# NVIDIA/OpenSeq2Seq

Hardware: AMD Instinct MI355X
Metric: audio-frames/sec/node Jasper10x5 bf16 (train step, objects = input feature frames) (higher is better)
Workload: dtype bf16; 1 GPU; Jasper 10x5 DR (jasper10x5_LibriSpeech_nvgrad_masks) full train step: log-mel front end from int16 PCM resident in HBM+fwd+bwd+NovoGrad/LARC/Backoff, B=32/GPU, durations U[2,16.7]s padded to the batch max, F=64, V=29; global_batch=32, parallelism=dp1, skipped_steps=0

## Files before the change

include/os2s.h:

```cpp
#ifndef OS2S_H_
#define OS2S_H_

#include <stddef.h>
#include <stdint.h>

#ifdef __cplusplus
extern "C" {
#endif

typedef void* os2s_stream_t;

enum {
  OS2S_OK = 0,
  OS2S_ERR_INVALID_ARG = -1,
  OS2S_ERR_LAUNCH = -2,
  OS2S_ERR_UNSUPPORTED = -3,
  OS2S_ERR_WORKSPACE = -4
};

int os2s_abi_version(void);
const char* os2s_strerror(int code);
const char* os2s_last_error_detail(void);
int os2s_deterministic(void);
void os2s_set_deterministic(int on);

size_t os2s_ctc_greedy_decode_workspace_bytes(int T, int B);
int os2s_ctc_greedy_decode(os2s_stream_t stream, const float* logits,
                           const int32_t* seq_len, int T, int B, int V,
                           int blank, int merge_repeated, int32_t* out_ids,
                           int32_t* out_len, float* neg_sum_logits,
                           void* workspace, size_t workspace_bytes);

int os2s_conv1d_num_mtiles(int B, int Tout);
int os2s_conv1d_fwd_ex(os2s_stream_t stream, const uint16_t* x, const uint16_t* w, void* y,
                       const int32_t* in_len, const float* bias, float* stats, int B,
                       int Tin, int Cin, int Cout, int K, int stride, int dil, int padL,
                       int Tout, long long y_stride_b, long long y_stride_t, int out_f32,
                       int accumulate, int act, float keep_prob, unsigned long long seed,
                       const uint16_t* residual, const int32_t* out_len);
int os2s_conv1d_dgrad_bnact_ws(os2s_stream_t stream, const uint16_t* dy, const uint16_t* wT, void* dx,
                               float* stats, int B, int Tin, int Cin, int Cout, int K, int dil, int padL,
                               int Tout, int accumulate, const int32_t* out_len, const uint16_t* mask_ref,
                               float mask_scale, const uint16_t* stat_ref, void* workspace,
                               size_t workspace_bytes);
int os2s_bn_bwd_finalize_raw(os2s_stream_t stream, const float* partial, int nparts, int C, long long count,
                             const float* mean, const float* rstd, float* dgamma, float* dbeta,
                             int accumulate, float* c1, float* c2);
size_t os2s_conv1d_workspace_bytes(void);
int os2s_conv1d_fwd_ws(os2s_stream_t stream, const uint16_t* x, const uint16_t* w, void* y,
                       const int32_t* in_len, const float* bias, float* stats, int B,
                       int Tin, int Cin, int Cout, int K, int stride, int dil, int padL,
                       int Tout, long long y_stride_b, long long y_stride_t, int out_f32,
                       int accumulate, int act, float keep_prob, unsigned long long seed,
                       const uint16_t* residual, const int32_t* out_len, void* workspace,
                       size_t workspace_bytes);
int os2s_conv1d_set_host_lens(const int32_t* lens, int B);
int os2s_set_option(const char* name, double value);
int os2s_get_option(const char* name, double* value);
const char* os2s_option_name(int index);
int os2s_set_debug_stamps(const char* kernel, void* stamps, int mode);
int os2s_clock_probe(void* out_u64x2, unsigned long long spin_cycles);
int os2s_clock_probe_wait(void);
typedef struct {
  const uint16_t* x;
  const uint16_t* w;
  void* y;
  float* stats;
  int Cin, Cout, accumulate;
} os2s_conv_group_t;
int os2s_conv1x1_fwd_grouped(os2s_stream_t stream, const os2s_conv_group_t* groups, int ngroups,
                             const int32_t* in_len, const int32_t* out_len, int B, int T);
typedef struct {
  const uint16_t* x;
  const uint16_t* dy;
  float* dw;
  long long x_row_stride;
  int Cin, Cout;
} os2s_wgrad_group_t;
int os2s_conv1x1_wgrad_grouped(os2s_stream_t stream, const os2s_wgrad_group_t* groups, int ngroups,
                               const int32_t* in_len, int B, int T);
typedef struct {
  const uint16_t* x;
  const uint16_t* dy;
  float* dw;
  long long x_row_stride;
} os2s_cwgrad_group_t;
int os2s_conv1d_wgrad_grouped_ws(os2s_stream_t stream, const os2s_cwgrad_group_t* groups, int ngroups,
                                 const int32_t* in_len, int B, int Tin, int Cin, int Cout, int K,
                                 int stride, int dil, int padL, int Tout, int accumulate,
                                 void* workspace, size_t workspace_bytes);
int os2s_conv1x1_wgrad_grouped_ws(os2s_stream_t stream, const os2s_wgrad_group_t* groups, int ngroups,
                                  const int32_t* in_len, int B, int T, void* workspace,
                                  size_t workspace_bytes);
int os2s_gemm_wgrad_grouped(os2s_stream_t stream, const os2s_wgrad_group_t* groups, int ngroups,
                            long long M, int accumulate, void* workspace, size_t workspace_bytes);
int os2s_gemm_nt(os2s_stream_t stream, const uint16_t* A, long long lda, const uint16_t* W, void* C,
                 long long ldc, int M, int N, int K, const float* bias, int act, float keep_prob,
                 unsigned long long seed, const uint16_t* residual, int accumulate, int out_f32);
int os2s_gemm_nt_ws(os2s_stream_t stream, const uint16_t* A, long long lda, const uint16_t* W, void* C,
                    long long ldc, int M, int N, int K, const float* bias, int act, float keep_prob,
                    unsigned long long seed, const uint16_t* residual, int accumulate, int out_f32,
                    void* workspace, size_t workspace_bytes);
int os2s_gemm_nt_mask_ws(os2s_stream_t stream, const uint16_t* A, long long lda, const uint16_t* W, void* C,
                         long long ldc, int M, int N, int K, const uint16_t* mask_ref, float mask_scale,
                         float* stats, void* workspace, size_t workspace_bytes);
int os2s_conv1d_fwd(os2s_stream_t stream, const uint16_t* x, const uint16_t* w,
                    void* y, const int32_t* in_len, const float* bias,
                    float* stats, int B, int Tin, int Cin, int Cout, int K,
                    int stride, int dil, int padL, int Tout,
                    long long y_stride_b, long long y_stride_t, int out_f32,
                    int accumulate);

int os2s_conv1d_wgrad(os2s_stream_t stream, const uint16_t* x, const uint16_t* dy,
                      float* dw, const int32_t* in_len, int B, int Tin, int Cin,
                      int Cout, int K, int stride, int dil, int padL, int Tout,
                      int accumulate);
int os2s_conv1d_wgrad_ex(os2s_stream_t stream, const uint16_t* x, long long x_row_stride,
                         const uint16_t* dy, float* dw, const int32_t* in_len, int B, int Tin,
                         int Cin, int Cout, int K, int stride, int dil, int padL, int Tout,
                         int accumulate);
int os2s_conv1d_wgrad_ws(os2s_stream_t stream, const uint16_t* x, long long x_row_stride,
                         const uint16_t* dy, float* dw, const int32_t* in_len, int B, int Tin,
                         int Cin, int Cout, int K, int stride, int dil, int padL, int Tout,
                         int accumulate, void* workspace, size_t workspace_bytes);

int os2s_bn_finalize(os2s_stream_t stream, const float* partial, int nparts, int C,
                     long long count, const float* gamma, const float* beta,
                     float eps, float momentum, int training, float* moving_mean,
                     float* moving_var, float* mean_out, float* rstd_out,
                     float* scale_out, float* shift_out);
int os2s_bn_finalize_multi(os2s_stream_t stream, int J, const float* const* partial, int nparts, int C,
                           long long count, const float* const* gamma, const float* const* beta, float eps,
                           float momentum, int training, float* const* moving_mean,
                           float* const* moving_var, float* const* mean_out, float* const* rstd_out,
                           float* const* scale_out, float* const* shift_out);
int os2s_bn_stats_num_parts(long long rows);
int os2s_bn_stats(os2s_stream_t stream, const uint16_t* y, long long rows, int C,
                  float* partial);
int os2s_bn_act_fwd(os2s_stream_t stream, int J, const uint16_t* const* y,
                    const float* const* scale, const float* const* shift,
                    uint16_t* out, const int32_t* out_len, int B, int T, int C,
                    int act, float keep_prob, unsigned long long seed);
int os2s_bn_act_bwd_num_parts(long long rows);
int os2s_bn_act_bwd_reduce(os2s_stream_t stream, int J, const uint16_t* dout,
                           const uint16_t* out, const uint16_t* const* y,
                           const float* const* mean, const float* const* rstd,
                           uint16_t* dz, float* partial, const int32_t* out_len,
                           int B, int T, int C, int act, float keep_prob,
                           unsigned long long seed);
int os2s_bn_bwd_finalize(os2s_stream_t stream, const float* partial, int nparts,
                         int nq, int q, int C, long long count, float* dgamma,
                         float* dbeta, int accumulate, float* c1, float* c2);
int os2s_bn_bwd_finalize_multi(os2s_stream_t stream, const float* partial, int nparts, int J,
                               int C, long long count, float* const* dgamma,
                               float* const* dbeta, int accumulate, float* c1, float* c2);
int os2s_bn_bwd_apply(os2s_stream_t stream, const uint16_t* dz, const uint16_t* y,
                      const float* gamma, const float* mean, const float* rstd,
                      const float* c1, const float* c2, uint16_t* dy,
                      long long rows, int C);
int os2s_bn_bwd_apply_ragged(os2s_stream_t stream, const uint16_t* dz, const uint16_t* y,
                             const float* gamma, const float* mean, const float* rstd,
                             const float* c1, const float* c2, uint16_t* dy,
                             const int32_t* out_len, int margin, int B, int T, int C);
int os2s_bn_bwd_apply_ragged_dz(os2s_stream_t stream, const uint16_t* dz, const uint16_t* y,
                             const float* gamma, const float* mean, const float* rstd,
                             const float* c1, const float* c2, uint16_t* dy,
                             const int32_t* out_len, int margin, int B, int T, int C);
int os2s_dropout_mask(os2s_stream_t stream, unsigned long long seed, long long n8,
                      float keep_prob, uint8_t* out);

size_t os2s_ctc_loss_workspace_bytes(int T, int B, int V, int Lmax);
int os2s_ctc_loss(os2s_stream_t stream, const float* logits, const int32_t* in_len,
                  const int32_t* labels, const int32_t* label_len, int T, int B,
                  int V, int Lmax, int blank, float grad_scale,
                  const float* grad_scale_dev, float* loss_per_sample,
                  float* loss_mean, float* dlogits,
                  uint16_t* dlogits_bf16, int Vpad, void* workspace,
                  size_t workspace_bytes);

#define OS2S_LR_MAX_BOUNDARIES 16
typedef struct {
  int optimizer;
  float beta1, beta2, epsilon, weight_decay;
  int grad_averaging;
  int lr_policy;
  float learning_rate, min_lr, power, decay_rate, max_lr, coefficient;
  long long decay_steps, begin_decay_at, warmup_steps;
  int use_staircase_decay, d_model, has_max_lr;
  int use_larc;
  float larc_eta, larc_min_update, larc_epsilon;
  int larc_mode_scale;
  float clip_global_norm;
  int scaler;
  float scale_min, scale_max, step_factor;
  long long step_window;
  float log_max, lm_beta1, lm_beta2, overflow_std_dev;
  int world_size;
  int pw_count;
  long long pw_boundaries[16];
  float pw_rates[17];
  int novograd_ema;
} os2s_opt_config_t;

int os2s_opt_chunk_elems(void);
size_t os2s_opt_state_bytes(void);
size_t os2s_opt_config_bytes(void);
int os2s_opt_init_state(os2s_stream_t stream, void* state, float loss_scale);
int os2s_opt_step(os2s_stream_t stream, const os2s_opt_config_t* cfg, void* state,
                  const float* grads, float* weights, float* m1, float* m2,
                  uint16_t* w16, int nchunks, int ntensors,
                  const int32_t* chunk_tensor, const int32_t* tensor_chunk_begin,
                  const float* tensor_l2, const float* tensor_wd_mask,
                  float* partial, float* tensor_gnorm2, float* tensor_wnorm2,
                  float* tensor_amax, float* tensor_mult, float* tensor_v);
int os2s_opt_prepare(os2s_stream_t stream, const os2s_opt_config_t* cfg, void* state,
                     const float* grads, const float* weights, int nchunks, int ntensors,
                     const int32_t* chunk_tensor, const int32_t* tensor_chunk_begin,
                     const float* tensor_l2, float* partial, float* tensor_gnorm2, float* tensor_wnorm2,
                     float* tensor_amax, float* tensor_mult, float* tensor_v);
int os2s_opt_apply_range(os2s_stream_t stream, const os2s_opt_config_t* cfg, const void* state,
                         float* grads, float* weights, float* m1, float* m2, uint16_t* w16,
                         int chunk_begin, int chunk_end, const int32_t* chunk_tensor,
                         const float* tensor_l2, const float* tensor_mult,
                         const float* tensor_wd_mask, int zero_grads);
int os2s_cast_f32_to_bf16(os2s_stream_t stream, const float* src, uint16_t* dst,
                          long long n);
int os2s_conv_weight_dgrad_copy(os2s_stream_t stream, const uint16_t* w16,
                                uint16_t* wt16, const void* descs, int ndesc,
                                int total_tiles);

uint32_t os2s_crc32c(uint32_t init, const void* data, size_t n);

size_t os2s_psf_spectrogram_workspace_bytes(int B, int Tpad, int num_features);
int os2s_psf_spectrogram(os2s_stream_t stream, const void* signal, int sample_is_int16,
                         const int32_t* n_samples, int B, long long Nmax, int n_win, int n_step,
                         int pad_to, int num_features, int Tpad, uint16_t* out_bf16, float* out_f32,
                         int32_t* out_len, void* workspace, size_t workspace_bytes);
int os2s_psf_logfbank(os2s_stream_t stream, const void* signal, int sample_is_int16, const int32_t* n_samples,
                      int B, long long Nmax, int n_win, int n_step, int pad_to, int nfilt, int nfft,
                      const float* fb, int Tpad, uint16_t* out_bf16, float* out_f32, int32_t* out_len,
                      void* workspace, size_t workspace_bytes);
int os2s_psf_mfcc(os2s_stream_t stream, const void* signal, int sample_is_int16, const int32_t* n_samples, int B,
                  long long Nmax, int n_win, int n_step, int pad_to, int numcep, int nfilt, int nfft,
                  const float* fb, const float* dctl, int Tpad, uint16_t* out_bf16, float* out_f32,
                  int32_t* out_len, void* workspace, size_t workspace_bytes);
size_t os2s_librosa_features_workspace_bytes(int B, int Tmax, int F);
int os2s_librosa_mfcc(os2s_stream_t stream, const void* signal, const int32_t* n_samples, int sample_is_int16,
                      int B, long long Nmax, int n_fft, int win_length, int hop, int n_mfcc, const double* window,
                      const double* dct, float preemph, float dither, unsigned long long seed, float fixed_gain,
                      int norm_per_feature, const double* features_mean, const double* features_std, int Tmax,
                      int Tpad, uint16_t* out_bf16, float* out_f32, int32_t* out_len, void* workspace,
                      size_t workspace_bytes);
int os2s_librosa_spectrogram(os2s_stream_t stream, const void* signal, const int32_t* n_samples,
                             int sample_is_int16, int B, long long Nmax, int n_win, int hop, int num_features,
                             const double* window, float dither, unsigned long long seed, float fixed_gain,
                             int norm_per_feature, const double* features_mean, const double* features_std,
                             int Tmax, int Tpad, uint16_t* out_bf16, float* out_f32, int32_t* out_len,
                             void* workspace, size_t workspace_bytes);
size_t os2s_logmel_workspace_bytes(int B, int Tmax, int n_mels);
int os2s_logmel(os2s_stream_t stream, const void* signal, const int32_t* n_samples,
                int sample_is_int16, int B, long long Nmax, int n_fft, int hop,
                int n_mels, const float* window, const int32_t* mel_start,
                const int32_t* mel_len, const float* mel_wt, int mel_maxlen,
                float preemph, float dither, unsigned long long seed, float fixed_gain,
                float log_floor, int norm_per_feature, int Tmax, int Tpad,
                uint16_t* out_bf16, float* out_f32, int32_t* out_len, void* workspace,
                size_t workspace_bytes);

int os2s_embed_fwd(os2s_stream_t stream, const int32_t* ids, const int32_t* pos,
                   const uint16_t* table, int V, int D, long long N, float emb_scale,
                   float keep_prob, unsigned long long seed, uint16_t* out, int plain_lookup);
int os2s_embed_bwd(os2s_stream_t stream, const int32_t* ids, const uint16_t* dout, int V,
                   int D, long long N, float emb_scale, float keep_prob,
                   unsigned long long seed, float* dtable, int plain_lookup);
int os2s_layernorm_fwd(os2s_stream_t stream, const uint16_t* x, const float* gamma,
                       const float* beta, float eps, long long N, int D, uint16_t* y,
                       float* mean, float* rstd);
int os2s_layernorm_bwd_num_parts(long long N);
int os2s_layernorm_bwd(os2s_stream_t stream, const uint16_t* dy, const uint16_t* x,
                       const float* gamma, const float* mean, const float* rstd,
                       const uint16_t* dres, long long N, int D, uint16_t* dx,
                       float* partial);
int os2s_layernorm_l1_fwd(os2s_stream_t stream, const uint16_t* x, const float* gamma,
                          const float* beta, float eps, long long N, int D, uint16_t* y,
                          float* mean, float* rinv);
int os2s_layernorm_l1_bwd_num_parts(long long N);
int os2s_layernorm_l1_bwd(os2s_stream_t stream, const uint16_t* dy, const uint16_t* x,
                          const float* gamma, const float* mean, const float* rinv,
                          const uint16_t* dres, long long N, int D, uint16_t* dx,
                          float* partial);
int os2s_token_bn_apply(os2s_stream_t stream, const uint16_t* x, const float* scale,
                        const float* shift, long long N, int D, uint16_t* y);
int os2s_token_bn_bwd_num_parts(long long N);
int os2s_token_bn_bwd_reduce(os2s_stream_t stream, const uint16_t* dy, const uint16_t* x,
                             const float* mean, const float* rstd, long long N, int D,
                             float* partial);
int os2s_token_bn_bwd_apply(os2s_stream_t stream, const uint16_t* dy, const uint16_t* x,
                            const float* gamma, const float* mean, const float* rstd,
                            const float* c1, const float* c2, const uint16_t* dres,
                            long long N, int D, uint16_t* dx);
int os2s_dropout_bwd(os2s_stream_t stream, const uint16_t* dout, const uint16_t* out,
                     int mode, float keep_prob, unsigned long long seed, long long n,
                     uint16_t* d);
int os2s_dropout_bwd_colsum_num_parts(long long rows);
int os2s_dropout_bwd_colsum(os2s_stream_t stream, const uint16_t* dout, const uint16_t* out, int mode,
                            float keep_prob, unsigned long long seed, long long rows, int C,
                            uint16_t* d, float* partial);
int os2s_add_bf16(os2s_stream_t stream, const uint16_t* a, const uint16_t* b, long long n,
                  uint16_t* out);
int os2s_attention_fwd(os2s_stream_t stream, const uint16_t* q, const uint16_t* k,
                       const uint16_t* v, uint16_t* o, float* lse, const int32_t* cu_q,
                       const int32_t* cu_k, int B, int H, int dh, int max_len,
                       long long ldq, long long ldk, long long ldv, long long ldo,
                       int causal, float scale, float keep_prob, unsigned long long seed);
int os2s_attention_bwd(os2s_stream_t stream, const uint16_t* q, const uint16_t* k,
                       const uint16_t* v, const uint16_t* d_o, const float* lse,
                       uint16_t* dq, uint16_t* dk, uint16_t* dv, const int32_t* cu_q,
                       const int32_t* cu_k, int B, int H, int dh, int max_len,
                       long long ldq, long long ldk, long long ldv, long long lddo,
                       long long lddq, long long lddk, long long lddv, int causal,
                       float scale, float keep_prob, unsigned long long seed);
int os2s_xent_smooth(os2s_stream_t stream, const uint16_t* logits, const int32_t* labels,
                     long long N, int V, int V_valid, long long ld, float label_smoothing,
                     float grad_scale, const float* grad_scale_dev, float* row_loss,
                     float* loss_mean, uint16_t* dlogits);
int os2s_argmax_rows(os2s_stream_t stream, const uint16_t* x, long long N, int V_valid,
                     long long ld, int32_t* out);

int os2s_augment_signal(os2s_stream_t stream, const void* signal, int is_int16, int B,
                        long long nmax, const int32_t* n_in, const int32_t* n_out,
                        const double* ratio, const float* noise_amp, float fixed_gain,
                        const float* interp_win, int nwin, int num_table, unsigned long long seed,
                        uint32_t* absmax_scratch, float* out, long long nout_max);
int os2s_spec_augment(os2s_stream_t stream, uint16_t* feats, int B, int T, int F,
                      const int32_t* masks, int n_masks);

int os2s_beam_chunks(int V);
long long os2s_beam_workspace_bytes(int B, int beam, int V);
int os2s_beam_init(os2s_stream_t stream, int B, int beam, int max_decode_length,
                   const int32_t* initial_ids, int32_t* status, int32_t* alive_seq,
                   int32_t* fin_seq, float* alive_lp, float* fin_scores, int32_t* fin_flags,
                   int32_t* last_ids, int32_t* pos);
int os2s_beam_step(os2s_stream_t stream, const void* logits, int logits_f32, long long ld, int B,
                   int beam, int V, int max_decode_length, int eos_id, const float* lnorm,
                   int32_t* status, int32_t* alive_seq, int32_t* fin_seq, float* alive_lp,
                   float* fin_scores, int32_t* fin_flags, int32_t* parent, float* topk_lp,
                   int32_t* topk_idx, int32_t* last_ids, int32_t* pos, void* workspace);
int os2s_beam_finalize(os2s_stream_t stream, int B, int beam, int max_decode_length,
                       const int32_t* status, const int32_t* alive_seq, const int32_t* fin_seq,
                       const float* alive_lp, const float* fin_scores, const int32_t* fin_flags,
                       int32_t* out_seq, float* out_scores);
long long os2s_tf_beam_workspace_bytes(int B, int beam);
int os2s_tf_beam_step(os2s_stream_t stream, const void* logits, int logits_f32, long long ld, int B,
                      int beam, int V, int eos_id, int time, float length_penalty_weight,
                      float* log_probs, int32_t* finished, int32_t* lengths, int32_t* word_ids,
                      int32_t* parent, float* scores, void* workspace);
int os2s_gather_rows(os2s_stream_t stream, const void* src, const int32_t* idx, long long rows,
                     long long row_bytes, const int32_t* enable, void* dst);
int os2s_dense_epilogue(os2s_stream_t stream, uint16_t* y, const float* bias, long long rows, int C,
                        int act, float keep_prob, unsigned long long seed, const uint16_t* residual);
int os2s_gemm_skinny(os2s_stream_t stream, const uint16_t* x, long long ldx, const uint16_t* w,
                     long long ldw, const float* bias, const uint16_t* residual, long long ldr,
                     int M, int N, int K, int relu, uint16_t* y, long long ldy);
int os2s_decode_self_attention(os2s_stream_t stream, const uint16_t* q, long long ldq,
                               const uint16_t* knew, const uint16_t* vnew, long long ldnew,
                               uint16_t* kcache, uint16_t* vcache, int32_t* ancestry, int N,
                               int H, int dh, int Tmax, int step, const int32_t* status_dev,
                               float scale, uint16_t* o, long long ldo);
int os2s_decode_cross_attention(os2s_stream_t stream, const uint16_t* q, long long ldq,
                                const uint16_t* k, const uint16_t* v, long long ldkv,
                                const int32_t* cu_k, int beam, int N, int H, int dh,
                                int max_len, float scale, uint16_t* o, long long ldo);

size_t os2s_rnn_fwd_workspace_bytes(int B, int H);
long long os2s_gru_xcd_launch_count(void);
void os2s_gru_xcd_set_mode(int mode);
int os2s_gru_xcd_status(int clear);
// ... 276 lines not shown
```

openseq2seq_amd/capi.py:

```python
import torch

from . import _lib
from ._lib import c_void_p, c_int, c_float

c_ll = _lib.ctypes.c_longlong


_raw_stream = getattr(torch._C, "_cuda_getCurrentRawStream", None)
_cur_device = getattr(torch._C, "_cuda_getDevice", None)


def _stream():
  if _raw_stream is not None and _cur_device is not None:
    return c_void_p(_raw_stream(_cur_device()))
  return c_void_p(torch.cuda.current_stream().cuda_stream)


def _ptr(t, dtype=None, allow_none=False):
  if t is None:
    if allow_none:
      return None
    raise ValueError("tensor required")
  if not t.is_cuda:
    raise _lib.Os2sError("os2s kernels need CUDA(HIP) tensors; got %s" % t.device)
# ... 168 lines not shown
def zero_arena_leave(depth):
  global _zero_arena
  _zero_arena = _zero_arenas[max(depth - 1, 0)]


def zero_arena_reset():
  zero_arena_enter(0)


def zero_scratch(shape, device):
  return _zero_arena.take(tuple(shape), device)


def conv1d_dgrad_bnact(dy, wt, dx, *, dil, pad_left, accumulate, out_len, mask_ref, mask_scale, stat_ref):
  B, Tin, Cin = dy.shape
  K, Cout, _ = wt.shape
  Tout = dx.shape[1]
  assert tuple(dx.shape) == (B, Tout, Cout) == tuple(mask_ref.shape) == tuple(stat_ref.shape)
  assert dx.is_contiguous() and mask_ref.is_contiguous() and stat_ref.is_contiguous() and dy.is_contiguous()
  stats = _zero_arena.take((conv1d_num_mtiles(B, Tout), 2, Cout), dy.device)
  ws = conv1d_workspace(dy.device)
  _lib.C.os2s_conv1d_dgrad_bnact_ws(_stream(), _ptr(dy, torch.bfloat16), _ptr(wt, torch.bfloat16),
                                    _ptr(dx, torch.bfloat16), _ptr(stats, torch.float32), B, Tin, Cin, Cout, K,
                                    int(dil), int(pad_left), Tout, int(bool(accumulate)),
                                    _ptr(out_len, torch.int32, True), _ptr(mask_ref, torch.bfloat16), float(mask_scale),
                                    _ptr(stat_ref, torch.bfloat16), _ptr(ws), ws.numel())
  return stats


def bn_bwd_finalize_raw(partial, count, mean, rstd, dgamma, dbeta, accumulate, c1, c2):
  nparts, two, C = partial.shape
  assert two == 2
  _lib.C.os2s_bn_bwd_finalize_raw(_stream(), _ptr(partial, torch.float32), nparts, C, int(count),
                                  _ptr(mean, torch.float32), _ptr(rstd, torch.float32),
                                  _ptr(dgamma, torch.float32, True), _ptr(dbeta, torch.float32, True), int(accumulate),
                                  _ptr(c1, torch.float32), _ptr(c2, torch.float32))


class _ConvGroup(_lib.ctypes.Structure):
  _fields_ = [("x", c_void_p), ("w", c_void_p), ("y", c_void_p), ("stats", c_void_p),
              ("Cin", c_int), ("Cout", c_int), ("accumulate", c_int)]


def conv1x1_fwd_grouped(items, in_len=None, out_len=None, out_f32=False):
  B, T, _ = items[0]["x"].shape
  ydt = torch.float32 if out_f32 else torch.bfloat16
  outs = [it["y"].data_ptr() for it in items]
  assert len(set(outs)) == len(outs), "two groups of one launch must not write the same tensor"
  for i0 in range(0, len(items), 16):
    part = items[i0:i0 + 16]
    arr = (_ConvGroup * len(part))()
    for g, it in zip(arr, part):
      x, w, y = it["x"], it["w"], it["y"]
      assert x.shape[0] == B and x.shape[1] == T and w.shape[0] == 1 and w.shape[2] == x.shape[2]
      assert tuple(y.shape) == (B, T, w.shape[1]) and x.is_contiguous() and y.is_contiguous()
      g.x, g.w, g.y = _ptr(x, torch.bfloat16), _ptr(w, torch.bfloat16), _ptr(y, ydt)
      g.stats = _ptr(it.get("stats"), torch.float32, True)
      g.Cin, g.Cout, g.accumulate = x.shape[2], w.shape[1], int(bool(it.get("accumulate", False)))
    _lib.C.os2s_conv1x1_fwd_grouped_ex(_stream(), arr, len(part), _ptr(in_len, torch.int32, True),
                                       _ptr(out_len, torch.int32, True), B, T, int(bool(out_f32)))


def _rows_view_ok(t):
  return t.dim() == 3 and t.stride(2) == 1 and t.stride(0) == t.shape[1] * t.stride(1) and t.stride(1) % 8 == 0


def dres_copy_cols(src, dst, lens=None, want_colsum=False):
  B, T, C = src.shape
  assert tuple(dst.shape) == (B, T, C) and _rows_view_ok(src) and _rows_view_ok(dst)
  assert src.dtype == torch.bfloat16 and dst.dtype == torch.bfloat16
  part = None
  if want_colsum:
    n = int(_lib.C.os2s_dres_copy_num_parts(B, T))
    part = torch.empty((n, C), dtype=torch.float32, device=src.device)
  _lib.C.os2s_dres_copy_cols(_stream(), c_void_p(src.data_ptr()), src.stride(1), c_void_p(dst.data_ptr()),
                             dst.stride(1), _ptr(lens, torch.int32, True), B, T, C, _ptr(part, torch.float32, True))
  return part


def dres_cov(colsum_partial, gram, count, s, m, chl):
  nparts, C = colsum_partial.shape
  assert tuple(gram.shape[-2:]) == (C, C) and chl.numel() == 2 * C * C and s.numel() == C and m.numel() == C
  _lib.C.os2s_dres_cov(_stream(), _ptr(colsum_partial, torch.float32), nparts, _ptr(gram, torch.float32), C, int(count),
                       _ptr(s, torch.float32), _ptr(m, torch.float32), _ptr(chl, torch.bfloat16))


class _DresSeg(_lib.ctypes.Structure):
  _fields_ = [("w", c_void_p), ("tt", c_void_p), ("m", c_void_p), ("s", c_void_p), ("gamma", c_void_p),
              ("beta", c_void_p), ("moving_mean", c_void_p), ("moving_var", c_void_p), ("mean", c_void_p),
              ("rstd", c_void_p), ("dgamma", c_void_p), ("dbeta", c_void_p), ("dw", c_void_p), ("wd1", c_void_p),
              ("wd2", c_void_p), ("wt", c_void_p), ("ld", c_ll), ("c", c_int), ("koff", c_int)]


def dres_seg_table(segs, device):
  import ctypes
  arr = (_DresSeg * len(segs))()
  for g, d in zip(arr, segs):
    for k, _ in _DresSeg._fields_:
      v = d[k]
      if k in ("ld", "c", "koff"):
        setattr(g, k, int(v))
      else:
        setattr(g, k, None if v is None else v.data_ptr())
  raw = bytes(ctypes.string_at(ctypes.addressof(arr), ctypes.sizeof(arr)))
  return torch.frombuffer(bytearray(raw), dtype=torch.uint8).to(device)


def dres_bn_fwd(table, nseg, Cout, Kk, wp, shift, count, eps, momentum, training):
  assert wp.numel() == Cout * Kk and shift.numel() == Cout and table.numel() == nseg * _lib.ctypes.sizeof(_DresSeg)
  _lib.C.os2s_dres_bn_fwd(_stream(), _ptr(table, torch.uint8), nseg, Cout, Kk, _ptr(wp, torch.bfloat16),
                          _ptr(shift, torch.float32), int(count), float(eps), float(momentum), int(bool(training)))


def dres_bn_bwd(table, nseg, Cout, Kk, P, mean_dz, count, coef):
  assert P.numel() == Cout * Kk and mean_dz.numel() == Cout and coef.numel() >= nseg * 4 * Cout
  _lib.C.os2s_dres_bn_bwd(_stream(), _ptr(table, torch.uint8), nseg, Cout, Kk, _ptr(P, torch.float32),
                          _ptr(mean_dz, torch.float32), int(count), _ptr(coef, torch.float32))


def conv1x1_cat_fwd(x, w, y, in_len=None, out_len=None, bias=None, accumulate=False):
  B, T, Cin = x.shape
  Cout = w.shape[-2]
  assert w.shape[-1] == Cin and w.is_contiguous() and w.numel() == Cout * Cin and w.dtype == torch.bfloat16
  assert tuple(y.shape) == (B, T, Cout) and _rows_view_ok(x) and _rows_view_ok(y)
  assert x.dtype == torch.bfloat16 and y.dtype == torch.bfloat16
  ws = conv1d_workspace(x.device)
  _lib.C.os2s_conv1x1_cat_fwd(_stream(), c_void_p(x.data_ptr()), x.stride(1), c_void_p(w.data_ptr()),
                              c_void_p(y.data_ptr()), y.stride(1), _ptr(in_len, torch.int32, True),
                              _ptr(out_len, torch.int32, True), _ptr(bias, torch.float32, True), B, T, Cin, Cout,
                              int(bool(accumulate)), _ptr(ws), ws.numel())
  return y


def conv1d_wgrad(x, dy, K, *, stride=1, dil=1, pad_left=None, in_len=None,
                 out=None, accumulate=False, use_workspace=True):
  B, Tin, Cin = x.shape
  B2, Tout, Cout = dy.shape
  assert B == B2
  if pad_left is None:
    tout, pad_left = same_padding(Tin, K, stride, dil)
    assert tout == Tout
  if out is None:
    assert not accumulate
    out = torch.empty((K, Cout, Cin), dtype=torch.float32, device=x.device)
  assert x.stride(2) == 1 and x.stride(0) == Tin * x.stride(1)
  ws = conv1d_workspace(x.device) if use_workspace else None
  _lib.C.os2s_conv1d_wgrad_ws(_stream(), c_void_p(x.data_ptr()), x.stride(1), _ptr(dy, torch.bfloat16),
                              _ptr(out, torch.float32), _ptr(in_len, torch.int32, True), B, Tin,
                              Cin, Cout, K, stride, dil, pad_left, Tout, int(accumulate), _ptr(ws, None, True),
                              ws.numel() if ws is not None else 0)
  return out


class _CWgradGroup(_lib.ctypes.Structure):
  _fields_ = [("x", c_void_p), ("dy", c_void_p), ("dw", c_void_p), ("x_row_stride", c_ll)]


def conv1d_wgrad_grouped(items, K, *, stride=1, dil=1, pad_left=None, in_len=None, accumulate=True):
  n = len(items)
  assert 1 <= n <= 8
  x0, dy0 = items[0]["x"], items[0]["dy"]
  B, Tin, Cin = x0.shape
  _, Tout, Cout = dy0.shape
  if pad_left is None:
    tout, pad_left = same_padding(Tin, K, stride, dil)
    assert tout == Tout
  arr = (_CWgradGroup * n)()
  for g, it in zip(arr, items):
    x, dy, dw = it["x"], it["dy"], it["dw"]
    assert tuple(x.shape) == (B, Tin, Cin) and tuple(dy.shape) == (B, Tout, Cout) and tuple(dw.shape) == (K, Cout, Cin)
    assert x.stride(2) == 1 and x.stride(0) == Tin * x.stride(1) and x.stride(1) == x0.stride(1)
    g.x, g.dy, g.dw = c_void_p(x.data_ptr()), _ptr(dy, torch.bfloat16), _ptr(dw, torch.float32)
    g.x_row_stride = x.stride(1)
  ws = conv1d_workspace(x0.device)
  _lib.C.os2s_conv1d_wgrad_grouped_ws(_stream(), arr, n, _ptr(in_len, torch.int32, True), B, Tin, Cin, Cout, K, stride,
                                      dil, pad_left, Tout, int(bool(accumulate)), _ptr(ws), ws.numel())


ACT_NONE, ACT_RELU, ACT_TANH = 0, 1, 2


class _WgradGroup(_lib.ctypes.Structure):
  _fields_ = [("x", c_void_p), ("dy", c_void_p), ("dw", c_void_p), ("x_row_stride", c_ll),
              ("Cin", c_int), ("Cout", c_int)]


def conv1x1_wgrad_grouped(items, in_len=None, pingpong=True):
  n = len(items)
  assert 1 <= n <= 16
  B, T, _ = items[0]["x"].shape
  arr = (_WgradGroup * n)()
  for i, it in enumerate(items):
    x, dy, dw = it["x"], it["dy"], it["dw"]
    assert x.shape[:2] == (B, T) and dy.shape[:2] == (B, T) and x.dtype == torch.bfloat16
    assert x.stride(2) == 1 and x.stride(0) == T * x.stride(1) and dy.is_contiguous()
    assert dw.dtype == torch.float32 and dw.is_contiguous() and dw.numel() == dy.shape[2] * x.shape[2]
    g = arr[i]
    g.x, g.dy, g.dw = c_void_p(x.data_ptr()), _ptr(dy, torch.bfloat16), _ptr(dw, torch.float32)
    g.x_row_stride, g.Cin, g.Cout = x.stride(1), x.shape[2], dy.shape[2]
  if not pingpong:
    _lib.C.os2s_conv1x1_wgrad_grouped(_stream(), arr, n, _ptr(in_len, torch.int32, True), B, T)
    return
  ws = conv1d_workspace(items[0]["x"].device)
  _lib.C.os2s_conv1x1_wgrad_grouped_ws(_stream(), arr, n, _ptr(in_len, torch.int32, True), B, T, _ptr(ws), ws.numel())


def gemm_wgrad_grouped(items, accumulate=True):
  n = len(items)
  assert 1 <= n <= 16
  M = items[0]["x"].shape[0]
  arr = (_WgradGroup * n)()
  keep = []
  for g, it in zip(arr, items):
    x, dy, dw = it["x"], it["dy"], it["dw"]
    if dy.stride(1) != 1 or dy.stride(0) != dy.shape[1]:
      dy = dy.contiguous()
    if x.stride(1) != 1 or x.stride(0) % 8:
      x = x.contiguous()
    keep += [x, dy]
    assert x.shape[0] == M and dy.shape[0] == M and x.dtype == torch.bfloat16 and dy.dtype == torch.bfloat16
    assert dw.dtype == torch.float32 and dw.is_contiguous() and tuple(dw.shape[-2:]) == (dy.shape[1], x.shape[1])
    g.x, g.dy, g.dw = c_void_p(x.data_ptr()), c_void_p(dy.data_ptr()), _ptr(dw, torch.float32)
    g.x_row_stride, g.Cin, g.Cout = x.stride(0), x.shape[1], dy.shape[1]
  ws = conv1d_workspace(items[0]["x"].device)
  _lib.C.os2s_gemm_wgrad_grouped(_stream(), arr, n, M, int(bool(accumulate)), _ptr(ws), ws.numel())


def _ptr_array(tensors, dtype):
  arr = (c_void_p * len(tensors))()
  for i, t in enumerate(tensors):
    arr[i] = _ptr(t, dtype)
  return arr


def bn_finalize(partial, count, gamma, beta, eps, momentum, training, moving_mean,
                moving_var, mean_out, rstd_out, scale_out, shift_out):
  C = scale_out.numel()
  nparts = 0 if partial is None else partial.shape[0]
  _lib.C.os2s_bn_finalize(_stream(), _ptr(partial, torch.float32, True), nparts, C, int(count),
                          _ptr(gamma, torch.float32, True), _ptr(beta, torch.float32, True),
                          float(eps), float(momentum), int(training),
                          _ptr(moving_mean, torch.float32, True), _ptr(moving_var, torch.float32, True),
                          _ptr(mean_out, torch.float32, True), _ptr(rstd_out, torch.float32, True),
                          _ptr(scale_out, torch.float32), _ptr(shift_out, torch.float32))


def bn_finalize_multi(items, count, eps, momentum, training):
  J = len(items)
  C = items[0]["scale_out"].numel()
  nparts = 0 if items[0]["partial"] is None else items[0]["partial"].shape[0]
  keys = ("partial", "gamma", "beta", "moving_mean", "moving_var", "mean_out", "rstd_out", "scale_out", "shift_out")
  arrs = {}
  for k in keys:
    a = (c_void_p * J)()
    for j, it in enumerate(items):
      t = it.get(k)
      assert t is None or (t.dtype == torch.float32 and t.is_contiguous())
      if k == "partial" and t is not None:
        assert t.shape[0] == nparts and t.shape[2] == C
      a[j] = None if t is None else t.data_ptr()
    arrs[k] = a
  _lib.C.os2s_bn_finalize_multi(_stream(), J, arrs["partial"], nparts, C, int(count), arrs["gamma"], arrs["beta"],
                                float(eps), float(momentum), int(training), arrs["moving_mean"], arrs["moving_var"],
                                arrs["mean_out"], arrs["rstd_out"], arrs["scale_out"], arrs["shift_out"])


def bn_stats(y2d):
  rows, C = y2d.shape
  n = int(_lib.C.os2s_bn_stats_num_parts(rows))
  partial = torch.empty((n, 2, C), dtype=torch.float32, device=y2d.device)
  _lib.C.os2s_bn_stats(_stream(), _ptr(y2d, torch.bfloat16), rows, C, _ptr(partial))
  return partial


def sample_norm_fwd(x, gamma, beta, mode, eps):
  B, T, C = x.shape
  assert x.is_contiguous() and x.dtype == torch.bfloat16
  dev = x.device
  z = torch.empty_like(x)
  mean = torch.empty((B, C), dtype=torch.float32, device=dev)
  rstd = torch.empty((B, C), dtype=torch.float32, device=dev)
  nf = int(_lib.C.os2s_sample_norm_partial_floats(B, C))
  part = torch.empty(nf, dtype=torch.float32, device=dev)
  _lib.C.os2s_sample_norm_fwd(_stream(), _ptr(x, torch.bfloat16), _ptr(gamma, torch.float32), _ptr(beta, torch.float32),
                              B, T, C, int(mode), float(eps), _ptr(z, torch.bfloat16), _ptr(mean, torch.float32),
                              _ptr(rstd, torch.float32), _ptr(part, torch.float32))
  return z, mean, rstd


def sample_norm_bwd(dz, x, gamma, mean, rstd, mode, dgamma, dbeta):
  B, T, C = x.shape
  assert x.is_contiguous() and dz.is_contiguous()
  dev = x.device
  dx = torch.empty_like(x)
  nf = int(_lib.C.os2s_sample_norm_partial_floats(B, C))
  part = torch.empty(nf, dtype=torch.float32, device=dev)
  scratch = torch.empty(4 * B * C, dtype=torch.float32, device=dev)
  _lib.C.os2s_sample_norm_bwd(_stream(), _ptr(dz, torch.bfloat16), _ptr(x, torch.bfloat16), _ptr(gamma, torch.float32),
                              _ptr(mean, torch.float32), _ptr(rstd, torch.float32), B, T, C, int(mode),
                              _ptr(dx, torch.bfloat16), _ptr(dgamma, torch.float32), _ptr(dbeta, torch.float32),
                              _ptr(part, torch.float32), _ptr(scratch, torch.float32))
  return dx


def bn_act_fwd(ys, scales, shifts, out, out_len, act, keep_prob, seed):
  B, T, C = out.shape
# ... 16 lines not shown
  _lib.C.os2s_bn_act_bwd_reduce(_stream(), J, _ptr(dout, torch.bfloat16), _ptr(out, torch.bfloat16),
                                _ptr_array(ys, torch.bfloat16), _ptr_array(means, torch.float32),
                                _ptr_array(rstds, torch.float32), _ptr(dz, torch.bfloat16),
                                _ptr(partial, torch.float32), _ptr(out_len, torch.int32, True), B, T, C,
                                int(act), float(keep_prob), int(seed) & (2**64 - 1))


def bn_bwd_finalize(partial, q, count, dgamma, dbeta, accumulate, c1, c2):
  nparts, nq, C = partial.shape
  _lib.C.os2s_bn_bwd_finalize(_stream(), _ptr(partial, torch.float32), nparts, nq, q, C, int(count),
                              _ptr(dgamma, torch.float32, True), _ptr(dbeta, torch.float32, True),
                              int(accumulate), _ptr(c1, torch.float32), _ptr(c2, torch.float32))


def colsum_finalize(partial, dgamma, dbeta):
  scratch = torch.empty((2, partial.shape[2]), dtype=torch.float32, device=partial.device)
  bn_bwd_finalize(partial, 1, 1, dgamma, dbeta, True, scratch[0], scratch[1])


def bn_bwd_finalize_multi(partial, count, dgammas, dbetas, accumulate, c1, c2):
  import ctypes
  nparts, nq, C = partial.shape
  J = nq - 1
  assert len(dgammas) == J and len(dbetas) == J and tuple(c1.shape) == (J, C) == tuple(c2.shape)
  arr = ctypes.c_void_p * J
  dg = arr(*[t.data_ptr() if t is not None else None for t in dgammas])
  db = arr(*[t.data_ptr() if t is not None else None for t in dbetas])
  _lib.C.os2s_bn_bwd_finalize_multi(_stream(), _ptr(partial, torch.float32), nparts, J, C, int(count), dg, db,
                                    int(accumulate), _ptr(c1, torch.float32), _ptr(c2, torch.float32))


def bn_bwd_apply(dz, y, gamma, mean, rstd, c1, c2, dy, out_len=None, margin=0, dz_to_len=False):
  C = dz.shape[-1]
  rows = dz.numel() // C
  if out_len is not None:
    B, T = dz.shape[0], dz.shape[1]
    f = _lib.C.os2s_bn_bwd_apply_ragged_dz if dz_to_len else _lib.C.os2s_bn_bwd_apply_ragged
    f(_stream(), _ptr(dz, torch.bfloat16), _ptr(y, torch.bfloat16),
      _ptr(gamma, torch.float32, True), _ptr(mean, torch.float32),
      _ptr(rstd, torch.float32), _ptr(c1, torch.float32), _ptr(c2, torch.float32),
      _ptr(dy, torch.bfloat16), _ptr(out_len, torch.int32), int(margin), B, T, C)
    return dy
  assert not dz_to_len
  _lib.C.os2s_bn_bwd_apply(_stream(), _ptr(dz, torch.bfloat16), _ptr(y, torch.bfloat16),
                           _ptr(gamma, torch.float32, True), _ptr(mean, torch.float32),
                           _ptr(rstd, torch.float32), _ptr(c1, torch.float32), _ptr(c2, torch.float32),
                           _ptr(dy, torch.bfloat16), rows, C)
  return dy


def dropout_mask(seed, n_elems, keep_prob, device):
  assert n_elems % 8 == 0
  out = torch.empty((n_elems // 8,), dtype=torch.uint8, device=device)
  _lib.C.os2s_dropout_mask(_stream(), int(seed) & (2**64 - 1), n_elems // 8, float(keep_prob),
                           _ptr(out))
  bits = (out[:, None].to(torch.int32) >> torch.arange(8, device=device)[None, :]) & 1
  return bits.reshape(-1).bool()


def ctc_loss(logits, in_len, labels, label_len, blank=None, grad_scale=1.0,
             want_grad=True, want_grad_bf16=False, vpad=32, grad_scale_dev=None):
  T, B, V = logits.shape
  Lmax = labels.shape[1]
  if blank is None:
    blank = V - 1
  dev = logits.device
  nbytes = int(_lib.C.os2s_ctc_loss_workspace_bytes(T, B, V, Lmax))
  ws = torch.empty((nbytes,), dtype=torch.uint8, device=dev)
  lps = torch.empty((B,), dtype=torch.float32, device=dev)
  lm = torch.empty((1,), dtype=torch.float32, device=dev)
  dl = torch.empty((T, B, V), dtype=torch.float32, device=dev) if want_grad else None
  dl16 = (torch.empty((B, T, vpad), dtype=torch.bfloat16, device=dev)
          if want_grad_bf16 else None)
  _lib.C.os2s_ctc_loss(_stream(), _ptr(logits, torch.float32), _ptr(in_len, torch.int32),
                       _ptr(labels, torch.int32), _ptr(label_len, torch.int32), T, B, V, Lmax,
                       int(blank), float(grad_scale), _ptr(grad_scale_dev, torch.float32, True),
                       _ptr(lps), _ptr(lm),
                       _ptr(dl, None, True), _ptr(dl16, None, True), int(vpad), _ptr(ws), nbytes)
  return {"loss_per_sample": lps, "loss_mean": lm, "dlogits": dl, "dlogits_bf16": dl16}


class OptConfig(_lib.ctypes.Structure):
  _fields_ = [
      ("optimizer", c_int), ("beta1", c_float), ("beta2", c_float), ("epsilon", c_float),
      ("weight_decay", c_float), ("grad_averaging", c_int), ("lr_policy", c_int),
      ("learning_rate", c_float), ("min_lr", c_float), ("power", c_float),
      ("decay_rate", c_float), ("max_lr", c_float), ("coefficient", c_float),
      ("decay_steps", c_ll), ("begin_decay_at", c_ll), ("warmup_steps", c_ll),
      ("use_staircase_decay", c_int), ("d_model", c_int), ("has_max_lr", c_int),
      ("use_larc", c_int), ("larc_eta", c_float), ("larc_min_update", c_float),
      ("larc_epsilon", c_float), ("larc_mode_scale", c_int), ("clip_global_norm", c_float),
      ("scaler", c_int), ("scale_min", c_float), ("scale_max", c_float),
      ("step_factor", c_float), ("step_window", c_ll), ("log_max", c_float),
      ("lm_beta1", c_float), ("lm_beta2", c_float), ("overflow_std_dev", c_float),
      ("world_size", c_int), ("pw_count", c_int), ("pw_boundaries", c_ll * 16), ("pw_rates", c_float * 17),
      ("novograd_ema", c_int),
  ]


OPT_STATE_FIELDS = [
    ("global_step", "q"), ("scaler_iteration", "q"), ("last_overflow_iteration", "q"),
    ("num_skipped", "q"), ("loss_scale", "f"), ("lr", "f"), ("global_grad_norm", "f"),
    ("grad_amax", "f"), ("has_nan", "i"), ("skip", "i"), ("x_hat", "f"),
    ("slow_x_hat", "f"), ("xsquared_hat", "f"), ("b1_correction", "f"),
    ("b2_correction", "f"), ("grad_scale_latched", "f"),
]


def opt_chunk_elems():
  return int(_lib.C.os2s_opt_chunk_elems())


def opt_state_bytes():
  n = int(_lib.C.os2s_opt_state_bytes())
  assert int(_lib.C.os2s_opt_config_bytes()) == _lib.ctypes.sizeof(OptConfig), \
      "OptConfig ctypes mirror out of sync with os2s_opt_config_t"
  return n


def opt_init_state(state, loss_scale):
  _lib.C.os2s_opt_init_state(_stream(), _ptr(state, torch.uint8), float(loss_scale))


def opt_read_state(state):
  import struct
  raw = bytes(state.cpu().numpy().tobytes())
  fmt = "<" + "".join(c for _, c in OPT_STATE_FIELDS)
  vals = struct.unpack(fmt, raw[:struct.calcsize(fmt)])
  gru_xcd_check()
  return dict(zip([n for n, _ in OPT_STATE_FIELDS], vals))


def gru_xcd_status(clear=False):
  return int(_lib.C.os2s_gru_xcd_status(int(bool(clear))))


def gru_xcd_launch_count():
  return int(_lib.C.os2s_gru_xcd_launch_count())


def gru_xcd_set_mode(mode):
  _lib.C.os2s_gru_xcd_set_mode(int(mode))


def gru_xcd_check(clear=False):
  st = gru_xcd_status(clear)
  if st and not clear:
    raise _lib.Os2sError("a persistent GRU launch gave up (code %d: 1 = poll timeout, 2 = workgroup placement); "
                         "the step's results are invalid. OS2S_GRU_XCD=0 selects the launch-per-step path" % st)
  return st


def opt_step(cfg, state, grads, weights, m1, m2, w16, chunk_tensor, tensor_chunk_begin,
             tensor_l2, tensor_wd_mask, partial, gnorm2, wnorm2, amax, mult, tensor_v):
  nchunks = chunk_tensor.numel()
  ntensors = tensor_chunk_begin.numel() - 1
  _lib.C.os2s_opt_step(_stream(), _lib.ctypes.byref(cfg), _ptr(state, torch.uint8),
                       _ptr(grads, torch.float32), _ptr(weights, torch.float32),
                       _ptr(m1, torch.float32, True), _ptr(m2, torch.float32, True),
                       _ptr(w16, torch.bfloat16, True), nchunks, ntensors,
                       _ptr(chunk_tensor, torch.int32), _ptr(tensor_chunk_begin, torch.int32),
                       _ptr(tensor_l2, torch.float32, True), _ptr(tensor_wd_mask, torch.float32, True),
                       _ptr(partial, torch.float32), _ptr(gnorm2, torch.float32),
                       _ptr(wnorm2, torch.float32), _ptr(amax, torch.float32),
                       _ptr(mult, torch.float32), _ptr(tensor_v, torch.float32, True))


def opt_prepare(cfg, state, grads, weights, chunk_tensor, tensor_chunk_begin, tensor_l2, partial, gnorm2, wnorm2,
                amax, mult, tensor_v):
  nchunks = chunk_tensor.numel()
  ntensors = tensor_chunk_begin.numel() - 1
  _lib.C.os2s_opt_prepare(_stream(), _lib.ctypes.byref(cfg), _ptr(state, torch.uint8), _ptr(grads, torch.float32),
                          _ptr(weights, torch.float32), nchunks, ntensors, _ptr(chunk_tensor, torch.int32),
                          _ptr(tensor_chunk_begin, torch.int32), _ptr(tensor_l2, torch.float32, True),
                          _ptr(partial, torch.float32), _ptr(gnorm2, torch.float32), _ptr(wnorm2, torch.float32),
                          _ptr(amax, torch.float32), _ptr(mult, torch.float32), _ptr(tensor_v, torch.float32, True))


def opt_apply_range(cfg, state, grads, weights, m1, m2, w16, chunk_begin, chunk_end, chunk_tensor, tensor_l2, mult,
                    zero_grads=False):
  _lib.C.os2s_opt_apply_range(_stream(), _lib.ctypes.byref(cfg), _ptr(state, torch.uint8), _ptr(grads, torch.float32),
                              _ptr(weights, torch.float32), _ptr(m1, torch.float32, True),
                              _ptr(m2, torch.float32, True), _ptr(w16, torch.bfloat16, True), int(chunk_begin),
                              int(chunk_end), _ptr(chunk_tensor, torch.int32), _ptr(tensor_l2, torch.float32, True),
                              _ptr(mult, torch.float32), c_void_p(0), int(bool(zero_grads)))


def cast_f32_to_bf16(src, dst):
  n = src.numel()
  _lib.C.os2s_cast_f32_to_bf16(_stream(), _ptr(src, torch.float32), _ptr(dst, torch.bfloat16), n)


def conv_weight_dgrad_copy(w16, wt16, descs, total_tiles):
  ndesc = descs.shape[0]
  _lib.C.os2s_conv_weight_dgrad_copy(_stream(), _ptr(w16, torch.bfloat16), _ptr(wt16, torch.bfloat16),
                                     _ptr(descs, torch.uint8), ndesc, int(total_tiles))


def _feature_buffers(signal, F, t_ws, tpad, want_f32, workspace_bytes_fn):
  B, dev = signal.shape[0], signal.device
  assert signal.dtype in (torch.int16, torch.float32)
  nbytes = int(workspace_bytes_fn(B, t_ws, F))
  ws = torch.empty((nbytes,), dtype=torch.uint8, device=dev)
  out = torch.empty((B, tpad, F), dtype=torch.bfloat16, device=dev)
  out32 = torch.empty((B, tpad, F), dtype=torch.float32, device=dev) if want_f32 else None
  olen = torch.empty((B,), dtype=torch.int32, device=dev)
  return ws, nbytes, out, out32, olen


def logmel(signal, n_samples, window, mel_start, mel_len, mel_wt, *, hop, n_mels, tmax, tpad,
           preemph=0.97, dither=0.0, seed=0, fixed_gain=-1.0, log_floor=1e-20,
           norm_per_feature=True, want_f32=False, n_fft=512):
  B, Nmax = signal.shape
  ws, nbytes, out, out32, olen = _feature_buffers(signal, n_mels, tmax, tpad, want_f32,
                                                  _lib.C.os2s_logmel_workspace_bytes)
  _lib.C.os2s_logmel(_stream(), _ptr(signal), _ptr(n_samples, torch.int32), int(signal.dtype == torch.int16), B, Nmax,
                     n_fft, hop, n_mels, _ptr(window, torch.float32), _ptr(mel_start, torch.int32),
                     _ptr(mel_len, torch.int32), _ptr(mel_wt, torch.float32), mel_wt.shape[0],
                     float(preemph), float(dither), int(seed) & (2**64 - 1), float(fixed_gain),
                     float(log_floor), int(bool(norm_per_feature)), tmax, tpad, _ptr(out),
                     _ptr(out32, None, True), _ptr(olen), _ptr(ws), nbytes)
  return out, olen, out32


def psf_spectrogram(signal, n_samples, *, n_win, n_step, pad_to, num_features, tpad, want_f32=False):
  B, Nmax = signal.shape
  ws, nbytes, out, out32, olen = _feature_buffers(signal, num_features, tpad, tpad, want_f32,
                                                  _lib.C.os2s_psf_spectrogram_workspace_bytes)
  _lib.C.os2s_psf_spectrogram(_stream(), _ptr(signal), int(signal.dtype == torch.int16), _ptr(n_samples, torch.int32),
                              B, Nmax, n_win, n_step, pad_to, num_features, tpad, _ptr(out), _ptr(out32, None, True),
                              _ptr(olen), _ptr(ws), nbytes)
  return out, olen, out32


def psf_logfbank(signal, n_samples, fb, *, n_win, n_step, pad_to, nfft, tpad, want_f32=False):
  B, Nmax = signal.shape
  nfilt = fb.shape[0]
  assert fb.is_contiguous() and fb.shape[1] == nfft // 2 + 1
  ws, nbytes, out, out32, olen = _feature_buffers(signal, nfilt, tpad, tpad, want_f32,
                                                  _lib.C.os2s_psf_spectrogram_workspace_bytes)
  _lib.C.os2s_psf_logfbank(_stream(), _ptr(signal), int(signal.dtype == torch.int16), _ptr(n_samples, torch.int32), B,
                           Nmax, n_win, n_step, pad_to, nfilt, nfft, _ptr(fb, torch.float32), tpad, _ptr(out),
                           _ptr(out32, None, True), _ptr(olen), _ptr(ws), nbytes)
  return out, olen, out32


def psf_mfcc(signal, n_samples, fb, dctl, *, n_win, n_step, pad_to, nfft, tpad, want_f32=False):
  B, Nmax = signal.shape
  nfilt, numcep = fb.shape[0], dctl.shape[0]
  assert fb.is_contiguous() and fb.shape[1] == nfft // 2 + 1 and dctl.is_contiguous() and dctl.shape[1] == nfilt
  ws, nbytes, out, out32, olen = _feature_buffers(signal, numcep, tpad, tpad, want_f32,
                                                  _lib.C.os2s_psf_spectrogram_workspace_bytes)
  _lib.C.os2s_psf_mfcc(_stream(), _ptr(signal), int(signal.dtype == torch.int16), _ptr(n_samples, torch.int32), B,
                       Nmax, n_win, n_step, pad_to, numcep, nfilt, nfft, _ptr(fb, torch.float32),
                       _ptr(dctl, torch.float32), tpad, _ptr(out), _ptr(out32, None, True), _ptr(olen), _ptr(ws),
                       nbytes)
  return out, olen, out32


def librosa_mfcc(signal, n_samples, window, dct, *, win_length, hop, tmax, tpad, preemph=0.97, dither=0.0, seed=0,
                 fixed_gain=-1.0, norm_per_feature=False, features_mean=None, features_std=None, want_f32=False):
  B, Nmax = signal.shape
  n_fft, F = window.numel(), dct.shape[0]
  assert dct.is_contiguous() and dct.shape[1] == n_fft // 2 + 1
  assert all(t is None or t.numel() == F for t in (features_mean, features_std))
  ws, nbytes, out, out32, olen = _feature_buffers(signal, F, tmax, tpad, want_f32,
                                                  _lib.C.os2s_librosa_features_workspace_bytes)
  _lib.C.os2s_librosa_mfcc(_stream(), _ptr(signal), _ptr(n_samples, torch.int32), int(signal.dtype == torch.int16),
                           B, Nmax, n_fft, int(win_length), int(hop), F, _ptr(window, torch.float64),
                           _ptr(dct, torch.float64), float(preemph), float(dither), int(seed) & (2**64 - 1),
                           float(fixed_gain), int(bool(norm_per_feature)), _ptr(features_mean, torch.float64, True),
                           _ptr(features_std, torch.float64, True), tmax, tpad, _ptr(out), _ptr(out32, None, True),
                           _ptr(olen), _ptr(ws), nbytes)
  return out, olen, out32


def librosa_spectrogram(signal, n_samples, window, *, hop, num_features, tmax, tpad, dither=0.0, seed=0,
                        fixed_gain=-1.0, norm_per_feature=False, features_mean=None, features_std=None,
                        want_f32=False):
  B, Nmax = signal.shape
  n_win, F = window.numel(), int(num_features)
  assert all(t is None or t.numel() == F for t in (features_mean, features_std))
  ws, nbytes, out, out32, olen = _feature_buffers(signal, F, tmax, tpad, want_f32,
                                                  _lib.C.os2s_librosa_features_workspace_bytes)
  _lib.C.os2s_librosa_spectrogram(_stream(), _ptr(signal), _ptr(n_samples, torch.int32),
                                  int(signal.dtype == torch.int16), B, Nmax, n_win, int(hop), F,
                                  _ptr(window, torch.float64), float(dither), int(seed) & (2**64 - 1),
                                  float(fixed_gain), int(bool(norm_per_feature)),
                                  _ptr(features_mean, torch.float64, True), _ptr(features_std, torch.float64, True),
                                  tmax, tpad, _ptr(out), _ptr(out32, None, True), _ptr(olen), _ptr(ws), nbytes)
  return out, olen, out32


def augment_signal(signal, n_in, n_out, ratio, noise_amp, interp_win, num_table, nout_max, seed=0,
                   fixed_gain=-1.0):
  B, Nmax = signal.shape
  dev = signal.device
  is_i16 = signal.dtype == torch.int16
  assert is_i16 or signal.dtype == torch.float32
  out = torch.empty((B, int(nout_max)), dtype=torch.float32, device=dev)
  scratch = torch.empty(B, dtype=torch.int32, device=dev)
  _lib.C.os2s_augment_signal(_stream(), _ptr(signal), int(is_i16), B, Nmax, _ptr(n_in, torch.int32),
                             _ptr(n_out, torch.int32), _ptr(ratio, torch.float64), _ptr(noise_amp, torch.float32, True),
                             float(fixed_gain), _ptr(interp_win, torch.float32), interp_win.numel(), int(num_table),
                             int(seed) & (2**64 - 1), _ptr(scratch), _ptr(out), int(nout_max))
  return out


def spec_augment(feats, masks):
  B, T, F = feats.shape
  _lib.C.os2s_spec_augment(_stream(), _ptr(feats, torch.bfloat16), B, T, F, _ptr(masks, torch.int32), masks.shape[1])
  return feats


BIG_TILE_MIN_ROWS = 256


def gemm(x2d, w, **kw):
  plain = (all(kw.get(k) is None for k in ("residual", "stats", "in_len", "out_len"))
           and not kw.get("act", 0) and not kw.get("out_f32", False) and not kw.get("time_major", False)
           and kw.get("keep_prob", 1.0) >= 1.0)
  bias = kw.get("bias", None)
  if bias is not None and bias.dtype != torch.float32:
    plain = False
  if plain and x2d.shape[0] >= BIG_TILE_MIN_ROWS and x2d.stride(1) == 1 and w.stride(1) == 1:
    out_t = kw.get("out", None)
    if (x2d.shape[1] % 64 == 0 and w.shape[0] % 8 == 0 and w.is_contiguous() and x2d.stride(0) % 8 == 0
          and (out_t is None or (out_t.stride(1) == 1 and out_t.stride(0) % 8 == 0))):
      return gemm_nt(x2d, w, out=out_t, bias=bias, accumulate=bool(kw.get("accumulate", False)))
  out = kw.pop("out", None)
  N, Cin = x2d.shape
  Cout = w.shape[0]
  if out is not None:
    out = out.view(1, N, Cout)
  res = kw.pop("residual", None)
  if res is not None:
    res = res.view(1, N, Cout)
  y = conv1d_fwd(x2d.view(1, N, Cin), w.view(1, Cout, Cin), pad_left=0, tout=N, out=out,
# ... 1041 lines not shown
```

openseq2seq_amd/csrc/conv1d_wgrad.hip:

```cpp
#include "os2s_common.hpp"
#include "os2s_split_reduce.hpp"

namespace os2s {

struct WgradArgs {
  const bf16_t* x;
  const bf16_t* dy;
  float* dw;
  const int32_t* in_len;
  int B, Tin, Tout, Cin, Cout, K, stride, dil, padL;
  int NCO, NCI, NTP, NSPLIT, steps_per_split, use_atomic;
  float* part;
  int xrows, xrows_pad;
  int xbuf_bytes, steptab_bytes;
  long long x_ld;
  int accumulate;
  float* ws_slabs;
  int* ws_cnt;
  int ws_nslabs, ncu, force_split;
  int xcd_order;
  int NG;
  const bf16_t* gx[8];
  const bf16_t* gdy[8];
  float* gdw[8];
// ... 851 lines not shown
#pragma unroll
          for (int j = 0; j < 2; ++j)
            acc[1][i][j] = __builtin_amdgcn_mfma_f32_32x32x16_bf16(yf[i][kk], xf[j][kk], acc[1][i][j], 0, 0, 0);
      wpp_barrier();
    }
    if (!grp) wpp_barrier();
  }
  __syncthreads();

  if (npiece > 1) {
    const int sidx = rank - nfull;
    auto at = [&](int v) -> f32x16& { return acc[v >> 2][(v >> 1) & 1][v & 1]; };
    if (!split_publish_and_reduce(at, p.ws_slabs + (size_t)sidx * f * kSplitSlabFloats,
                                  p.ws_cnt + sidx, piece, f, smem, tid))
      return;
  }

  const int l31 = lane & 31;
  const bool inside = __builtin_amdgcn_readfirstlane((co0 + 256 <= p.Cout && ci0 + 256 <= p.Cin) ? 1 : 0);
#pragma unroll
  for (int e = 0; e < 2; ++e) {
    const int cob = co0 + grp * 128 + e * 64, cib = ci0 + wn * 64;
    if (inside) {
      float* const base = p.dw + (long long)(cob + 4 * lhi) * p.Cin + cib + l31;
      float old[2][2][16];
      if (p.accumulate) {
#pragma unroll
        for (int i = 0; i < 2; ++i)
#pragma unroll
          for (int j = 0; j < 2; ++j)
#pragma unroll
            for (int v = 0; v < 16; ++v)
              old[i][j][v] = base[(long long)(i * 32 + (v & 3) + 8 * (v >> 2)) * p.Cin + j * 32];
#pragma unroll
        for (int i = 0; i < 2; ++i)
#pragma unroll
          for (int j = 0; j < 2; ++j)
#pragma unroll
            for (int v = 0; v < 16; ++v) acc[e][i][j][v] += old[i][j][v];
      }
#pragma unroll
      for (int i = 0; i < 2; ++i)
#pragma unroll
        for (int j = 0; j < 2; ++j)
#pragma unroll
          for (int v = 0; v < 16; ++v)
            base[(long long)(i * 32 + (v & 3) + 8 * (v >> 2)) * p.Cin + j * 32] = acc[e][i][j][v];
    } else {
#pragma unroll
      for (int i = 0; i < 2; ++i)
#pragma unroll
        for (int j = 0; j < 2; ++j) {
          const int ci = cib + j * 32 + l31;
#pragma unroll
          for (int v = 0; v < 16; ++v) {
            const int co = cob + i * 32 + (v & 3) + 8 * (v >> 2) + 4 * lhi;
            if (co < p.Cout && ci < p.Cin) {
              float* dst = p.dw + (long long)co * p.Cin + ci;
              float val = acc[e][i][j][v];
              if (p.accumulate) val += *dst;
              *dst = val;
            }
          }
        }
    }
  }
}

}

static int g_wgrad_pp_min_units = 8;
static int g_wgrad_k1_pp = -1;
static bool wgrad1x1_pp_auto(int B, int T, int Cin, int Cout, bool have_ws) {
  if (g_wgrad_k1_pp == 0) return false;
  if (g_wgrad_k1_pp == 1) return true;
  const long long rows = (long long)B * T;
  const int units = os2s::ceil_div(Cout, 256) * os2s::ceil_div(Cin, 256);
  return have_ws && rows >= 2048 && units >= 32;
}
static int g_wgrad_variant = -1;
static int g_wgrad_split = -1;
static int g_wgrad_sw_ablate = 0;
static int g_wgrad_xcd = 1;
static unsigned long long* g_wgrad_dbg = nullptr;
static int g_wgrad_dbg_mode = 0;
static os2s::OptionReg r_wg_variant("conv1d_wgrad.variant", &g_wgrad_variant);
static os2s::OptionReg r_wg_split("conv1d_wgrad.split", &g_wgrad_split);
static os2s::OptionReg r_wg_abl("conv1d_wgrad.sw_ablate", &g_wgrad_sw_ablate);
static os2s::OptionReg r_wg_xcd("conv1d_wgrad.xcd_order", &g_wgrad_xcd);
static os2s::OptionReg r_wg_min("conv1d_wgrad.pp_min_units", &g_wgrad_pp_min_units, "OS2S_WGRAD_PP_MIN_UNITS");
static os2s::OptionReg r_wg_k1("conv1d_wgrad.k1_pp", &g_wgrad_k1_pp, "OS2S_WGRAD1X1_PP");
static os2s::StampReg r_wg_stamps("conv1d_wgrad", [](void* stamps, int mode) {
  g_wgrad_dbg = (unsigned long long*)stamps;
  g_wgrad_dbg_mode = mode;
});


static os2s::WgradArgs wgrad_args(const uint16_t* x, long long x_ld, const uint16_t* dy, float* dw,
                                  const int32_t* in_len, int B, int T, int Cin, int Cout, int accumulate) {
  os2s::WgradArgs a{};
  a.x = x; a.dy = dy; a.dw = dw; a.in_len = in_len; a.x_ld = x_ld;
  a.B = B; a.Tin = T; a.Tout = T; a.Cin = Cin; a.Cout = Cout;
  a.K = 1; a.stride = 1; a.dil = 1;
  a.accumulate = accumulate ? 1 : 0;
  a.NTP = 1; a.NSPLIT = 1; a.NG = 1;
  a.xrows = 64; a.xrows_pad = 64;
  a.ncu = 256; a.force_split = g_wgrad_split; a.xcd_order = g_wgrad_xcd != 0;
  return a;
}

static void wgrad_tap_quad_geometry(os2s::WgradArgs& a, int xbuf_bytes) {
  using namespace os2s;
  a.NCO = ceil_div(a.Cout, 128);
  a.NCI = ceil_div(a.Cin, 128);
  a.NTP = ceil_div(a.K, kWppTaps);
  a.xrows = 63 + (kWppTaps - 1) * a.dil + 1;
  a.xrows_pad = ceil_div(a.xrows, 4) * 4;
  a.xbuf_bytes = xbuf_bytes;
  a.steptab_bytes = ceil_div(a.B * ceil_div(a.Tout, 64) * 4, 16) * 16;
}

static int wgrad_split_grid(os2s::WgradArgs& a, int units, void* workspace, size_t workspace_bytes) {
  a.ncu = os2s::device_cus();
  const os2s::SplitWorkspace ws = os2s::split_carve(workspace, workspace_bytes, a.ncu);
  a.ws_cnt = ws.tickets; a.ws_slabs = ws.slabs; a.ws_nslabs = ws.nslabs;
  return units + os2s::split_tail_pieces(units, a.ncu, ws.nslabs);
}

static os2s::WgradGroupTable wgrad_group_table(const os2s_wgrad_group_t* groups, int ngroups, int edge, int nsplit) {
  using namespace os2s;
  WgradGroupTable gt;
  gt.ngroups = ngroups;
  int units = 0;
  for (int i = 0; i < kMaxWgradGroups; ++i) {
    const os2s_wgrad_group_t& s = groups[i < ngroups ? i : 0];
    WgradGroup& g = gt.g[i];
    g.x = s.x; g.dy = s.dy; g.dw = s.dw; g.x_ld = s.x_row_stride;
    g.Cin = s.Cin; g.Cout = s.Cout; g.NCI = ceil_div(s.Cin, edge);
    g.unit_begin = units;
    if (i < ngroups) units += ceil_div(s.Cout, edge) * g.NCI * nsplit;
  }
  gt.total_units = units;
  return gt;
}

static int launch_wgrad1x1_pp(hipStream_t stream, os2s::WgradArgs a, const os2s::WgradGroupTable& gt, int units,
                              void* workspace, size_t workspace_bytes) {
  using namespace os2s;
  const int grid = wgrad_split_grid(a, units, workspace, workspace_bytes);
  OS2S_LAUNCH_LDS(conv1d_wgrad1x1_pp_kernel, dim3(grid), dim3(512), (size_t)160 * 1024, stream, a, gt);
  return OS2S_OK;
}

static int conv1d_wgrad_impl_g(os2s_stream_t stream, const uint16_t* x, long long x_row_stride,
                               const uint16_t* dy, float* dw, const int32_t* in_len, int B,
                               int Tin, int Cin, int Cout, int K, int stride, int dil,
                               int padL, int Tout, int accumulate, void* workspace,
                               size_t workspace_bytes, const os2s_cwgrad_group_t* groups, int ngroups) {
  using namespace os2s;
  OS2S_REQUIRE(x_row_stride >= Cin && x_row_stride % 8 == 0);
  OS2S_REQUIRE(x && dy && dw);
  OS2S_REQUIRE(B >= 0 && Tin >= 1 && Tout >= 1 && Cin >= 8 && Cout >= 8 && K >= 1);
  OS2S_REQUIRE(Cin % 8 == 0 && Cout % 8 == 0 && stride >= 1 && dil >= 1);
  if (B == 0) return OS2S_OK;
  WgradArgs a = wgrad_args(x, x_row_stride, dy, dw, in_len, B, Tin, Cin, Cout, accumulate);
  a.Tout = Tout; a.K = K; a.stride = stride; a.dil = dil; a.padL = padL;
  a.dbg = g_wgrad_dbg; a.dbg_mode = g_wgrad_dbg_mode;
  if (groups) {
    a.NG = ngroups;
    for (int i = 0; i < ngroups; ++i) { a.gx[i] = groups[i].x; a.gdy[i] = groups[i].dy; a.gdw[i] = groups[i].dw; }
  }

  const bool pp_shape = stride == 1 && K >= 2 && B <= 64 && Cout >= 128 && Cin >= 64 &&
                        Tin < 65536 && Tout <= 255 * 64 && 63 + 3 * dil + 1 <= 96 &&
                        (long long)Tin * x_row_stride * 2 < (1ll << 30) &&
                        (long long)Tin * x_row_stride * 2 < (1ll << 31) &&
                        (long long)Tout * Cout * 2 < (1ll << 31);
  const int pp_units = ceil_div(Cout, 128) * ceil_div(Cin, 128) * ceil_div(K, kWppTaps);
  const bool sw_shape = pp_shape && 63 + 3 * dil + 1 <= kSwXInstr * 16 &&
                        Cout % 128 == 0 && Cin % 128 == 0;
  if (sw_shape && g_wgrad_variant == 3 && !groups) {
    wgrad_tap_quad_geometry(a, kSwXBuf);
    const size_t smem = (size_t)kSwRing * (kSwYBuf + kSwXBuf) + a.steptab_bytes;
    if (smem <= 160 * 1024) {
      const int grid = wgrad_split_grid(a, pp_units, workspace, workspace_bytes);
#ifdef OS2S_SW_ABLATE
      switch (g_wgrad_sw_ablate) {
        case 1: OS2S_LAUNCH_LDS(conv1d_wgrad_sw_kernel<1>, dim3(grid), dim3(256), smem, (hipStream_t)stream, a); return OS2S_OK;
        case 2: OS2S_LAUNCH_LDS(conv1d_wgrad_sw_kernel<2>, dim3(grid), dim3(256), smem, (hipStream_t)stream, a); return OS2S_OK;
        case 3: OS2S_LAUNCH_LDS(conv1d_wgrad_sw_kernel<3>, dim3(grid), dim3(256), smem, (hipStream_t)stream, a); return OS2S_OK;
        case 4: OS2S_LAUNCH_LDS(conv1d_wgrad_sw_kernel<4>, dim3(grid), dim3(256), smem, (hipStream_t)stream, a); return OS2S_OK;
        case 5: OS2S_LAUNCH_LDS(conv1d_wgrad_sw_kernel<5>, dim3(grid), dim3(256), smem, (hipStream_t)stream, a); return OS2S_OK;
        case 8: OS2S_LAUNCH_LDS(conv1d_wgrad_sw_kernel<8>, dim3(grid), dim3(256), smem, (hipStream_t)stream, a); return OS2S_OK;
        default: break;
      }
#endif
      OS2S_LAUNCH_LDS(conv1d_wgrad_sw_kernel<0>, dim3(grid), dim3(256), smem, (hipStream_t)stream, a);
      return OS2S_OK;
    }
  }

  if (pp_shape && g_wgrad_variant != 0 && (groups || g_wgrad_variant == 1 || pp_units >= g_wgrad_pp_min_units)) {
    wgrad_tap_quad_geometry(a, 24 * 1024);
    const size_t smem = (size_t)2 * 64 * 256 + (size_t)3 * a.xbuf_bytes + a.steptab_bytes + (a.dbg ? 2 * 48 * 10 * 8 : 0);
    if (smem <= 160 * 1024) {
      const int grid = wgrad_split_grid(a, a.NG * pp_units, workspace, workspace_bytes);
      if (a.dbg) {
        OS2S_LAUNCH_LDS(conv1d_wgrad_pp_kernel<true>, dim3(grid), dim3(512), smem, (hipStream_t)stream, a);
      } else {
        OS2S_LAUNCH_LDS(conv1d_wgrad_pp_kernel<false>, dim3(grid), dim3(512), smem, (hipStream_t)stream, a);
      }
      return OS2S_OK;
    }
  }

  if (groups) return OS2S_ERR_UNSUPPORTED;

  const bool pp1_shape = K == 1 && stride == 1 && padL == 0 && Tin == Tout && B <= 64 &&
                         Cout >= 128 && Cin >= 128 && x_row_stride * 2 * 64 < (1ll << 30) &&
                         (long long)Cout * 2 * 64 < (1ll << 30);
  if (pp1_shape && g_wgrad_variant != 0 && g_wgrad_variant != 1 &&
      (g_wgrad_variant == 2 || wgrad1x1_pp_auto(B, Tout, Cin, Cout, workspace != nullptr))) {
    a.NCO = ceil_div(Cout, 256);
    a.NCI = ceil_div(Cin, 256);
    WgradGroupTable none;
    none.ngroups = 0; none.total_units = 0;
    return launch_wgrad1x1_pp((hipStream_t)stream, a, none, a.NCO * a.NCI, workspace, workspace_bytes);
  }

  const int TAPS = K == 1 ? 1 : 2;
  const bool wide = (Cout % 256 == 0) && (K >= 8) && (Cout >= 512);
  const int COT = wide ? 256 : 128;
  a.NCO = ceil_div(Cout, COT);
  a.NCI = ceil_div(Cin, 128);
  a.NTP = ceil_div(K, TAPS);
  const int base_blocks = a.NCO * a.NCI * a.NTP;
  const int total_steps = B * ceil_div(Tout, 64);
  int nsplit = 1;
  if (accumulate) {
    const int target = wide ? 256 : 512;
    nsplit = ceil_div(target, base_blocks);
    const int max_split = total_steps / 8 > 0 ? total_steps / 8 : 1;
    if (nsplit > max_split) nsplit = max_split;
    if (nsplit < 1) nsplit = 1;
    if (os2s_deterministic()) nsplit = 1;
  }
  const long long dw_elems = (long long)K * Cout * Cin;
  if (workspace) {
    const long long part_room = workspace_bytes > kSplitTicketBytes
                                    ? (long long)((workspace_bytes - kSplitTicketBytes) / ((size_t)dw_elems * 4)) : 0;
    if (nsplit > part_room) nsplit = (int)part_room;
    if (nsplit < 1) nsplit = 1;
  }
  a.steps_per_split = ceil_div(total_steps, nsplit);
  a.NSPLIT = ceil_div(total_steps, a.steps_per_split);
  if (workspace && a.NSPLIT > 1)
    a.part = reinterpret_cast<float*>(reinterpret_cast<char*>(workspace) + kSplitTicketBytes);
  a.use_atomic = (accumulate && !a.part) ? 1 : 0;
  a.xrows = 63 * stride + (TAPS - 1) * dil + 1;
  a.xrows_pad = ceil_div(a.xrows, 4) * 4;
  const size_t smem = (size_t)2 * 64 * 2 * COT + (size_t)2 * a.xrows_pad * 256;
  if (smem > 160 * 1024) return OS2S_ERR_UNSUPPORTED;
  const int nunits = a.NCO * a.NCI * a.NSPLIT;
  const int grid = ceil_div(nunits, 8) * 8 * a.NTP;
  if (wide) {
    if (TAPS == 1)
      OS2S_LAUNCH_LDS((conv1d_wgrad_kernel<1, 256>), dim3(grid), dim3(512), smem, (hipStream_t)stream, a);
    else
      OS2S_LAUNCH_LDS((conv1d_wgrad_kernel<2, 256>), dim3(grid), dim3(512), smem, (hipStream_t)stream, a);
  } else {
    if (TAPS == 1)
      OS2S_LAUNCH_LDS((conv1d_wgrad_kernel<1, 128>), dim3(grid), dim3(256), smem, (hipStream_t)stream, a);
    else
      OS2S_LAUNCH_LDS((conv1d_wgrad_kernel<2, 128>), dim3(grid), dim3(256), smem, (hipStream_t)stream, a);
  }
  if (a.part) {
    const int blocks = ceil_div(dw_elems, 256) < 2048 ? ceil_div(dw_elems, 256) : 2048;
    OS2S_LAUNCH(wgrad_split_sum_kernel, dim3(blocks), dim3(256), 0, (hipStream_t)stream,
                (const float*)a.part, dw, dw_elems, a.NSPLIT);
  }
  return OS2S_OK;
}

extern "C" int os2s_conv1d_wgrad_ws(os2s_stream_t stream, const uint16_t* x, long long x_row_stride,
                                    const uint16_t* dy, float* dw, const int32_t* in_len, int B,
                                    int Tin, int Cin, int Cout, int K, int stride, int dil,
                                    int padL, int Tout, int accumulate, void* workspace,
                                    size_t workspace_bytes) {
  return conv1d_wgrad_impl_g(stream, x, x_row_stride, dy, dw, in_len, B, Tin, Cin, Cout, K, stride,
                             dil, padL, Tout, accumulate, workspace, workspace_bytes, nullptr, 1);
}

extern "C" int os2s_conv1d_wgrad_ex(os2s_stream_t stream, const uint16_t* x, long long x_row_stride,
                                    const uint16_t* dy, float* dw, const int32_t* in_len, int B,
                                    int Tin, int Cin, int Cout, int K, int stride, int dil,
                                    int padL, int Tout, int accumulate) {
  return conv1d_wgrad_impl_g(stream, x, x_row_stride, dy, dw, in_len, B, Tin, Cin, Cout, K, stride,
                             dil, padL, Tout, accumulate, nullptr, 0, nullptr, 1);
}

extern "C" int os2s_conv1d_wgrad(os2s_stream_t stream, const uint16_t* x,
                                 const uint16_t* dy, float* dw,
                                 const int32_t* in_len, int B, int Tin, int Cin,
                                 int Cout, int K, int stride, int dil, int padL,
                                 int Tout, int accumulate) {
  return conv1d_wgrad_impl_g(stream, x, Cin, dy, dw, in_len, B, Tin, Cin, Cout, K, stride, dil,
                             padL, Tout, accumulate, nullptr, 0, nullptr, 1);
}

extern "C" int os2s_conv1d_wgrad_grouped_ws(os2s_stream_t stream, const os2s_cwgrad_group_t* groups, int ngroups,
                                            const int32_t* in_len, int B, int Tin, int Cin, int Cout, int K,
                                            int stride, int dil, int padL, int Tout, int accumulate,
                                            void* workspace, size_t workspace_bytes) {
  OS2S_REQUIRE(groups && ngroups >= 1 && ngroups <= 8);
  for (int i = 0; i < ngroups; ++i) OS2S_REQUIRE(groups[i].x && groups[i].dy && groups[i].dw);
  for (int i = 1; i < ngroups; ++i) OS2S_REQUIRE(groups[i].x_row_stride == groups[0].x_row_stride);
  int rc = OS2S_ERR_UNSUPPORTED;
  if (ngroups > 1)
    rc = conv1d_wgrad_impl_g(stream, groups[0].x, groups[0].x_row_stride, groups[0].dy, groups[0].dw, in_len, B, Tin,
                             Cin, Cout, K, stride, dil, padL, Tout, accumulate, workspace, workspace_bytes, groups,
                             ngroups);
  if (rc != OS2S_ERR_UNSUPPORTED) return rc;
  for (int i = 0; i < ngroups; ++i) {
    rc = conv1d_wgrad_impl_g(stream, groups[i].x, groups[i].x_row_stride, groups[i].dy, groups[i].dw, in_len, B, Tin,
                             Cin, Cout, K, stride, dil, padL, Tout, accumulate, workspace, workspace_bytes, nullptr, 1);
    if (rc != OS2S_OK) return rc;
  }
  return OS2S_OK;
}


extern "C" int os2s_conv1x1_wgrad_grouped(os2s_stream_t stream, const os2s_wgrad_group_t* groups, int ngroups,
                                          const int32_t* in_len, int B, int T) {
  using namespace os2s;
  OS2S_REQUIRE(groups && ngroups >= 1 && ngroups <= kMaxWgradGroups && B >= 0 && T >= 1);
  if (B == 0) return OS2S_OK;
  int tiles = 0;
  for (int i = 0; i < ngroups; ++i) {
    const os2s_wgrad_group_t& s = groups[i];
    OS2S_REQUIRE(s.x && s.dy && s.dw && s.Cin >= 8 && s.Cout >= 8 && s.Cin % 8 == 0 && s.Cout % 8 == 0);
    OS2S_REQUIRE(s.x_row_stride >= s.Cin && s.x_row_stride % 8 == 0);
    tiles += ceil_div(s.Cout, 128) * ceil_div(s.Cin, 128);
  }
  const int total_steps = B * ceil_div(T, 64);
  int nsplit = ceil_div(512, tiles);
  const int max_split = total_steps / 8 > 0 ? total_steps / 8 : 1;
  if (nsplit > max_split) nsplit = max_split;
  if (tiles >= 256 || nsplit < 1 || os2s_deterministic()) nsplit = 1;
  WgradArgs a = wgrad_args(nullptr, 0, nullptr, nullptr, in_len, B, T, 0, 0, 1);
  a.force_split = -1;
  a.steps_per_split = ceil_div(total_steps, nsplit);
  a.NSPLIT = ceil_div(total_steps, a.steps_per_split);
  a.use_atomic = 1;
  const WgradGroupTable gt = wgrad_group_table(groups, ngroups, 128, a.NSPLIT);
  const size_t smem = (size_t)2 * 64 * 2 * 128 + (size_t)2 * a.xrows_pad * 256;
  OS2S_LAUNCH_LDS(conv1d_wgrad_grouped_kernel, dim3(gt.total_units), dim3(256), smem, (hipStream_t)stream, a, gt);
  return OS2S_OK;
}


extern "C" int os2s_conv1x1_wgrad_grouped_ws(os2s_stream_t stream, const os2s_wgrad_group_t* groups, int ngroups,
                                             const int32_t* in_len, int B, int T, void* workspace,
                                             size_t workspace_bytes) {
  using namespace os2s;
  OS2S_REQUIRE(groups && ngroups >= 1 && ngroups <= kMaxWgradGroups && B >= 0 && T >= 1);
  if (B == 0) return OS2S_OK;
  bool pp = B <= 64 && (long long)B * T >= 2048 && workspace != nullptr;
  for (int i = 0; i < ngroups && pp; ++i) {
    const os2s_wgrad_group_t& s = groups[i];
    OS2S_REQUIRE(s.x && s.dy && s.dw && s.Cin >= 8 && s.Cout >= 8 && s.Cin % 8 == 0 && s.Cout % 8 == 0);
    OS2S_REQUIRE(s.x_row_stride >= s.Cin && s.x_row_stride % 8 == 0);
    pp = s.Cin >= 128 && s.Cout >= 128 && s.x_row_stride * 2 * 64 < (1ll << 30) &&
         (long long)s.Cout * 2 * 64 < (1ll << 30);
  }
  if (!pp) return os2s_conv1x1_wgrad_grouped(stream, groups, ngroups, in_len, B, T);
  const WgradGroupTable gt = wgrad_group_table(groups, ngroups, 256, 1);
  const os2s_wgrad_group_t& g0 = groups[0];
  WgradArgs a = wgrad_args(g0.x, g0.x_row_stride, g0.dy, g0.dw, in_len, B, T, g0.Cin, g0.Cout, 1);
  a.NCO = gt.total_units; a.NCI = 1;
  return launch_wgrad1x1_pp((hipStream_t)stream, a, gt, gt.total_units, workspace, workspace_bytes);
}

extern "C" int os2s_gemm_wgrad_grouped(os2s_stream_t stream, const os2s_wgrad_group_t* groups, int ngroups,
                                       long long M, int accumulate, void* workspace, size_t workspace_bytes) {
  using namespace os2s;
  OS2S_REQUIRE(groups && ngroups >= 1 && ngroups <= kMaxWgradGroups && M >= 1 && M < (1ll << 30));
  for (int i = 0; i < ngroups; ++i) {
    const os2s_wgrad_group_t& s = groups[i];
    OS2S_REQUIRE(s.x && s.dy && s.dw && s.Cin >= 128 && s.Cout >= 128 && s.Cin % 8 == 0 && s.Cout % 8 == 0);
    OS2S_REQUIRE(s.x_row_stride >= s.Cin && s.x_row_stride % 8 == 0);
    OS2S_REQUIRE(s.x_row_stride * 2 * 64 < (1ll << 30) && (long long)s.Cout * 2 * 64 < (1ll << 30));
  }
  const WgradGroupTable gt = wgrad_group_table(groups, ngroups, 256, 1);
  const os2s_wgrad_group_t& g0 = groups[0];
  WgradArgs a = wgrad_args(g0.x, g0.x_row_stride, g0.dy, g0.dw, nullptr, 1, (int)M, g0.Cin, g0.Cout, accumulate);
  a.NCO = gt.total_units; a.NCI = 1;
  return launch_wgrad1x1_pp((hipStream_t)stream, a, gt, gt.total_units, workspace, workspace_bytes);
}
```

openseq2seq_amd/csrc/optimizer.hip:

```cpp
#include "os2s_common.hpp"

namespace os2s {

constexpr int kChunk = 4096;

struct OptDeviceState {
  long long global_step;
  long long scaler_iteration;
  long long last_overflow_iteration;
  long long num_skipped;
  float loss_scale;
  float lr;
  float global_grad_norm;
  float grad_amax;
  int has_nan;
  int skip;
  float x_hat, slow_x_hat, xsquared_hat, b1_correction, b2_correction;
  float grad_scale_latched;
};

}

using namespace os2s;

namespace os2s {

__device__ float lr_policy_value(const os2s_opt_config_t& c, long long step) {
  float lr = c.learning_rate;
  const float fs = (float)step;
  switch (c.lr_policy) {
    case 1: {
      if (c.warmup_steps > 0 && step < c.warmup_steps) lr = lr * fs / (float)c.warmup_steps;
      if (step < c.begin_decay_at) return lr;
      long long s = step - c.begin_decay_at;
      if (s > c.decay_steps) s = c.decay_steps;
      const float frac = 1.f - (float)s / (float)c.decay_steps;
      return (lr - c.min_lr) * powf(frac, c.power) + c.min_lr;
    }
    case 2: {
      if (step >= c.begin_decay_at) {
        float p = (float)(step - c.begin_decay_at) / (float)c.decay_steps;
        if (c.use_staircase_decay) p = floorf(p);
        lr = lr * powf(c.decay_rate, p);
      }
      return fmaxf(c.min_lr, lr);
    }
    case 3: {
      const float ws = (float)c.warmup_steps;
      const float decay = c.coefficient * powf((float)c.d_model, -0.5f) *
                          fminf((fs + 1.f) * powf(ws, -1.5f), powf(fs + 1.f, -0.5f));
      const float nl = decay * lr;
      return c.has_max_lr ? fminf(c.max_lr, nl) : nl;
    }
    case 4: {
      if (c.warmup_steps > 0 && step < c.warmup_steps) lr = lr * fs / (float)c.warmup_steps;
      if (step < c.begin_decay_at) return lr;
      long long s = step - c.begin_decay_at;
      if (s > c.decay_steps) s = c.decay_steps;
      const float cosd = 0.5f * (1.f + cosf(3.14159265358979323846f * (float)s / (float)c.decay_steps));
      return lr * ((1.f - c.min_lr) * cosd + c.min_lr);
    }
    case 5: {
      int i = 0;
      while (i < c.pw_count && step > c.pw_boundaries[i]) ++i;
      return lr * c.pw_rates[i];
    }
    case 6: {
      const float mn = fminf(fmaxf(c.min_lr, 1e-8f), lr);
      const float scale = (powf(lr / mn, 1.f / c.power) - 1.f) / (float)c.decay_steps;
      return lr / powf(1.f + scale * fs, c.power);
    }
    default:
      return lr;
  }
}

template <bool NEED_W>
__global__ __launch_bounds__(256) void mt_grad_stats_kernel(
    const float* __restrict__ grads, const float* __restrict__ weights,
    const int32_t* __restrict__ chunk_tensor, const float* __restrict__ tensor_l2,
    const OptDeviceState* __restrict__ st, int world_size, float* __restrict__ partial) {
  __shared__ float red[4][4];
  const int c = blockIdx.x;
  const int ti = chunk_tensor[c];
  const float inv = 1.f / (st->grad_scale_latched * (float)world_size);
  const float l2 = tensor_l2 ? tensor_l2[ti] : 0.f;
  const f32x4* g4 = reinterpret_cast<const f32x4*>(grads + (long long)c * kChunk);
  const f32x4* w4 = reinterpret_cast<const f32x4*>(weights + (long long)c * kChunk);
  float sg = 0.f, sw = 0.f, mx = 0.f, nan = 0.f;
#pragma unroll
  for (int i = 0; i < kChunk / 4 / 256; ++i) {
    const f32x4 g = g4[i * 256 + threadIdx.x];
    f32x4 w = {0.f, 0.f, 0.f, 0.f};
    if (NEED_W) w = w4[i * 256 + threadIdx.x];
#pragma unroll
    for (int e = 0; e < 4; ++e) {
      const float ge = NEED_W ? g[e] * inv + l2 * w[e] : g[e] * inv;
      sg += ge * ge;
      sw += w[e] * w[e];
      mx = fmaxf(mx, fabsf(ge));
      nan = (ge != ge) ? 1.f : nan;
    }
  }
  sg = wave_sum(sg); sw = wave_sum(sw); mx = wave_max(mx); nan = wave_max(nan);
  const int lane = threadIdx.x & 63, wid = threadIdx.x >> 6;
  if (lane == 0) { red[wid][0] = sg; red[wid][1] = sw; red[wid][2] = mx; red[wid][3] = nan; }
  __syncthreads();
  if (threadIdx.x == 0) {
    float a = 0.f, b = 0.f, m = 0.f, n = 0.f;
    for (int w = 0; w < 4; ++w) { a += red[w][0]; b += red[w][1]; m = fmaxf(m, red[w][2]); n = fmaxf(n, red[w][3]); }
    partial[c * 4 + 0] = a; partial[c * 4 + 1] = b; partial[c * 4 + 2] = m; partial[c * 4 + 3] = n;
  }
}

__global__ __launch_bounds__(256) void mt_tensor_reduce_kernel(
    const float* __restrict__ partial, const int32_t* __restrict__ tensor_chunk_begin,
    float* __restrict__ tensor_gnorm2, float* __restrict__ tensor_wnorm2,
    float* __restrict__ tensor_amax, float* __restrict__ tensor_nan) {
  __shared__ double sh_g[4], sh_w[4];
  __shared__ float sh_m[4], sh_n[4];
  const int t = blockIdx.x;
  const int c0 = tensor_chunk_begin[t], c1 = tensor_chunk_begin[t + 1];
  double g2 = 0.0, w2 = 0.0;
  float mx = 0.f, nn = 0.f;
  for (int c = c0 + threadIdx.x; c < c1; c += 256) {
    const f32x4 v = *reinterpret_cast<const f32x4*>(partial + (long long)c * 4);
    g2 += (double)v[0];
    w2 += (double)v[1];
    mx = fmaxf(mx, v[2]);
    nn = fmaxf(nn, v[3]);
  }
#pragma unroll
  for (int o = 32; o > 0; o >>= 1) {
    g2 += __shfl_xor(g2, o, 64);
    w2 += __shfl_xor(w2, o, 64);
  }
  mx = wave_max(mx);
  nn = wave_max(nn);
  const int lane = threadIdx.x & 63, wid = threadIdx.x >> 6;
  if (lane == 0) { sh_g[wid] = g2; sh_w[wid] = w2; sh_m[wid] = mx; sh_n[wid] = nn; }
  __syncthreads();
  if (threadIdx.x == 0) {
    g2 = (sh_g[0] + sh_g[1]) + (sh_g[2] + sh_g[3]);
    w2 = (sh_w[0] + sh_w[1]) + (sh_w[2] + sh_w[3]);
    mx = fmaxf(fmaxf(sh_m[0], sh_m[1]), fmaxf(sh_m[2], sh_m[3]));
    nn = fmaxf(fmaxf(sh_n[0], sh_n[1]), fmaxf(sh_n[2], sh_n[3]));
    tensor_gnorm2[t] = (float)g2;
    tensor_wnorm2[t] = (float)w2;
    tensor_amax[t] = mx;
    tensor_nan[t] = (nn > 0.f || g2 != g2) ? 1.f : 0.f;
  }
}

__global__ __launch_bounds__(256) void mt_finalize_kernel(
    int ntensors, os2s_opt_config_t cfg, OptDeviceState* __restrict__ st,
    float* __restrict__ tensor_gnorm2, float* __restrict__ tensor_wnorm2,
    float* __restrict__ tensor_amax, float* __restrict__ tensor_mult ,
    float* __restrict__ tensor_v ) {
  __shared__ float sh_f[256];
  __shared__ float sh_m[256];
  __shared__ int sh_nan;
  __shared__ float s_gn, s_amax;
  if (threadIdx.x == 0) sh_nan = 0;
  __syncthreads();
  float tot = 0.f;
  int anynan = 0;
  for (int t = threadIdx.x; t < ntensors; t += 256) {
    tot += tensor_gnorm2[t];
    if (tensor_mult[t] > 0.f) anynan = 1;
  }
  if (anynan) atomicOr(&sh_nan, 1);
  sh_f[threadIdx.x] = tot;
  __syncthreads();
  if (threadIdx.x == 0) {
    double s = 0.0;
    for (int i = 0; i < 256; ++i) s += (double)sh_f[i];
    s_gn = (float)sqrt(s);
  }
  __syncthreads();
  const float gnorm = s_gn;
  if (threadIdx.x == 0 && cfg.clip_global_norm > 0.f && !(gnorm == gnorm)) sh_nan = 1;
  const long long step = st->global_step;
  const float lr = lr_policy_value(cfg, step);
  float clip_scale = 1.f;
  if (cfg.clip_global_norm > 0.f)
    clip_scale = cfg.clip_global_norm * fminf(1.f / gnorm, 1.f / cfg.clip_global_norm);
  float amax = 0.f;
  for (int t = threadIdx.x; t < ntensors; t += 256) {
    float f = clip_scale;
    if (cfg.use_larc) {
      const float vn = sqrtf(tensor_wnorm2[t]);
      const float gn = sqrtf(tensor_gnorm2[t]) * clip_scale;
      float u;
      if (!cfg.larc_mode_scale) {
        u = fmaxf(cfg.larc_eta * vn / (lr * (gn + cfg.larc_epsilon)), cfg.larc_min_update);
        u = fminf(u, 1.f);
      } else {
        u = fmaxf(cfg.larc_eta * vn / (gn + cfg.larc_epsilon), cfg.larc_min_update);
      }
      f *= u;
    }
    tensor_mult[t] = f;
    const float am = tensor_amax[t] * f;
    amax = fmaxf(amax, am);
    if (!(f == f) || !(am == am)) atomicOr(&sh_nan, 1);
  }
  sh_m[threadIdx.x] = amax;
  __syncthreads();
  if (threadIdx.x == 0) {
    float m = 0.f;
    for (int i = 0; i < 256; ++i) m = fmaxf(m, sh_m[i]);
    s_amax = m;
    const int has_nan = sh_nan;
    const bool overflow = has_nan || isinf(m);
    st->has_nan = has_nan;
    st->grad_amax = m;
    st->global_grad_norm = gnorm;
    st->lr = lr;
    int skip = 0;
    if (cfg.scaler == 1) {
      skip = overflow;
      float sc = st->loss_scale;
      if (overflow) {
        sc = fminf(fmaxf(sc / cfg.step_factor, cfg.scale_min), cfg.scale_max);
        st->last_overflow_iteration = st->scaler_iteration;
      } else {
        const long long since = st->scaler_iteration - st->last_overflow_iteration;
        if (since % cfg.step_window == 0)
          sc = fminf(fmaxf(sc * cfg.step_factor, cfg.scale_min), cfg.scale_max);
      }
      st->loss_scale = sc;
      st->scaler_iteration += 1;
    } else if (cfg.scaler == 2) {
      skip = overflow;
      const float x = overflow ? powf(2.f, cfg.log_max) : (logf(m) / logf(2.f));
      st->x_hat = cfg.lm_beta1 * st->x_hat + (1.f - cfg.lm_beta1) * x;
      st->b1_correction *= cfg.lm_beta1;
      const float mu = st->x_hat / (1.f - st->b1_correction);
      st->slow_x_hat = cfg.lm_beta2 * st->slow_x_hat + (1.f - cfg.lm_beta2) * x;
      st->xsquared_hat = cfg.lm_beta2 * st->xsquared_hat + (1.f - cfg.lm_beta2) * (x * x);
      st->b2_correction *= cfg.lm_beta2;
      const float e_x2 = st->xsquared_hat / (1.f - st->b2_correction);
      const float slow_mu = st->slow_x_hat / (1.f - st->b2_correction);
      const float sigma = sqrtf(fmaxf(e_x2 - slow_mu * slow_mu, 0.f));
      const float log_cutoff = sigma * cfg.overflow_std_dev + mu;
      const float proposed = powf(2.f, 16.f - log_cutoff);
      st->loss_scale = fminf(fmaxf(proposed, cfg.scale_min), cfg.scale_max);
      st->scaler_iteration += 1;
    }
    st->skip = skip;
    if (skip) st->num_skipped += 1;
  }
  __syncthreads();
  if (st->skip) return;
  if (cfg.optimizer == 2) {
    for (int t = threadIdx.x; t < ntensors; t += 256) {
      const float f = tensor_mult[t];
      const float g2 = tensor_gnorm2[t] * f * f;
      float v = tensor_v[t];
      v = (v == 0.f || !cfg.novograd_ema) ? g2 : (v * cfg.beta2 + g2 * (1.f - cfg.beta2));
      tensor_v[t] = v;
      tensor_mult[t] = f / sqrtf(v + cfg.epsilon);
    }
  }
  if (threadIdx.x == 0) st->global_step = step + 1;
}

template <int OPT>
__global__ __launch_bounds__(256) void mt_apply_kernel(
    float* __restrict__ grads, float* __restrict__ weights, float* __restrict__ m1,
    float* __restrict__ m2, bf16_t* __restrict__ w16, const int32_t* __restrict__ chunk_tensor,
    const float* __restrict__ tensor_l2, const float* __restrict__ tensor_mult,
    const float* __restrict__ tensor_wd_mask, os2s_opt_config_t cfg,
    const OptDeviceState* __restrict__ st, int chunk0, int zero_grads) {
  constexpr int N = kChunk / 4 / 256;
  const int c = blockIdx.x + chunk0;
  if (st->skip) {
    if (zero_grads) {
      const long long b0 = (long long)c * kChunk + (long long)threadIdx.x * 4;
#pragma unroll
      for (int i = 0; i < N; ++i) *reinterpret_cast<f32x4*>(grads + b0 + (long long)i * 1024) = f32x4{0.f, 0.f, 0.f, 0.f};
    }
    return;
  }
  const int ti = chunk_tensor[c];
  const float inv = 1.f / (st->grad_scale_latched * (float)cfg.world_size);
  const float l2 = tensor_l2 ? tensor_l2[ti] : 0.f;
  const float mult = tensor_mult[ti];
  const float lr = st->lr;
  const float wd = cfg.weight_decay * (tensor_wd_mask ? tensor_wd_mask[ti] : 1.f);
  const float ga = cfg.grad_averaging ? (1.f - cfg.beta1) : 1.f;
  float adam_lr = lr;
  if (OPT == 3) {
    const float t = (float)(st->global_step);
    adam_lr = lr * sqrtf(1.f - powf(cfg.beta2, t)) / (1.f - powf(cfg.beta1, t));
  }
  const long long base = (long long)c * kChunk + (long long)threadIdx.x * 4;
  f32x4 g[N], w[N], m[N], v[N];
#pragma unroll
  for (int i = 0; i < N; ++i) {
    const long long off = base + (long long)i * 1024;
    g[i] = __builtin_nontemporal_load(reinterpret_cast<const f32x4*>(grads + off));
    w[i] = *reinterpret_cast<const f32x4*>(weights + off);
    if (OPT != 0) m[i] = *reinterpret_cast<const f32x4*>(m1 + off);
    if (OPT == 3) v[i] = *reinterpret_cast<const f32x4*>(m2 + off);
  }
#pragma unroll
  for (int i = 0; i < N; ++i) {
    const long long off = base + (long long)i * 1024;
#pragma unroll
    for (int e = 0; e < 4; ++e) {
      float ge = (g[i][e] * inv + l2 * w[i][e]) * mult;
      if (OPT == 0) {
        w[i][e] -= lr * ge;
      } else if (OPT == 1) {
        m[i][e] = cfg.beta1 * m[i][e] + ge;
        w[i][e] -= lr * m[i][e];
      } else if (OPT == 2) {
        ge += wd * w[i][e];
        ge *= ga;
        m[i][e] = cfg.beta1 * m[i][e] + ge;
        w[i][e] -= lr * m[i][e];
      } else {
        m[i][e] = cfg.beta1 * m[i][e] + (1.f - cfg.beta1) * ge;
        v[i][e] = cfg.beta2 * v[i][e] + (1.f - cfg.beta2) * ge * ge;
        w[i][e] -= adam_lr * m[i][e] / (sqrtf(v[i][e]) + cfg.epsilon);
      }
    }
    *reinterpret_cast<f32x4*>(weights + off) = w[i];
    if (zero_grads) *reinterpret_cast<f32x4*>(grads + off) = f32x4{0.f, 0.f, 0.f, 0.f};
    if (OPT != 0) *reinterpret_cast<f32x4*>(m1 + off) = m[i];
    if (OPT == 3) *reinterpret_cast<f32x4*>(m2 + off) = v[i];
    if (w16) {
      u32x2 o;
      o[0] = pack2bf(w[i][0], w[i][1]);
      o[1] = pack2bf(w[i][2], w[i][3]);
      __builtin_nontemporal_store(o, reinterpret_cast<u32x2*>(w16 + off));
    }
  }
}

__global__ void opt_latch_scale_kernel(OptDeviceState* st) { st->grad_scale_latched = st->loss_scale; }

__global__ void opt_init_state_kernel(OptDeviceState* st, float loss_scale) {
  st->global_step = 0; st->scaler_iteration = 0; st->last_overflow_iteration = -1;
  st->num_skipped = 0; st->loss_scale = loss_scale; st->lr = 0.f; st->global_grad_norm = 0.f;
  st->grad_amax = 0.f; st->has_nan = 0; st->skip = 0; st->x_hat = 0.f; st->slow_x_hat = 0.f;
  st->xsquared_hat = 0.f; st->b1_correction = 1.f; st->b2_correction = 1.f; st->grad_scale_latched = loss_scale;
}

__global__ __launch_bounds__(256) void cast_f32_bf16_kernel(const float* __restrict__ src,
                                                            bf16_t* __restrict__ dst,
                                                            long long n4) {
  for (long long i = (long long)blockIdx.x * 256 + threadIdx.x; i < n4;
       i += (long long)gridDim.x * 256) {
    const f32x4 v = reinterpret_cast<const f32x4*>(src)[i];
    u32x2 o;
    o[0] = pack2bf(v[0], v[1]);
    o[1] = pack2bf(v[2], v[3]);
    reinterpret_cast<u32x2*>(dst)[i] = o;
  }
}

struct WtDesc { long long src_off, dst_off; int K, Cout, Cin, tile_begin; };

__global__ __launch_bounds__(256) void conv_weight_dgrad_copy_kernel(
    const bf16_t* __restrict__ w16, bf16_t* __restrict__ wt16, const WtDesc* __restrict__ descs,
    int ndesc) {
  __shared__ bf16_t tile[64][66];
  const int tileid = blockIdx.x;
  int lo = 0, hi = ndesc - 1;
  while (lo < hi) {
    const int mid = (lo + hi + 1) >> 1;
    if (descs[mid].tile_begin <= tileid) lo = mid; else hi = mid - 1;
  }
  const WtDesc d = descs[lo];
  const int local = tileid - d.tile_begin;
  const int tco = (d.Cout + 63) / 64, tci = (d.Cin + 63) / 64;
  const int k = local / (tco * tci);
  const int r = local - k * (tco * tci);
  const int co0 = (r / tci) * 64, ci0 = (r % tci) * 64;
  const bf16_t* src = w16 + d.src_off + (long long)k * d.Cout * d.Cin;
  bf16_t* dst = wt16 + d.dst_off + (long long)(d.K - 1 - k) * d.Cin * d.Cout;
  const bool vec = (d.Cin % 8 == 0) && (d.Cout % 8 == 0) && ((((uintptr_t)src) | ((uintptr_t)dst)) % 16 == 0);
  if (vec) {
#pragma unroll
    for (int it = 0; it < 2; ++it) {
      const int piece = it * 256 + threadIdx.x;
      const int a = piece >> 3, b8 = piece & 7;
      const int co = co0 + a, ci = ci0 + b8 * 8;
      u32x4 v = {0u, 0u, 0u, 0u};
      if (co < d.Cout && ci < d.Cin) v = *reinterpret_cast<const u32x4*>(src + (long long)co * d.Cin + ci);
      uint32_t* t32 = reinterpret_cast<uint32_t*>(&tile[a][b8 * 8]);
      t32[0] = v[0]; t32[1] = v[1]; t32[2] = v[2]; t32[3] = v[3];
    }
    __syncthreads();
#pragma unroll
    for (int it = 0; it < 2; ++it) {
      const int piece = it * 256 + threadIdx.x;
      const int a = piece >> 3, b8 = piece & 7;
      const int ci = ci0 + a, co = co0 + b8 * 8;
      if (ci < d.Cin && co < d.Cout) {
        u32x4 v;
#pragma unroll
        for (int e = 0; e < 4; ++e)
          v[e] = (uint32_t)tile[b8 * 8 + 2 * e][a] | ((uint32_t)tile[b8 * 8 + 2 * e + 1][a] << 16);
        *reinterpret_cast<u32x4*>(dst + (long long)ci * d.Cout + co) = v;
      }
    }
    return;
  }
  for (int i = threadIdx.x; i < 64 * 64; i += 256) {
    const int a = i >> 6, b = i & 63;
    const int co = co0 + a, ci = ci0 + b;
    tile[a][b] = (co < d.Cout && ci < d.Cin) ? src[(long long)co * d.Cin + ci] : (bf16_t)0;
  }
  __syncthreads();
  for (int i = threadIdx.x; i < 64 * 64; i += 256) {
    const int a = i >> 6, b = i & 63;
    const int ci = ci0 + a, co = co0 + b;
    if (co < d.Cout && ci < d.Cin) dst[(long long)ci * d.Cout + co] = tile[b][a];
  }
}

}

extern "C" int os2s_opt_chunk_elems(void) { return kChunk; }
extern "C" size_t os2s_opt_state_bytes(void) { return sizeof(OptDeviceState); }
extern "C" size_t os2s_opt_config_bytes(void) { return sizeof(os2s_opt_config_t); }

extern "C" int os2s_opt_init_state(os2s_stream_t stream, void* state, float loss_scale) {
  OS2S_REQUIRE(state);
  OS2S_LAUNCH(opt_init_state_kernel, dim3(1), dim3(1), 0, (hipStream_t)stream,
              (OptDeviceState*)state, loss_scale);
  return OS2S_OK;
}

extern "C" int os2s_opt_prepare(os2s_stream_t stream_, const os2s_opt_config_t* cfg, void* state,
                                const float* grads, const float* weights, int nchunks, int ntensors,
                                const int32_t* chunk_tensor, const int32_t* tensor_chunk_begin,
                                const float* tensor_l2, float* partial, float* tensor_gnorm2, float* tensor_wnorm2,
                                float* tensor_amax, float* tensor_mult, float* tensor_v) {
  OS2S_REQUIRE(cfg && state && grads && weights && chunk_tensor && tensor_chunk_begin);
  OS2S_REQUIRE(partial && tensor_gnorm2 && tensor_wnorm2 && tensor_amax && tensor_mult);
  OS2S_REQUIRE(nchunks >= 1 && ntensors >= 1 && cfg->world_size >= 1);
  if (cfg->optimizer == 2) OS2S_REQUIRE(tensor_v);
  hipStream_t stream = (hipStream_t)stream_;
  OptDeviceState* st = (OptDeviceState*)state;
  OS2S_LAUNCH(opt_latch_scale_kernel, dim3(1), dim3(1), 0, stream, st);
  if (tensor_l2 != nullptr || cfg->use_larc) {
    OS2S_LAUNCH(mt_grad_stats_kernel<true>, dim3(nchunks), dim3(256), 0, stream, grads, weights,
                chunk_tensor, tensor_l2, st, cfg->world_size, partial);
  } else {
    OS2S_LAUNCH(mt_grad_stats_kernel<false>, dim3(nchunks), dim3(256), 0, stream, grads, weights,
                chunk_tensor, tensor_l2, st, cfg->world_size, partial);
  }
  OS2S_LAUNCH(mt_tensor_reduce_kernel, dim3(ntensors), dim3(256), 0, stream, partial,
              tensor_chunk_begin, tensor_gnorm2, tensor_wnorm2, tensor_amax, tensor_mult);
  OS2S_LAUNCH(mt_finalize_kernel, dim3(1), dim3(256), 0, stream, ntensors, *cfg, st,
              tensor_gnorm2, tensor_wnorm2, tensor_amax, tensor_mult, tensor_v);
  return OS2S_OK;
}

extern "C" int os2s_opt_apply_range(os2s_stream_t stream_, const os2s_opt_config_t* cfg, const void* state,
                                    float* grads, float* weights, float* m1, float* m2, uint16_t* w16,
                                    int chunk_begin, int chunk_end, const int32_t* chunk_tensor,
                                    const float* tensor_l2, const float* tensor_mult,
                                    const float* tensor_wd_mask, int zero_grads) {
  OS2S_REQUIRE(cfg && state && grads && weights && chunk_tensor && tensor_mult);
  OS2S_REQUIRE(chunk_begin >= 0 && chunk_end >= chunk_begin);
  if (cfg->optimizer != 0) OS2S_REQUIRE(m1);
  if (cfg->optimizer == 3) OS2S_REQUIRE(m2);
  if (chunk_end == chunk_begin) return OS2S_OK;
  hipStream_t stream = (hipStream_t)stream_;
  const OptDeviceState* st = (const OptDeviceState*)state;
  const int n = chunk_end - chunk_begin;
#define OS2S_APPLY(OPT)                                                                    \
  OS2S_LAUNCH(mt_apply_kernel<OPT>, dim3(n), dim3(256), 0, stream, grads, weights, m1, m2, \
              w16, chunk_tensor, tensor_l2, tensor_mult, tensor_wd_mask, *cfg, st, chunk_begin, zero_grads ? 1 : 0)
  switch (cfg->optimizer) {
    case 0: OS2S_APPLY(0); break;
    case 1: OS2S_APPLY(1); break;
    case 2: OS2S_APPLY(2); break;
    default: OS2S_APPLY(3); break;
  }
#undef OS2S_APPLY
  return OS2S_OK;
}

extern "C" int os2s_opt_step(os2s_stream_t stream_, const os2s_opt_config_t* cfg, void* state,
                             const float* grads, float* weights, float* m1, float* m2,
                             uint16_t* w16, int nchunks, int ntensors,
                             const int32_t* chunk_tensor, const int32_t* tensor_chunk_begin,
                             const float* tensor_l2, const float* tensor_wd_mask,
                             float* partial, float* tensor_gnorm2, float* tensor_wnorm2,
                             float* tensor_amax, float* tensor_mult, float* tensor_v) {
  OS2S_REQUIRE(cfg);
  if (cfg->optimizer != 0) OS2S_REQUIRE(m1);
  if (cfg->optimizer == 3) OS2S_REQUIRE(m2);
  const int rc = os2s_opt_prepare(stream_, cfg, state, grads, weights, nchunks, ntensors, chunk_tensor,
                                  tensor_chunk_begin, tensor_l2, partial, tensor_gnorm2, tensor_wnorm2, tensor_amax,
                                  tensor_mult, tensor_v);
  if (rc != OS2S_OK) return rc;
  return os2s_opt_apply_range(stream_, cfg, state, const_cast<float*>(grads), weights, m1, m2, w16, 0, nchunks,
                              chunk_tensor, tensor_l2, tensor_mult, tensor_wd_mask, 0);
}

extern "C" int os2s_cast_f32_to_bf16(os2s_stream_t stream, const float* src, uint16_t* dst,
                                     long long n) {
  OS2S_REQUIRE(src && dst && n >= 0 && n % 4 == 0);
  if (n == 0) return OS2S_OK;
  long long blocks = (n / 4 + 255) / 256;
  if (blocks > 4096) blocks = 4096;
  OS2S_LAUNCH(cast_f32_bf16_kernel, dim3((int)blocks), dim3(256), 0, (hipStream_t)stream, src,
              dst, n / 4);
  return OS2S_OK;
}

extern "C" int os2s_conv_weight_dgrad_copy(os2s_stream_t stream, const uint16_t* w16,
                                           uint16_t* wt16, const void* descs, int ndesc,
                                           int total_tiles) {
  OS2S_REQUIRE(w16 && wt16 && descs && ndesc >= 1 && total_tiles >= 1);
  static_assert(sizeof(WtDesc) == 32, "descriptor layout");
  OS2S_LAUNCH(conv_weight_dgrad_copy_kernel, dim3(total_tiles), dim3(256), 0,
              (hipStream_t)stream, w16, wt16, (const WtDesc*)descs, ndesc);
  return OS2S_OK;
}
```

openseq2seq_amd/models/model.py:

```python
from __future__ import absolute_import, division, print_function

import abc
import os
import copy
import time

import six
import torch

from .. import capi
from ..optimizers.flat_params import FlatParams
from ..optimizers.optimizers import optimize_loss
from ..parts.streams import set_side_stream_enabled
from ..parts.tape import Tape
from ..utils import distributed as dist_utils
from ..utils.utils import check_params

ASYNC_OPTIMIZER = os.environ.get("OS2S_ASYNC_OPT", "0") == "1"
DEFER_TAPE_FREE = os.environ.get("OS2S_DEFER_TAPE_FREE", "1") != "0"


def resolve_lr_params(lr_policy, lr_policy_params, last_step, steps_in_epoch, has_num_epochs):
  import inspect
  lr_params = dict(lr_policy_params)
# ... 49 lines not shown
        'os2s_async_optimizer': bool,
    }

  def __init__(self, params, mode="train", hvd=None, device=None):
    check_params(params, self.get_required_params(), self.get_optional_params())
    self._params = copy.deepcopy(params)
    if self._params.get('iter_size', 1) > 1 and not self._params['use_horovod']:
      raise ValueError("iter_size is only supported in Horovod mode")
    if mode not in ['train', 'infer', 'eval', 'interactive_infer']:
      raise ValueError("Mode has to be one of ['train', 'infer', 'eval', 'interactive_infer']")
    if 'max_steps' in params and 'num_epochs' in params and mode == "train":
      raise ValueError("You can't provide both max_steps and num_epochs. "
                       "Please, remove one of them from the config.")
    self._mode = mode
    self._hvd = hvd
    p = self._params
    self._towers = 1
    if not p['use_horovod']:
      self._towers = dist_utils.configured_towers(p)
      world = hvd.size() if hvd is not None else 1
      if self._towers != world and mode in ("train", "eval"):
        raise ValueError(
            "config asks for %d replicas (use_horovod False, num_gpus/gpu_ids) but this process "
            "group has %d rank(s): launch through run.py (it starts the ranks itself) or "
            "`python -m torch.distributed.run --nproc-per-node %d`" % (self._towers, world,
                                                                      self._towers))
    p.setdefault('dtype', 'mixed')
    p.setdefault('iter_size', 1)
    p.setdefault('loss_scaling', 1.0)
    self._device = device or torch.device("cuda", torch.cuda.current_device())
    rs = p.get('random_seed', int(time.time()))
    rank = hvd.rank() if hvd is not None else 0
    self._seed = rs + rank
    torch.manual_seed(rs)
    self._step_count = 0
    self._store = None
    self._train_op = None
    self._compiled = False
    self._data_layer = None

  @property
  def params(self):
    return self._params

  @property
  def mode(self):
    return self._mode

  @property
  def hvd(self):
    return self._hvd

  @property
  def on_horovod(self):
    return self._hvd is not None

  def get_data_layer(self, worker_id=0):
    return self._data_layer

  @property
  def num_gpus(self):
    return self._towers

  @property
  def store(self):
    return self._store

  @property
  def train_op(self):
    return self._train_op

  def compile(self, force_var_reuse=False, checkpoint=None):
    self._store = FlatParams(self._device)
    self._build_forward_pass_objects(self._store)
    need_m2 = False
    if self._mode == "train":
      from ..optimizers.optimizers import needs_second_moments
      need_m2 = needs_second_moments(self._params['optimizer'])
    self._store.finalize(need_m2=need_m2)
    world = self._hvd.size() if self._hvd is not None else 1
    if self._hvd is not None and world > 1:
      dist_utils.broadcast_parameters(self._store, self._extra_state_tensors())
    if self._mode == "train":
      p = self._params
      if 'lr_policy' not in p:
        raise ValueError("lr_policy has to be specified for train mode")
      lr_params = resolve_lr_params(p['lr_policy'], p.get('lr_policy_params', {}), self._last_step,
                                    lambda: self.steps_in_epoch, 'num_epochs' in p)
      self._train_op = optimize_loss(
          self._store, p['optimizer'], p.get('optimizer_params', {}), p['lr_policy'],
          lr_params, dtype=p['dtype'], clip_gradients=p.get('max_grad_norm', None),
          summaries=p.get('summaries', None), larc_params=p.get('larc_params', None),
          loss_scaling=p.get('loss_scaling', 1.0),
          loss_scaling_params=p.get('loss_scaling_params', None),
          on_horovod=self.on_horovod, iter_size=p.get('iter_size', 1), world_size=world)
      force = self._hvd is not None and os.environ.get("OS2S_FORCE_REDUCER", "") == "1"
      self._reducer = dist_utils.GradientReducer(self._store, world) if (world > 1 or force) else None
    self._compiled = True
    return self

  def _last_step(self, default=100000):
    p = self._params
    if 'max_steps' in p:
      return p['max_steps']
    if 'num_epochs' in p and self._data_layer is not None:
      try:
        n = self._data_layer.get_size_in_samples()
        world = self._hvd.size() if self._hvd is not None else 1
        spe = n // (p['batch_size_per_gpu'] * world * p.get('iter_size', 1))
        return max(spe * p['num_epochs'], 1)
      except Exception:
        pass
    return default

  @property
  def steps_in_epoch(self):
    p = self._params
    if self._data_layer is None:
      return None
    try:
      n = self._data_layer.get_size_in_samples()
    except Exception:
      return None
    world = self._hvd.size() if self._hvd is not None else 1
    return n // (p['batch_size_per_gpu'] * world * p.get('iter_size', 1))

  @property
  def last_step(self):
    return self._last_step()

  def _extra_state_tensors(self):
    return list(self._store.state.values()) if self._store is not None else []

  @abc.abstractmethod
  def _build_forward_pass_objects(self, store):
    """Create data layer + encoder/decoder/loss objects and their variables."""

  @abc.abstractmethod
  def _forward_backward(self, batch, tape):
    """Run forward (and record backward) for one batch; returns the loss tensor [1]."""

  @abc.abstractmethod
  def _get_num_objects_per_step(self, batch):
    pass

  def train_step(self, batch):
    assert self._compiled and self._mode == "train"
    p = self._params
    prev = set_side_stream_enabled(p.get('os2s_side_stream', True))
    try:
      iter_size = p.get('iter_size', 1)
      micro = self._step_count % iter_size
      if micro == 0:
        if self._store.grads_zeroed:
          self._store.grads_zeroed = False
        else:
          self._store.zero_grads()
      last_micro = (micro == iter_size - 1)
      overlap = self._reducer is not None and last_micro
      snap = None
      if self._gru_guard:
        snap = ([t.clone() for t in self._extra_state_tensors()],
                self._store.grads.clone() if micro > 0 else None)
      launches0 = capi.gru_xcd_launch_count()
      tape = None
      if getattr(self, "_halves_enabled", None) is not None and self._halves_enabled():
        loss = self._forward_backward_halves(batch)
      else:
        tape = Tape(on_done=self._reducer.mark_done if overlap else None)
        tape.defer_free = DEFER_TAPE_FREE
        loss = self._forward_backward(batch, tape)
        tape.backward()
      ran_persistent = capi.gru_xcd_launch_count() != launches0
      world = self._hvd.size() if self._hvd is not None else 1
      if self._gru_agree is None:
        self._gru_agree = world > 1 and self._has_gru_layers()
      if ran_persistent or (world > 1 and self._gru_agree):
        self._gru_guard = ran_persistent
        loss = self._recover_gru_abort(batch, loss, snap, micro, overlap, ran_persistent)
      self._step_count += 1
      if last_micro:
        if self._reducer is not None:
          self._reducer.finish()
        if p.get('os2s_async_optimizer', ASYNC_OPTIMIZER):
          self._train_op.run_async()
        else:
          self._train_op.run()
      if tape is not None:
        tape.ops = []
    finally:
      set_side_stream_enabled(prev)
    return loss

  def _has_gru_layers(self):
    for part in (getattr(self, "_encoder", None), getattr(self, "_decoder", None)):
      params = getattr(part, "params", None) or {}
      if "gru" in str(params.get("rnn_type", "")).lower():
        return True
    return False

  _gru_guard = False
  _gru_agree = None

  def _recover_gru_abort(self, batch, loss, snap, micro, overlap, ran_persistent=True):
    code = 0
    if ran_persistent:
      torch.cuda.current_stream().synchronize()
      code = capi.gru_xcd_status(clear=True)
    world = self._hvd.size() if self._hvd is not None else 1
    if world > 1:
      t = torch.tensor([code, int(ran_persistent)], dtype=torch.int32, device=self._device)
      torch.distributed.all_reduce(t, op=torch.distributed.ReduceOp.MAX)
      code, anyone = int(t[0].item()), int(t[1].item())
      self._gru_agree = bool(anyone) and code == 0
    if code == 0:
      return loss
    self._gru_guard = False
    import warnings
    warnings.warn("a persistent GRU launch gave up (code %d: 1 = poll timeout, 2 = workgroup placement); the step "
                  "is redone on the launch-per-step kernels, which stay selected for this process" % code)
    capi.gru_xcd_set_mode(0)
    if self._reducer is not None:
      if overlap:
        self._reducer.finish()
      self._reducer.reset()
    if snap is not None:
      for t, s0 in zip(self._extra_state_tensors(), snap[0]):
        t.copy_(s0)
    if micro == 0:
      self._store.zero_grads()
    elif snap is not None and snap[1] is not None:
      self._store.grads.copy_(snap[1])
    else:
      raise RuntimeError("persistent GRU abort inside an accumulation window before a snapshot existed")
    tape = Tape(on_done=self._reducer.mark_done if overlap else None)
    loss = self._forward_backward(batch, tape)
    tape.backward()
    torch.cuda.current_stream().synchronize()
    assert capi.gru_xcd_status(clear=True) == 0
    return loss

  def copy_weights_from(self, other):
    assert self._store.total == other._store.total
    self._store.master.copy_(other._store.master)
    self._store.refresh_compute_copies()
    for mine, theirs in zip(self._extra_state_tensors(), other._extra_state_tensors()):
      mine.copy_(theirs)

  def global_step(self):
    return self._train_op.read_state()["global_step"]
```

openseq2seq_amd/optimizers/flat_params.py:

```python
import struct

import numpy as np
import os

import torch

from .. import capi


def _guarded(slot, wt=False):
  def get(self):
    st = self.store
    if st is not None and (st._pending or st._wt_event is not None):
      st._ready(self, wt)
    return getattr(self, slot)

  def put(self, value):
    setattr(self, slot, value)
  return property(get, put)


class Param(object):
  __slots__ = ("name", "shape", "index", "offset", "numel", "l2", "kind", "store",
               "_master", "_grad", "_w16", "_wt16", "wt_offset", "trainable_mask", "logical_out", "logical_in")
  master = _guarded("_master")
  grad = _guarded("_grad")
  w16 = _guarded("_w16")
  wt16 = _guarded("_wt16", wt=True)

  def __init__(self, name, shape, kind, l2, logical_out=None):
    self.name, self.shape, self.kind, self.l2 = name, tuple(int(s) for s in shape), kind, l2
    self.numel = int(np.prod(self.shape))
    self.logical_out = logical_out
    self.logical_in = None
    self.store = None
    self._master = self._grad = self._w16 = self._wt16 = None


def _whole(slot):
  def get(self):
    if self._pending or self._wt_event is not None:
      self.wait_all()
    return getattr(self, slot)

  def put(self, value):
    setattr(self, slot, value)
  return property(get, put)


class FlatParams(object):

  master = _whole("_master")
  grads = _whole("_grads")
  m1 = _whole("_m1")
  m2 = _whole("_m2")
  w16 = _whole("_w16")
  wt16 = _whole("_wt16")
  t_v = _whole("_t_v")

  def __init__(self, device):
    self.device = device
    self._pending, self._wt_event, self._main_stream, self._opt_stream = [], None, None, None
    self._done_upto = 0
    self.grads_zeroed = False
    self._master = self._grads = self._m1 = self._m2 = self._w16 = self._wt16 = self._t_v = None
    self.params = []
    self.state = {}
    self._inits = []
    self.finalized = False
    self.chunk = capi.opt_chunk_elems()

  def add(self, name, shape, init, kind="dense", l2=0.0, logical_out=None):
    assert not self.finalized
    for p in self.params:
      if p.name == name:
        raise ValueError("duplicate variable " + name)
    p = Param(name, shape, kind, float(l2), logical_out)
    p.index = len(self.params)
    p.store = self
    self.params.append(p)
    self._inits.append(init)
    return p

  def add_state(self, name, tensor):
    if name in self.state:
      raise ValueError("duplicate state variable " + name)
    self.state[name] = tensor
    return tensor

  def finalize(self, need_m2=False):
    dev, ch = self.device, self.chunk
    off = 0
    wt_off = 0
    begins = []
    for p in self.params:
      p.offset = off
      begins.append(off // ch)
      off += -(-p.numel // ch) * ch
      if p.kind == "conv":
        p.wt_offset = wt_off
        wt_off += -(-p.numel // 8) * 8
    self.total = off
    begins.append(off // ch)
    self.master = torch.zeros(off, dtype=torch.float32, device=dev)
    self.grads = torch.zeros(off, dtype=torch.float32, device=dev)
    self.m1 = torch.zeros(off, dtype=torch.float32, device=dev)
    self.m2 = torch.zeros(off, dtype=torch.float32, device=dev) if need_m2 else None
    self.w16 = torch.zeros(off, dtype=torch.bfloat16, device=dev)
    self.wt16 = torch.zeros(max(wt_off, 8), dtype=torch.bfloat16, device=dev)
    nt = len(self.params)
    chunk_tensor = np.zeros(off // ch, np.int32)
    for i, p in enumerate(self.params):
      chunk_tensor[begins[i]:begins[i + 1]] = i
    self.chunk_tensor = torch.from_numpy(chunk_tensor).to(dev)
    self.tensor_chunk_begin = torch.tensor(begins, dtype=torch.int32, device=dev)
    self.tensor_l2 = torch.tensor([p.l2 for p in self.params], dtype=torch.float32, device=dev)
    self.l2_active = any(float(p.l2) != 0.0 for p in self.params)
    self.partial = torch.zeros(off // ch * 4, dtype=torch.float32, device=dev)
    self.t_gnorm2 = torch.zeros(nt, dtype=torch.float32, device=dev)
    self.t_wnorm2 = torch.zeros(nt, dtype=torch.float32, device=dev)
    self.t_amax = torch.zeros(nt, dtype=torch.float32, device=dev)
    self.t_mult = torch.zeros(nt, dtype=torch.float32, device=dev)
    self.t_v = torch.zeros(nt, dtype=torch.float32, device=dev)
    descs = b""
    tiles = 0
    for p, init in zip(self.params, self._inits):
      sl = slice(p.offset, p.offset + p.numel)
      p.master = self.master[sl].view(p.shape)
      p.grad = self.grads[sl].view(p.shape)
      p.w16 = self.w16[sl].view(p.shape)
      val = init(p.shape) if callable(init) else init
      p.master.copy_(torch.as_tensor(val, dtype=torch.float32).reshape(p.shape))
      if p.kind == "conv":
        K, Cout, Cin = p.shape
        p.wt16 = self.wt16[p.wt_offset:p.wt_offset + p.numel].view(K, Cin, Cout)
        descs += struct.pack("<qqiiii", p.offset, p.wt_offset, K, Cout, Cin, tiles)
        tiles += K * (-(-Cout // 64)) * (-(-Cin // 64))
    self._wt_tiles = tiles
    self._wt_descs = (torch.frombuffer(bytearray(descs), dtype=torch.uint8).to(dev)
                      if tiles else None)
    self._n_wt = len(descs) // 32
    self._inits = None
    self.finalized = True
    self.refresh_compute_copies()
    return self

  def refresh_compute_copies(self):
    capi.cast_f32_to_bf16(self.master, self.w16)
    self.refresh_dgrad_copies()

  def refresh_dgrad_copies(self):
    self.version = getattr(self, "version", 0) + 1
    self._refresh_dgrad_copies_raw()

  def _refresh_dgrad_copies_raw(self):
    if self._wt_tiles:
      capi.conv_weight_dgrad_copy(self._w16, self._wt16, self._wt_descs.view(-1, 32),
                                  self._wt_tiles)

  def zero_grads(self):
    self.grads.zero_()

  def _streams(self):
    cur = torch.cuda.current_stream()
    return (cur,) if self._main_stream is None or cur == self._main_stream else (cur, self._main_stream)

  def _ready(self, p, wt=False):
    if wt:
      if self._wt_event is not None:
        for st in self._streams():
          st.wait_event(self._wt_event)
        self._wt_event = None
        self._pending = []
      return
    pend = self._pending
    end = p.offset + p.numel
    if not pend or end <= self._done_upto:
      return
    i, n = 0, len(pend)
    while i < n - 1 and pend[i][0] < end:
      i += 1
    for st in self._streams():
      st.wait_event(pend[i][1])
    self._done_upto = pend[i][0]
    del pend[:i + 1]

  def wait_all(self):
    ev = self._wt_event if self._wt_event is not None else (self._pending[-1][1] if self._pending else None)
    if ev is not None:
      for st in self._streams():
        st.wait_event(ev)
    self._pending, self._wt_event = [], None
    self._done_upto = 0

  def opt_stream(self):
    if self._opt_stream is None:
      self._opt_stream = torch.cuda.Stream(device=self.device)
    return self._opt_stream

  def num_trainable(self):
    return sum(p.numel for p in self.params)

  def by_name(self, name):
    for p in self.params:
      if p.name == name:
        return p
    raise KeyError(name)
```

openseq2seq_amd/optimizers/optimizers.py:

```python
import six

import torch

from .. import capi
from ..utils.utils import check_params
from . import lr_policies
from .automatic_loss_scaler import AutomaticLossScaler
from .novograd import NovoGrad

OPTIMIZER_CLS_NAMES = {"Adagrad": None, "Adam": 3, "Ftrl": None, "Momentum": 1,
                       "RMSProp": None, "SGD": 0, "AdamW": None, "NovoGrad": 2,
                       "LazyAdam": 3}

OPTIMIZER_SUMMARIES = ["learning_rate", "gradients", "gradient_norm", "global_gradient_norm",
                       "variables", "variable_norm", "larc_summaries", "loss_scale"]


def _optimizer_id(optimizer):
  if isinstance(optimizer, six.string_types):
    if optimizer not in OPTIMIZER_CLS_NAMES:
      raise ValueError("Optimizer name should be one of [{}], you provided {}.".format(
          ", ".join(OPTIMIZER_CLS_NAMES), optimizer))
    oid = OPTIMIZER_CLS_NAMES[optimizer]
  else:
    name = getattr(optimizer, "__name__", type(optimizer).__name__)
    name = {"LazyAdamOptimizer": "LazyAdam", "AdamOptimizer": "Adam",
            "MomentumOptimizer": "Momentum", "GradientDescentOptimizer": "SGD"}.get(name, name)
    oid = OPTIMIZER_CLS_NAMES.get(name)
  if oid is None:
    raise NotImplementedError("optimizer %r has no HIP implementation yet" % (optimizer,))
  return oid


def needs_second_moments(optimizer):
  return _optimizer_id(optimizer) == 3


def build_opt_config(optimizer, optimizer_params, learning_rate_decay_fn,
                     lr_policy_params, larc_params=None, loss_scaling=1.0,
                     loss_scaling_params=None, clip_gradients=None, dtype="mixed",
                     world_size=1):
  if clip_gradients is not None and larc_params is not None:
    raise AttributeError("LARC and gradient norm clipping should not be used together")
  cfg = capi.OptConfig()
  oid = _optimizer_id(optimizer)
  op = dict(optimizer_params or {})
  cfg.optimizer = oid
  if oid == 2:
    d = dict(NovoGrad.DEFAULTS, **op)
    cfg.beta1, cfg.beta2, cfg.epsilon = d["beta1"], d["beta2"], d["epsilon"]
    cfg.weight_decay, cfg.grad_averaging = d["weight_decay"], int(bool(d["grad_averaging"]))
    cfg.novograd_ema = int(bool(d["ema_second_moment"]))
  elif oid == 1:
    cfg.beta1 = op.get("momentum", 0.9)
  elif oid == 3:
    cfg.beta1, cfg.beta2 = op.get("beta1", 0.9), op.get("beta2", 0.999)
    cfg.epsilon = op.get("epsilon", 1e-8)
  for k, v in lr_policies.device_policy(learning_rate_decay_fn, lr_policy_params).items():
    if isinstance(v, list):
      arr = getattr(cfg, k)
      for i, e in enumerate(v):
        arr[i] = e
    else:
      setattr(cfg, k, v)
  if larc_params is not None:
    check_params(larc_params, {'larc_eta': float},
                 {'larc_mode': ['clip', 'scale'], 'min_update': float, 'epsilon': float})
    cfg.use_larc = 1
    cfg.larc_eta = larc_params['larc_eta']
    cfg.larc_mode_scale = int(larc_params.get('larc_mode', 'clip') == 'scale')
    cfg.larc_min_update = larc_params.get('min_update', 1e-7)
    cfg.larc_epsilon = larc_params.get('epsilon', 1e-7)
  cfg.clip_global_norm = float(clip_gradients) if clip_gradients is not None else 0.0
  initial_scale = 1.0
  cfg.scaler = 0
  cfg.scale_min, cfg.scale_max, cfg.step_factor, cfg.step_window = 1.0, 2. ** 14, 2.0, 2000
  cfg.log_max, cfg.lm_beta1, cfg.lm_beta2, cfg.overflow_std_dev = 16., 0.99, 0.999, 3.09
  if dtype == "mixed":
    if isinstance(loss_scaling, six.string_types):
      als = AutomaticLossScaler(algorithm=loss_scaling, params=loss_scaling_params)
      cfg.scaler = als.scaler_id
      for k, v in als.cfg.items():
        setattr(cfg, k, v)
      initial_scale = als.initial_scale
    else:
      initial_scale = float(loss_scaling)
  cfg.world_size = int(world_size)
  return cfg, float(initial_scale)


class TrainOp(object):

  def __init__(self, store, cfg, initial_scale):
    self.store, self.cfg = store, cfg
    self.state = torch.zeros(capi.opt_state_bytes(), dtype=torch.uint8, device=store.device)
    capi.opt_init_state(self.state, initial_scale)
    self.loss_scale_view = self.state[32:36].view(torch.float32)
    self.lr_view = self.state[36:40].view(torch.float32)

  def run(self):
    s = self.store
    capi.opt_step(self.cfg, self.state, s.grads, s.master, s.m1, s.m2, s.w16,
                  s.chunk_tensor, s.tensor_chunk_begin, s.tensor_l2 if s.l2_active else None, None, s.partial,
                  s.t_gnorm2, s.t_wnorm2, s.t_amax, s.t_mult, s.t_v)
    s.refresh_dgrad_copies()

  def run_async(self, nranges=8):
    s = self.store
    s.wait_all()
    main = torch.cuda.current_stream()
    side = s.opt_stream()
    side.wait_stream(main)
    nchunks = s.chunk_tensor.numel()
    nranges = max(1, min(int(nranges), nchunks))
    bounds = [(nchunks * i) // nranges for i in range(nranges + 1)]
    pending = []
    with torch.cuda.stream(side):
      capi.opt_prepare(self.cfg, self.state, s._grads, s._master, s.chunk_tensor, s.tensor_chunk_begin,
                       s.tensor_l2 if s.l2_active else None, s.partial, s.t_gnorm2, s.t_wnorm2, s.t_amax,
                       s.t_mult, s._t_v)
      for c0, c1 in zip(bounds[:-1], bounds[1:]):
        capi.opt_apply_range(self.cfg, self.state, s._grads, s._master, s._m1, s._m2, s._w16, c0, c1,
                             s.chunk_tensor, s.tensor_l2 if s.l2_active else None, s.t_mult, zero_grads=True)
        ev = torch.cuda.Event()
        ev.record(side)
        pending.append((c1 * s.chunk, ev))
      s.version = getattr(s, "version", 0) + 1
      s._refresh_dgrad_copies_raw()
      evw = torch.cuda.Event()
      evw.record(side)
    s._pending, s._wt_event, s._main_stream, s._done_upto = pending, evw, main, 0
    s.grads_zeroed = True

  def read_state(self):
    self.store.wait_all()
    return capi.opt_read_state(self.state)


def optimize_loss(store, optimizer, optimizer_params, learning_rate_decay_fn,
                  lr_policy_params=None, dtype="mixed", clip_gradients=None, summaries=None,
                  larc_params=None, loss_scaling=1.0, loss_scaling_params=None,
                  on_horovod=False, iter_size=1, world_size=1):
  if summaries is not None:
    for summ in summaries:
      if summ not in OPTIMIZER_SUMMARIES:
        raise ValueError("Summaries should be one of [{}], you provided {}.".format(
            ", ".join(OPTIMIZER_SUMMARIES), summ))
  cfg, scale = build_opt_config(optimizer, optimizer_params, learning_rate_decay_fn,
                                lr_policy_params or {}, larc_params, loss_scaling,
                                loss_scaling_params, clip_gradients, dtype, world_size)
  if iter_size > 1 and not on_horovod:
    raise ValueError("iter_size is only supported in Horovod mode")
  cfg.world_size = int(world_size) * int(iter_size)
  if cfg.optimizer == 3 and store.m2 is None:
    raise ValueError("Adam needs FlatParams.finalize(need_m2=True)")
  return TrainOp(store, cfg, scale)
```

openseq2seq_amd/parts/cnns/conv_blocks.py:

```python
import math
import os

import torch

from ... import capi
from .. import streams, tape as _tape
from ..activations import act_id
from ..streams import join_side_streams, on_side_stream, set_side_stream_enabled, side_streams
from ..tape import Act, Tape, accumulate_grad, backward_interleaved, current_tape, reshape_act


FUSE_BN_BWD = os.environ.get("OS2S_FUSE_BN_BWD", "1") != "0"
GROUP_WGRAD = os.environ.get("OS2S_GROUP_WGRAD", "1") != "0"
GROUP_POINTWISE_WGRAD = os.environ.get("OS2S_GROUP_POINTWISE_WGRAD", "1") != "0"
POINTWISE_WGRAD_GROUP = int(os.environ.get("OS2S_POINTWISE_WGRAD_GROUP", "5"))
GROUP_WGRAD_PP = os.environ.get("OS2S_GROUP_WGRAD_PP", "1") != "0"
DRES_FWD_SIDE = os.environ.get("OS2S_DRES_FWD_SIDE", "1") != "0"
WGRAD_STREAMS = int(os.environ.get("OS2S_WGRAD_STREAMS", "1"))
_WGRAD_RR = 0
DRES_FUSE_BN_BWD = os.environ.get("OS2S_DRES_FUSE_BN_BWD", "1") != "0"
SEP_FUSE_BN_BWD = os.environ.get("OS2S_SEP_FUSE_BN_BWD", "1") != "0"
FOLD_SEP_K1 = os.environ.get("OS2S_FOLD_SEP_K1", "1") != "0"


def xavier_normal_conv(shape_dev):
  K, Cout, Cin = shape_dev
  std = math.sqrt(1.3 * 2.0 / (K * Cin + K * Cout))
  w = torch.empty(shape_dev)
  torch.nn.init.trunc_normal_(w, 0.0, std, -2 * std, 2 * std)
  return w


def glorot_uniform_conv(shape_dev):
  K, Cout, Cin = shape_dev
  lim = math.sqrt(6.0 / (K * Cin + K * Cout))
  return (torch.rand(shape_dev) * 2 - 1) * lim


class ConvBN(object):

  def __init__(self, store, name, bn_name, cin, cout, k, stride=1, dilation=1,
               padding="SAME", bn_momentum=0.9, bn_epsilon=1e-3, l2=0.0,
               initializer=xavier_normal_conv):
    self._set_geometry(name, cin, cout, k, stride, dilation, padding)
    self.momentum, self.eps = bn_momentum, bn_epsilon
    self.kernel = store.add(name + "/kernel", (k, cout, cin), initializer, kind="conv", l2=l2)
    self._add_bn(store, bn_name, cout, l2)

  def _set_geometry(self, name, cin, cout, k, stride, dilation, padding):
    self.name, self.cin, self.cout, self.k = name, cin, cout, k
    self.stride, self.dil, self.padding = stride, dilation, padding

  def _add_bn(self, store, bn_name, cout, l2):
    self.gamma = store.add(bn_name + "/gamma", (cout,), torch.ones(cout), kind="vector", l2=l2)
    self.beta = store.add(bn_name + "/beta", (cout,), torch.zeros(cout), kind="vector")
    dev = store.device
    self.moving_mean = torch.zeros(cout, dtype=torch.float32, device=dev)
    self.moving_var = torch.ones(cout, dtype=torch.float32, device=dev)
    if hasattr(store, "add_state"):
      store.add_state(bn_name + "/moving_mean", self.moving_mean)
      store.add_state(bn_name + "/moving_variance", self.moving_var)

  def out_geometry(self, tin):
    if self.padding == "SAME":
      return capi.same_padding(tin, self.k, self.stride, self.dil)
    return capi.valid_padding(tin, self.k, self.stride, self.dil)

  def conv_bn_stats(self, x, training):
    B, Tin, _ = x.data.shape
    tout, pl = self.out_geometry(Tin)
    dev = x.data.device
    C = self.cout
    stats = None
    if training:
      stats = torch.empty((capi.conv1d_num_mtiles(B, tout), 2, C), dtype=torch.float32,
                          device=dev)
    y = capi.conv1d_fwd(x.data, self.kernel.w16, stride=self.stride, dil=self.dil,
                        pad_left=pl, tout=tout, in_len=x.lens, stats=stats)
    return self.bn_from_stats(y, stats, B, tout, training, pl)

  def bn_outputs(self, y, training, tout, pl=0):
    sc, sh, mean, rstd = bn_vectors(self.cout, y.device, training)
    return dict(y=y, scale=sc, shift=sh, mean=mean, rstd=rstd, tout=tout, pad_left=pl)

  def bn_from_stats(self, y, stats, B, tout, training, pl=0):
    d = self.bn_outputs(y, training, tout, pl)
    capi.bn_finalize(stats, B * tout, self.gamma.master, self.beta.master, self.eps,
                     self.momentum, training, self.moving_mean, self.moving_var, d["mean"], d["rstd"],
                     d["scale"], d["shift"])
    return d

  def trainable(self):
    return [self.kernel, self.gamma, self.beta]

  def backward_weights(self, inp, dy, f):
    x = inp.data
    tape = current_tape()
    units = ((self.cout + 127) // 128) * ((self.cin + 127) // 128) * ((self.k + 3) // 4)
    if _tape.CONV_WGRAD_UNIT_BUDGET > 0 and tape is not None and self.stride == 1 and self.k >= 2 and \
       units < _tape.CONV_WGRAD_UNIT_BUDGET and x.dim() == 3 and x.shape[0] <= 64 and self.cout >= 128 and self.cin >= 64 and \
       dy.is_contiguous() and x.stride(2) == 1 and x.stride(0) == x.shape[1] * x.stride(1):
      key = (tuple(x.shape), tuple(dy.shape), x.stride(1), self.k, self.dil, f["pad_left"],
             None if inp.lens is None else inp.lens.data_ptr())
      tape.defer_conv_wgrad(self.kernel, key, dict(x=x, dy=dy, dw=self.kernel.grad), units,
                            dict(K=self.k, stride=1, dil=self.dil, pad_left=f["pad_left"], in_len=inp.lens))
      return
    global _WGRAD_RR
    _WGRAD_RR += 1
    with on_side_stream(dy.device, inp.data, dy, which=0 if WGRAD_STREAMS < 2 else (0, 2)[_WGRAD_RR & 1]):
      capi.conv1d_wgrad(inp.data, dy, self.k, stride=self.stride, dil=self.dil,
                        pad_left=f["pad_left"], in_len=inp.lens, out=self.kernel.grad,
                        accumulate=True)

  def backward_branch(self, inp, dy, f, final=False):
    self.backward_weights(inp, dy, f)
    self.backward_data(inp, dy, f, final, self.kernel.wt16)

  def backward_data(self, inp, dy, f, final, wt16):
    if inp.requires_grad:
      g = inp.grad_buffer()
      tin = inp.data.shape[1]
      pl = (self.k - 1) * self.dil - f["pad_left"]
      if self.stride != 1:
        dy = capi.upsample_rows(dy.contiguous(), self.stride, (dy.shape[1] - 1) * self.stride + 1)
        capi.conv1d_fwd(dy, wt16, dil=self.dil, pad_left=pl, tout=tin, out=g,
                        accumulate=inp.grad_init, out_len=inp.lens)
        inp.grad_init = True
        return
      if final and FUSE_BN_BWD and inp.bn_y is not None and not inp.bn_full_rows and dy.is_contiguous() and \
         g.is_contiguous():
        inp.bias_part = capi.conv1d_dgrad_bnact(dy, wt16, g, dil=self.dil, pad_left=pl,
                                                accumulate=inp.grad_init, out_len=inp.lens,
                                                mask_ref=inp.data, mask_scale=inp.bn_scale, stat_ref=inp.bn_y)
        inp.grad_init = True
        inp.grad_masked = True
        return
      capi.conv1d_fwd(dy, wt16, dil=self.dil, pad_left=pl, tout=tin, out=g,
                      accumulate=inp.grad_init, out_len=inp.lens)
      inp.grad_init = True


def bn_vectors(C, dev, training):
  if not training:
    sc, sh = torch.empty((2, C), dtype=torch.float32, device=dev).unbind(0)
    return sc, sh, None, None
  return torch.empty((4, C), dtype=torch.float32, device=dev).unbind(0)


class SepConvBN(ConvBN):

  def __init__(self, store, name, bn_name, cin, cout, k, stride=1, dilation=1,
               padding="SAME", bn_momentum=0.9, bn_epsilon=1e-3, l2=0.0,
               initializer=xavier_normal_conv):
    self._set_geometry(name, cin, cout, k, stride, dilation, padding)
    self.momentum, self.eps = bn_momentum, bn_epsilon

    def dw_init(shape):
      return initializer((shape[0], 1, shape[1]))[:, 0, :] if shape[0] * shape[1] > 0 else torch.zeros(shape)

    self.depthwise = store.add(name + "/depthwise_kernel", (k, cin), dw_init, kind="vector", l2=l2)
    self.kernel = store.add(name + "/pointwise_kernel", (1, cout, cin), initializer, kind="conv", l2=l2)
    self._add_bn(store, bn_name, cout, l2)

  def conv_bn_stats(self, x, training):
    B, Tin, _ = x.data.shape
    tout, pl = self.out_geometry(Tin)
    dev = x.data.device
    C = self.cout
    stats = None
    if training:
      stats = torch.empty((capi.conv1d_num_mtiles(B, tout), 2, C), dtype=torch.float32, device=dev)
    wt_eff = None
    if self.folded():
      if getattr(self, "_fold_bufs", None) is None:
        self._fold_bufs = (torch.empty((1, C, self.cin), dtype=torch.bfloat16, device=dev),
                           torch.empty((1, self.cin, C), dtype=torch.bfloat16, device=dev))
      w_eff, wt_eff = capi.pointwise_fold(self.kernel.master, self.depthwise.master, out=self._fold_bufs)
      z = None
      y = capi.conv1d_fwd(x.data, w_eff, pad_left=0, tout=tout, in_len=x.lens, stats=stats)
    else:
      z = capi.depthwise_conv1d_fwd(x.data, self.depthwise.master, stride=self.stride, dil=self.dil,
                                    pad_left=pl, tout=tout, in_len=x.lens)
      y = capi.conv1d_fwd(z, self.kernel.w16, pad_left=0, tout=tout, stats=stats)
    sc, sh, mean, rstd = bn_vectors(C, dev, training)
    capi.bn_finalize(stats, B * tout, self.gamma.master, self.beta.master, self.eps,
                     self.momentum, training, self.moving_mean, self.moving_var, mean, rstd,
                     sc, sh)
    return dict(y=y, scale=sc, shift=sh, mean=mean, rstd=rstd, tout=tout, pad_left=pl,
                z=z if training else None, wt_eff=wt_eff if training else None)

  def folded(self):
    return FOLD_SEP_K1 and self.k == 1 and self.stride == 1 and self.cin % 8 == 0 and self.cout % 8 == 0

  def trainable(self):
    return [self.depthwise, self.kernel, self.gamma, self.beta]

  def backward_branch(self, inp, dy, f, final=False):
    if f.get("wt_eff") is not None:
      x = inp.data
      rows = x.shape[0] * x.shape[1]
      gw = capi.zero_scratch(self.kernel.grad.shape, dy.device)

      def split(gw=gw):
        capi.pointwise_fold_bwd(gw, self.kernel.master, self.depthwise.master, self.kernel.grad, self.depthwise.grad)
      if GROUP_POINTWISE_WGRAD and current_tape() is not None and self.cin >= 128 and self.cout >= 128 and \
         rows >= 2048 and x.is_contiguous() and dy.is_contiguous():
        current_tape().defer_wgrad(self.kernel, dict(x=x.view(rows, self.cin), dy=dy.view(rows, self.cout),
                                                     dw=gw.view(self.cout, self.cin), after=split,
                                                     also=(self.depthwise,)),
                                   group=POINTWISE_WGRAD_GROUP)
      else:
        with on_side_stream(dy.device, x, dy, gw):
          capi.conv1d_wgrad(x, dy, 1, pad_left=0, in_len=inp.lens, out=gw, accumulate=True)
          split()
      wt_eff, f["wt_eff"] = f["wt_eff"], None
      self.backward_data(inp, dy, f, final, wt_eff)
      return
    z = f["z"]
    rows = z.shape[0] * z.shape[1]
    units = ((self.cout + 255) // 256) * ((self.cin + 255) // 256)
    if GROUP_POINTWISE_WGRAD and current_tape() is not None and units < 32 and self.cin >= 128 and \
       self.cout >= 128 and rows >= 2048 and self.cin % 8 == 0 and self.cout % 8 == 0 and \
       z.is_contiguous() and dy.is_contiguous():
      current_tape().defer_wgrad(self.kernel, dict(x=z.view(rows, self.cin), dy=dy.view(rows, self.cout),
                                                   dw=self.kernel.grad.view(self.cout, self.cin)),
                                 group=POINTWISE_WGRAD_GROUP)
    else:
      with on_side_stream(dy.device, z, dy):
        capi.conv1d_wgrad(z, dy, 1, pad_left=0, out=self.kernel.grad, accumulate=True)
    dz = capi.conv1d_fwd(dy, self.kernel.wt16, pad_left=0, tout=z.shape[1])
    f["z"] = None
    with on_side_stream(dy.device, inp.data, dz):
      capi.depthwise_conv1d_wgrad(inp.data, dz, self.depthwise.grad, stride=self.stride, dil=self.dil,
                                  pad_left=f["pad_left"], in_len=inp.lens)
    if inp.requires_grad:
      if final and FUSE_BN_BWD and SEP_FUSE_BN_BWD and inp.bn_y is not None and dz.is_contiguous() and \
         capi.depthwise_dgrad_bnact_supported(self.k, self.stride, self.dil) and \
         (inp.grad is None or not inp.grad_init or inp.grad.is_contiguous()):
        inp.wait_grad()
        prev = inp.grad if inp.grad_init else None
        out = prev if prev is not None else torch.empty_like(inp.data)
        inp.bias_part = capi.depthwise_dgrad_bnact(dz, self.depthwise.master, out, pad_left=(self.k - 1) - f["pad_left"],
                                                   out_len=inp.lens, mask_ref=inp.data, mask_scale=inp.bn_scale,
                                                   stat_ref=inp.bn_y, addend=prev)
        inp.grad, inp.grad_init, inp.grad_masked = out, True, True
        return
      if self.stride != 1:
        dz = capi.upsample_rows(dz.contiguous(), self.stride, (dz.shape[1] - 1) * self.stride + 1)
      tin = inp.data.shape[1]
      dx = capi.depthwise_conv1d_fwd(dz, self.depthwise.master, dil=self.dil,
                                     pad_left=(self.k - 1) * self.dil - f["pad_left"], tout=tin,
                                     out_len=inp.lens, flip=True)
      accumulate_grad(inp, dx)


class DepthwiseBN(ConvBN):

  def __init__(self, store, name, channels, k, bn_momentum=0.99, bn_epsilon=1e-3, l2=0.0):
    self._set_geometry(name, channels, channels, k, 1, 1, "SAME")
    self.momentum, self.eps = bn_momentum, bn_epsilon

    def init(shape):
      lim = math.sqrt(6.0 / (shape[0] * shape[1] + shape[0]))
      return (torch.rand(shape) * 2 - 1) * lim

    self.depthwise = store.add(name + "/w", (k, channels), init, kind="vector", l2=l2)
    self._add_bn(store, name + "/bn", channels, l2)

  def conv_bn_stats(self, x, training):
    B, Tin, C = x.data.shape
    tout, pl = self.out_geometry(Tin)
    dev = x.data.device
    y = capi.depthwise_conv1d_fwd(x.data, self.depthwise.master, stride=1, dil=1, pad_left=pl,
                                  tout=tout, in_len=x.lens)
    stats = capi.bn_stats(y.view(B * tout, C)) if training else None
    sc, sh, mean, rstd = bn_vectors(C, dev, training)
    capi.bn_finalize(stats, B * tout, self.gamma.master, self.beta.master, self.eps,
                     self.momentum, training, self.moving_mean, self.moving_var, mean, rstd, sc, sh)
    return dict(y=y, scale=sc, shift=sh, mean=mean, rstd=rstd, tout=tout, pad_left=pl)

  def trainable(self):
    return [self.depthwise, self.gamma, self.beta]

  def backward_branch(self, inp, dy, f):
    capi.depthwise_conv1d_wgrad(inp.data, dy, self.depthwise.grad, stride=1, dil=1,
                                pad_left=f["pad_left"], in_len=inp.lens)
    if inp.requires_grad:
      tin = inp.data.shape[1]
      dx = capi.depthwise_conv1d_fwd(dy, self.depthwise.master, dil=1,
                                     pad_left=(self.k - 1) - f["pad_left"], tout=tin,
                                     out_len=inp.lens, flip=True)
      accumulate_grad(inp, dx)


def _bn_act_backward_head(result, dout, out, branches, fw, rows, lens, act, keep_prob, seed, c1, c2):
  if result.grad_masked:
    partial, result.bias_part = result.bias_part, None
    capi.bn_bwd_finalize_raw(partial, rows, fw[0]["mean"], fw[0]["rstd"], branches[0].gamma.grad,
                             branches[0].beta.grad, True, c1[0], c2[0])
    return dout, lens is not None
  dz = torch.empty_like(out)
  partial = torch.empty((capi.bn_act_bwd_num_parts(rows), 1 + len(branches), out.shape[2]), dtype=torch.float32,
                        device=out.device)
  capi.bn_act_bwd_reduce(dout, out, [f["y"] for f in fw], [f["mean"] for f in fw],
                         [f["rstd"] for f in fw], dz, partial, lens, act, keep_prob, seed)
  capi.bn_bwd_finalize_multi(partial, rows, [br.gamma.grad for br in branches],
                             [br.beta.grad for br in branches], True, c1, c2)
  return dz, False


def conv_bn_res_bn_actv(main, res_branches, x, res_inputs, out_lens, activation_fn,
                        training, tape, keep_prob=1.0, seed=0, mask_output=True,
                        drop_block_prob=0.0, drop_block=False, res_fw=None):
  act = act_id(activation_fn)
  branches = [main] + list(res_branches)
  inputs = [x] + list(res_inputs)
  fw_main = main.conv_bn_stats(x, training)
  if res_fw is not None:
    streams.join_side_streams()
    global _FWD_SIDE_BUSY
    _FWD_SIDE_BUSY = False
    fw = [fw_main] + res_fw
  else:
    fw = [fw_main] + grouped_conv1x1_bn_stats(res_branches, res_inputs, training)
  dropped = False
  if res_branches and drop_block_prob > 0:
    if training:
      import random
      dropped = random.Random(int(seed) * 2654435761 % (2 ** 31)).random() < drop_block_prob
    else:
      dropped = bool(drop_block)
  if dropped:
    tout0 = fw[0]["tout"]
    branches, inputs, fw = branches[1:], inputs[1:], fw[1:]
    fw[0]["tout"] = tout0
  B = x.data.shape[0]
  tout, C = fw[0]["tout"], main.cout
  out = torch.empty((B, tout, C), dtype=torch.bfloat16, device=x.data.device)
  lens = out_lens if mask_output else None
  capi.bn_act_fwd([f["y"] for f in fw], [f["scale"] for f in fw], [f["shift"] for f in fw],
                  out, lens, act, keep_prob if training else 1.0, seed)
  result = Act(out, out_lens if mask_output else None)
  if not (training and tape is not None):
    return result
  if FUSE_BN_BWD and len(fw) == 1 and act == 1 and (type(main) is ConvBN or (SEP_FUSE_BN_BWD and type(main) is SepConvBN)) \
     and not dropped and (lens is None or main.stride == 1):
    result.bn_y = fw[0]["y"]
    result.bn_scale = 1.0 / (keep_prob if training else 1.0)
    result.bn_full_rows = type(main) is not ConvBN

  def backward():
    result.wait_grad()
    dout = result.grad
    if dout is None and drop_block_prob > 0:
      return
    assert dout is not None, "no gradient reached " + main.name
    rows = B * tout
    J = len(branches)
    c1 = torch.empty((J, C), dtype=torch.float32, device=out.device)
    c2 = torch.empty((J, C), dtype=torch.float32, device=out.device)
    dz, dz_to_len = _bn_act_backward_head(result, dout, out, branches, fw, rows, lens, act, keep_prob, seed, c1, c2)
    result.grad = None
    grouped = []
    wgrouped = []
    plain = [j for j in range(1, len(branches)) if _is_plain_1x1(branches[j])]
    can_group = len(branches) > 2 and len(plain) >= 2 and \
        len({tuple(inputs[j].data.shape[:2]) for j in plain}) == 1 and \
        len({id(inputs[j].lens) for j in plain}) == 1
    for j, (br, inp, f) in enumerate(zip(branches, inputs, fw)):
      dy = torch.empty_like(f["y"])
      ragged = lens is not None and type(br) is ConvBN and br.stride == 1
      capi.bn_bwd_apply(dz, f["y"], br.gamma.master, f["mean"], f["rstd"], c1[j], c2[j], dy,
                        out_len=lens if ragged else None, margin=(br.k - 1) * br.dil,
                        dz_to_len=dz_to_len and ragged)
      f["y"] = None
      if can_group and j in plain:
        if GROUP_WGRAD:
          wgrouped.append((br, inp, dy))
        else:
          br.backward_weights(inp, dy, f)
        if inp.requires_grad:
          grouped.append((br, inp, dy))
      elif j == 0 and br is main and type(br) in (ConvBN, SepConvBN):
        br.backward_branch(inp, dy, f, final=all(r is not inp for r in inputs[1:]))
      else:
        br.backward_branch(inp, dy, f)
    if wgrouped:
      with on_side_stream(dz.device, *([w[1].data for w in wgrouped] + [w[2] for w in wgrouped])):
        for i0 in range(0, len(wgrouped), 16):
          capi.conv1x1_wgrad_grouped([dict(x=inp.data, dy=dy, dw=br.kernel.grad)
                                      for br, inp, dy in wgrouped[i0:i0 + 16]], in_len=wgrouped[0][1].lens,
                                     pingpong=GROUP_WGRAD_PP)
    if grouped:
      items = []
      for br, inp, dy in grouped:
        items.append(dict(x=dy, w=br.kernel.wt16, y=inp.grad_buffer(), accumulate=inp.grad_init))
        inp.grad_init = True
      capi.conv1x1_fwd_grouped(items, out_len=grouped[0][1].lens)

  tape.record(backward, [p for br in [main] + list(res_branches) for p in br.trainable()])
  return result


def launch_dense_residual(dpass, k, x):
  if not DRES_FWD_SIDE or streams._side_stream(x.data.device, 1) is None:
    dpass.add_source(x)
    return dpass.forward_end(k)
  global _FWD_SIDE_BUSY
  _FWD_SIDE_BUSY = True
  with on_side_stream(x.data.device, x.data, which=1) as ctx:
    dpass.add_source(x)
    fw = dpass.forward_end(k)
    ctx.hand_over(fw["y"])
  return fw


def conv_bn_dres_actv(main, x, dfw, out_lens, activation_fn, training, tape, keep_prob=1.0, seed=0,
                      mask_output=True):
  act = act_id(activation_fn)
  fw = main.conv_bn_stats(x, training)
  streams.join_side_streams()
  global _FWD_SIDE_BUSY
  _FWD_SIDE_BUSY = False
  B = x.data.shape[0]
  tout, C = fw["tout"], main.cout
  out = torch.empty((B, tout, C), dtype=torch.bfloat16, device=x.data.device)
  lens = out_lens if mask_output else None
  capi.bn_act_fwd([fw["y"], dfw["y"]], [fw["scale"], dfw["scale"]], [fw["shift"], dfw["shift"]],
                  out, lens, act, keep_prob if training else 1.0, seed)
  result = Act(out, lens)
  if not (training and tape is not None):
    return result
  dpass, k = dfw["dres"], dfw["k"]
  dfw = None
  if FUSE_BN_BWD and DRES_FUSE_BN_BWD and act == 1 and type(main) is ConvBN and (lens is None or main.stride == 1):
    result.bn_y = fw["y"]
    result.bn_scale = 1.0 / (keep_prob if training else 1.0)

  def backward():
    result.wait_grad()
    dout = result.grad
    assert dout is not None, "no gradient reached " + main.name
    rows = B * tout
    c1 = torch.empty((1, C), dtype=torch.float32, device=out.device)
    c2 = torch.empty((1, C), dtype=torch.float32, device=out.device)
    dz, dz_to_len = _bn_act_backward_head(result, dout, out, [main], [fw], rows, lens, act, keep_prob, seed, c1, c2)
    result.grad = None
    src = dpass.acts[k]
    with on_side_stream(dz.device, dz, c1, which=1) as ctx:
      dpass.backward_end(k, dz, c1[0], dz_lens=lens if dz_to_len else None)
      if src.requires_grad:
        ctx.hand_over(src.grad)
        if ctx.side is not None:
          src.grad_event = torch.cuda.Event()
          src.grad_event.record(ctx.side)
    dy = torch.empty_like(fw["y"])
    ragged = lens is not None and type(main) is ConvBN and main.stride == 1
    capi.bn_bwd_apply(dz, fw["y"], main.gamma.master, fw["mean"], fw["rstd"], c1[0], c2[0], dy,
                      out_len=lens if ragged else None, margin=(main.k - 1) * main.dil,
                      dz_to_len=dz_to_len and ragged)
    fw["y"] = None
    if type(main) is ConvBN:
      main.backward_branch(x, dy, fw, final=all(x is not a for a in dpass.acts[:k + 1]))
    else:
      main.backward_branch(x, dy, fw)

  tape.record(backward, [p for br in [main] + list(dpass.plan.ends[k].branches) for p in br.trainable()])
  return result


_FWD_SIDE_BUSY = False


def forward_side_busy():
  return _FWD_SIDE_BUSY


def launch_residual_early(res_branches, res_inputs, training):
  if not res_branches or streams._side_stream(res_inputs[0].data.device) is None:
    return None
  global _FWD_SIDE_BUSY
  _FWD_SIDE_BUSY = True
  with on_side_stream(res_inputs[0].data.device, *[r.data for r in res_inputs]) as ctx:
    fw = grouped_conv1x1_bn_stats(res_branches, res_inputs, training)
    for f in fw:
      ctx.hand_over(*[v for v in f.values() if torch.is_tensor(v)])
  return fw


def _is_plain_1x1(br):
  return type(br) is ConvBN and br.k == 1 and br.stride == 1


def grouped_conv1x1_bn_stats(branches, inputs, training):
  plain = [i for i, br in enumerate(branches) if _is_plain_1x1(br)]
  if len(plain) < 2 or len({tuple(inputs[i].data.shape[:2]) for i in plain}) != 1 or \
     len({id(inputs[i].lens) for i in plain}) != 1:
    return [br.conv_bn_stats(inp, training) for br, inp in zip(branches, inputs)]
  out = [None] * len(branches)
  items = []
  for i in plain:
    br, x = branches[i], inputs[i]
    B, T, _ = x.data.shape
    dev = x.data.device
    stats = torch.empty((capi.conv1d_num_mtiles(B, T), 2, br.cout), dtype=torch.float32,
                        device=dev) if training else None
    y = torch.empty((B, T, br.cout), dtype=torch.bfloat16, device=dev)
    items.append(dict(x=x.data, w=br.kernel.w16, y=y, stats=stats))
    out[i] = (y, stats)
  capi.conv1x1_fwd_grouped(items, in_len=inputs[plain[0]].lens)
  B, T = inputs[plain[0]].data.shape[:2]
  same = len({branches[i].cout for i in plain}) == 1 and len(plain) <= 16 and \
      len({(branches[i].eps, branches[i].momentum) for i in plain}) == 1
  if same:
    fin = []
    for i in plain:
      br = branches[i]
      y, stats = out[i]
      d = br.bn_outputs(y, training, T)
      fin.append(dict(partial=stats, gamma=br.gamma.master, beta=br.beta.master, moving_mean=br.moving_mean,
                      moving_var=br.moving_var, mean_out=d["mean"], rstd_out=d["rstd"], scale_out=d["scale"],
                      shift_out=d["shift"]))
      out[i] = d
    br0 = branches[plain[0]]
    capi.bn_finalize_multi(fin, B * T, br0.eps, br0.momentum, training)
  for i, br in enumerate(branches):
    if out[i] is None:
      out[i] = br.conv_bn_stats(inputs[i], training)
    elif not same:
      y, stats = out[i]
      out[i] = br.bn_from_stats(y, stats, inputs[i].data.shape[0], inputs[i].data.shape[1], training)
  return out


class ConvOnly(ConvBN):

  def __init__(self, store, name, cin, cout, k, stride=1, dilation=1, padding="SAME", l2=0.0,
               initializer=xavier_normal_conv):
    self._set_geometry(name, cin, cout, k, stride, dilation, padding)
    self.kernel = store.add(name + "/kernel", (k, cout, cin), initializer, kind="conv", l2=l2)

# ... 61 lines not shown
```

openseq2seq_amd/parts/cnns/dense_residual.py:

```python
from __future__ import absolute_import, division, print_function

import os

import torch

from ... import capi
from .conv_blocks import ConvBN

ENABLED = os.environ.get("OS2S_DENSE_RES_ALGEBRA", "1") != "0"
GRAM_PINGPONG = os.environ.get("OS2S_DRES_GRAM_PP", "1") != "0"
P_PINGPONG = os.environ.get("OS2S_DRES_P_PP", "1") != "0"


class _End(object):
  __slots__ = ("k", "branches", "cout", "kk", "doff", "eps", "momentum", "tt", "mean", "rstd", "wp", "shift", "P",
               "coef", "table", "ptrs")


class _Source(object):
  __slots__ = ("i", "c", "koff", "wd", "gram", "s", "m", "chl", "wd1", "wd2", "wt", "mf", "mb")


class DenseResidualPlan(object):

  @staticmethod
  def eligible(ends):
    if not ENABLED or len(ends) < 2 or len(ends) > 16:
      return False
    for k, brs in enumerate(ends):
      if len(brs) != k + 1:
        return False
      for i, br in enumerate(brs):
        if type(br) is not ConvBN or br.k != 1 or br.stride != 1 or br.cin % 64 or br.cout % 64:
          return False
        if br.cout != brs[0].cout or br.eps != brs[0].eps or br.momentum != brs[0].momentum:
          return False
        if br.cin != ends[-1][i].cin:
          return False
    return True

  def __init__(self, ends, device):
    self.device = device
    self.generation = 0
    n = len(ends)
    self.n = n
    f32 = dict(dtype=torch.float32, device=device)
    b16 = dict(dtype=torch.bfloat16, device=device)
    chans = [ends[-1][i].cin for i in range(n)]
    couts = [ends[k][0].cout for k in range(n)]
    self.ktot = sum(chans)
    self.dtot = sum(couts)
    doff = [sum(couts[:k]) for k in range(n)]
    self.sources = []
    for i in range(n):
      S = _Source()
      S.i, S.c, S.koff = i, chans[i], sum(chans[:i])
      S.wd = self.dtot - doff[i]
      S.gram = torch.zeros((S.c, S.c), **f32)
      S.s = torch.zeros(S.c, **f32)
      S.m = torch.zeros(S.c, **f32)
      S.chl = torch.zeros((2 * S.c, S.c), **b16)
      S.wd1 = torch.zeros((S.c, S.wd), **b16)
      S.wd2 = torch.zeros((S.c + 8, S.wd), **b16)
      S.wt = torch.zeros((S.c, S.wd), **b16)
      S.mf = torch.zeros((S.c + 8, S.c), **f32)
      S.mb = torch.zeros((S.c, S.c), **b16)
      self.sources.append(S)
    self.ends = []
    for k in range(n):
      E = _End()
      E.k, E.branches, E.cout = k, list(ends[k]), couts[k]
      E.kk = sum(chans[:k + 1])
      E.doff = doff[k]
      E.eps, E.momentum = ends[k][0].eps, ends[k][0].momentum
      E.tt = [torch.zeros((E.cout, 2 * chans[i]), **f32) for i in range(k + 1)]
      E.mean = [torch.zeros(E.cout, **f32) for _ in range(k + 1)]
      E.rstd = [torch.ones(E.cout, **f32) for _ in range(k + 1)]
      E.wp = torch.zeros((E.cout, E.kk), **b16)
      E.shift = torch.zeros(E.cout, **f32)
      E.P = torch.zeros((E.cout, E.kk), **f32)
      E.coef = torch.zeros((k + 1) * 4 * E.cout, **f32)
      E.table, E.ptrs = None, None
      self.ends.append(E)
    self._ones = {}

  def ones(self, c):
    t = self._ones.get(c)
    if t is None:
      t = self._ones[c] = torch.ones(c, dtype=torch.float32, device=self.device)
    return t

  def table(self, E):
    ptrs = tuple(p.data_ptr() for br in E.branches
                 for p in (br.kernel._w16, br.kernel._grad, br.gamma._master, br.beta._master, br.gamma._grad,
                           br.beta._grad, br.moving_mean, br.moving_var))
    if E.table is not None and ptrs == E.ptrs:
      return E.table
    segs = []
    for i, br in enumerate(E.branches):
      S = self.sources[i]
      col = E.doff - (self.dtot - S.wd)
      segs.append(dict(w=br.kernel._w16, tt=E.tt[i], m=S.m, s=S.s, gamma=br.gamma._master, beta=br.beta._master,
                       moving_mean=br.moving_mean, moving_var=br.moving_var, mean=E.mean[i], rstd=E.rstd[i],
                       dgamma=br.gamma._grad, dbeta=br.beta._grad, dw=br.kernel._grad, wd1=S.wd1[:, col:],
                       wd2=S.wd2[:, col:], wt=S.wt[:, col:], ld=S.wd, c=S.c, koff=S.koff))
    E.table, E.ptrs = capi.dres_seg_table(segs, self.device), ptrs
    return E.table

  def begin(self, training):
    if training:
      self.generation += 1
    return DenseResidualPass(self, training)


class DenseResidualPass(object):

  def __init__(self, plan, training):
    self.plan, self.training = plan, training
    self.generation = plan.generation
    self.xcat = self.dzcat = None
    self.acts = []
    self.lens = None
    self.B = self.T = 0

  def add_source(self, x):
    plan = self.plan
    i = len(self.acts)
    S = plan.sources[i]
    B, T, C = x.data.shape
    assert C == S.c
    if i == 0:
      self.B, self.T, self.lens = B, T, x.lens
      self.xcat = torch.empty((B, T, plan.ktot), dtype=torch.bfloat16, device=x.data.device)
    elif (B, T) != (self.B, self.T) or x.lens is not self.lens:
      raise ValueError("dense-residual plan: block inputs of different geometry")
    self.acts.append(x)
    xs = self.xcat[:, :, S.koff:S.koff + C]
    part = capi.dres_copy_cols(x.data, xs, self.lens, want_colsum=self.training)
    if self.training:
      S.gram.zero_()
      capi.conv1x1_wgrad_grouped([dict(x=xs, dy=x.data, dw=S.gram.view(1, C, C))], in_len=self.lens,
                                 pingpong=GRAM_PINGPONG or capi.deterministic())
      capi.dres_cov(part, S.gram, B * T, S.s, S.m, S.chl)

  def forward_end(self, k):
    plan = self.plan
    E = plan.ends[k]
    assert len(self.acts) >= k + 1
    table = plan.table(E)
    for br in E.branches:
      br.kernel.w16, br.gamma.master, br.beta.master
    if self.training:
      items = []
      for i, br in enumerate(E.branches):
        S = plan.sources[i]
        items.append(dict(x=br.kernel._w16.view(1, E.cout, S.c), w=S.chl.view(1, 2 * S.c, S.c),
                          y=E.tt[i].view(1, E.cout, 2 * S.c)))
      capi.conv1x1_fwd_grouped(items, out_f32=True)
    capi.dres_bn_fwd(table, k + 1, E.cout, E.kk, E.wp, E.shift, self.B * self.T, E.eps, E.momentum, self.training)
    R = torch.empty((self.B, self.T, E.cout), dtype=torch.bfloat16, device=self.xcat.device)
    capi.conv1x1_cat_fwd(self.xcat[:, :, :E.kk], E.wp, R, in_len=self.lens)
    return dict(y=R, scale=plan.ones(E.cout), shift=E.shift, dres=self, k=k)

  def backward_end(self, k, dz, mean_dz, dz_lens=None):
    plan = self.plan
    if self.generation != plan.generation:
      raise RuntimeError("dense-residual plan: a later training forward pass overwrote this pass's saved statistics")
    E = plan.ends[k]
    N = self.B * self.T
    if self.dzcat is None:
      self.dzcat = torch.empty((self.B, self.T, plan.dtot), dtype=torch.bfloat16, device=dz.device)
    for br in E.branches:
      br.kernel.grad, br.gamma.grad, br.beta.grad
    capi.dres_copy_cols(dz, self.dzcat[:, :, E.doff:E.doff + E.cout], dz_lens)
    E.P.zero_()
    capi.conv1x1_wgrad_grouped([dict(x=self.xcat[:, :, :E.kk], dy=dz, dw=E.P.view(1, E.cout, E.kk))],
                               in_len=self.lens, pingpong=P_PINGPONG or capi.deterministic())
    capi.dres_bn_bwd(plan.table(E), k + 1, E.cout, E.kk, E.P, mean_dz, N, E.coef)
    inp = self.acts[k]
    if not inp.requires_grad:
      return
    S = plan.sources[k]
    g = inp.grad_buffer()
    capi.conv1x1_cat_fwd(self.dzcat[:, :, E.doff:], S.wd1, g, out_len=self.lens, accumulate=inp.grad_init)
    capi.gemm_nt(S.wd2, S.wt, out=S.mf, out_f32=True)
    capi.cast_f32_to_bf16(S.mf[:S.c], S.mb)
    capi.conv1x1_cat_fwd(self.xcat[:, :, S.koff:S.koff + S.c], S.mb, g, out_len=self.lens, bias=S.mf[S.c],
                         accumulate=True)
    inp.grad_init = True
```

Before: 946,000 frames/sec.

## Cache LARC weight norms in optimizer apply and overwrite conv grads instead of zero+accumulate

Adds cached weight-norm partials: the apply kernel writes per-chunk weight sum-of-squares for the updated weights, so the next prepare pass can skip re-reading weights for tensors whose norm is still valid. Also lets conv weight-gradient kernels that have a single owner write gradients directly instead of accumulating, and zeroes only the gradient chunks that will not be overwritten. This cuts memory traffic in the optimizer and gradient zeroing, at the cost of extra host-side bookkeeping (epochs, masks, pinned copies) and more complex correctness invariants.

```diff
diff --git a/include/os2s.h b/include/os2s.h
--- a/include/os2s.h
+++ b/include/os2s.h
@@ -123,6 +123,8 @@
                          const uint16_t* dy, float* dw, const int32_t* in_len, int B, int Tin,
                          int Cin, int Cout, int K, int stride, int dil, int padL, int Tout,
                          int accumulate, void* workspace, size_t workspace_bytes);
+int os2s_conv1d_wgrad_single_owner(int B, int Tin, int Cin, int Cout, int K, int stride, int dil, int Tout,
+                                   long long x_row_stride);
 
 int os2s_bn_finalize(os2s_stream_t stream, const float* partial, int nparts, int C,
                      long long count, const float* gamma, const float* beta,
@@ -223,6 +225,20 @@
                          int chunk_begin, int chunk_end, const int32_t* chunk_tensor,
                          const float* tensor_l2, const float* tensor_mult,
                          const float* tensor_wd_mask, int zero_grads);
+int os2s_opt_prepare_cached(os2s_stream_t stream, const os2s_opt_config_t* cfg, void* state,
+                            const float* grads, const float* weights, int nchunks, int ntensors,
+                            const int32_t* chunk_tensor, const int32_t* tensor_chunk_begin,
+                            const float* tensor_l2, float* partial, float* tensor_gnorm2, float* tensor_wnorm2,
+                            float* tensor_amax, float* tensor_mult, float* tensor_v,
+                            float* partial_w, const uint8_t* tensor_need_w, int* mismatch);
+int os2s_opt_apply_range_cached(os2s_stream_t stream, const os2s_opt_config_t* cfg, const void* state,
+                                float* grads, float* weights, float* m1, float* m2, uint16_t* w16,
+                                int chunk_begin, int chunk_end, const int32_t* chunk_tensor,
+                                const float* tensor_l2, const float* tensor_mult,
+                                const float* tensor_wd_mask, int zero_grads, float* partial_w);
+int os2s_fill_zero_chunks(os2s_stream_t stream, float* buf, int nchunks, const int32_t* chunk_tensor,
+                          const uint8_t* tensor_skip, const int32_t* tensor_chunk_begin,
+                          const long long* tensor_numel);
 int os2s_cast_f32_to_bf16(os2s_stream_t stream, const float* src, uint16_t* dst,
                           long long n);
 int os2s_conv_weight_dgrad_copy(os2s_stream_t stream, const uint16_t* w16,
diff --git a/openseq2seq_amd/capi.py b/openseq2seq_amd/capi.py
--- a/openseq2seq_amd/capi.py
+++ b/openseq2seq_amd/capi.py
@@ -344,6 +344,12 @@
   return out
 
 
+def conv1d_wgrad_single_owner(x, dy, K, *, stride=1, dil=1):
+  B, Tin, Cin = x.shape
+  return bool(_lib.C.os2s_conv1d_wgrad_single_owner(B, Tin, Cin, dy.shape[2], int(K), int(stride), int(dil),
+                                                    dy.shape[1], x.stride(1)))
+
+
 class _CWgradGroup(_lib.ctypes.Structure):
   _fields_ = [("x", c_void_p), ("dy", c_void_p), ("dw", c_void_p), ("x_row_stride", c_ll)]
 
@@ -666,7 +672,15 @@
 
 
 def opt_step(cfg, state, grads, weights, m1, m2, w16, chunk_tensor, tensor_chunk_begin,
-             tensor_l2, tensor_wd_mask, partial, gnorm2, wnorm2, amax, mult, tensor_v):
+             tensor_l2, tensor_wd_mask, partial, gnorm2, wnorm2, amax, mult, tensor_v, *, partial_w=None,
+             need_w=None, mismatch=None):
+  if partial_w is not None:
+    opt_prepare(cfg, state, grads, weights, chunk_tensor, tensor_chunk_begin, tensor_l2, partial, gnorm2, wnorm2,
+                amax, mult, tensor_v, partial_w=partial_w, need_w=need_w, mismatch=mismatch)
+    opt_apply_range(cfg, state, grads, weights, m1, m2, w16, 0, chunk_tensor.numel(), chunk_tensor, tensor_l2, mult,
+                    tensor_wd_mask=tensor_wd_mask, partial_w=partial_w)
+    return
+  assert need_w is None and mismatch is None
   nchunks = chunk_tensor.numel()
   ntensors = tensor_chunk_begin.numel() - 1
   _lib.C.os2s_opt_step(_stream(), _lib.ctypes.byref(cfg), _ptr(state, torch.uint8),
@@ -681,23 +695,41 @@
 
 
 def opt_prepare(cfg, state, grads, weights, chunk_tensor, tensor_chunk_begin, tensor_l2, partial, gnorm2, wnorm2,
-                amax, mult, tensor_v):
+                amax, mult, tensor_v, *, partial_w=None, need_w=None, mismatch=None):
   nchunks = chunk_tensor.numel()
   ntensors = tensor_chunk_begin.numel() - 1
-  _lib.C.os2s_opt_prepare(_stream(), _lib.ctypes.byref(cfg), _ptr(state, torch.uint8), _ptr(grads, torch.float32),
-                          _ptr(weights, torch.float32), nchunks, ntensors, _ptr(chunk_tensor, torch.int32),
-                          _ptr(tensor_chunk_begin, torch.int32), _ptr(tensor_l2, torch.float32, True),
-                          _ptr(partial, torch.float32), _ptr(gnorm2, torch.float32), _ptr(wnorm2, torch.float32),
-                          _ptr(amax, torch.float32), _ptr(mult, torch.float32), _ptr(tensor_v, torch.float32, True))
+  assert partial_w is None or partial_w.numel() == nchunks
+  assert need_w is None or (partial_w is not None and need_w.numel() == ntensors)
+  assert mismatch is None or partial_w is not None
+  _lib.C.os2s_opt_prepare_cached(
+      _stream(), _lib.ctypes.byref(cfg), _ptr(state, torch.uint8), _ptr(grads, torch.float32),
+      _ptr(weights, torch.float32), nchunks, ntensors, _ptr(chunk_tensor, torch.int32),
+      _ptr(tensor_chunk_begin, torch.int32), _ptr(tensor_l2, torch.float32, True),
+      _ptr(partial, torch.float32), _ptr(gnorm2, torch.float32), _ptr(wnorm2, torch.float32),
+      _ptr(amax, torch.float32), _ptr(mult, torch.float32), _ptr(tensor_v, torch.float32, True),
+      _ptr(partial_w, torch.float32, True), _ptr(need_w, torch.uint8, True), _ptr(mismatch, torch.int32, True))
 
 
 def opt_apply_range(cfg, state, grads, weights, m1, m2, w16, chunk_begin, chunk_end, chunk_tensor, tensor_l2, mult,
-                    zero_grads=False):
-  _lib.C.os2s_opt_apply_range(_stream(), _lib.ctypes.byref(cfg), _ptr(state, torch.uint8), _ptr(grads, torch.float32),
-                              _ptr(weights, torch.float32), _ptr(m1, torch.float32, True),
-                              _ptr(m2, torch.float32, True), _ptr(w16, torch.bfloat16, True), int(chunk_begin),
-                              int(chunk_end), _ptr(chunk_tensor, torch.int32), _ptr(tensor_l2, torch.float32, True),
-                              _ptr(mult, torch.float32), c_void_p(0), int(bool(zero_grads)))
+                    zero_grads=False, *, tensor_wd_mask=None, partial_w=None):
+  assert 0 <= chunk_begin <= chunk_end <= chunk_tensor.numel()
+  assert partial_w is None or partial_w.numel() == chunk_tensor.numel()
+  _lib.C.os2s_opt_apply_range_cached(
+      _stream(), _lib.ctypes.byref(cfg), _ptr(state, torch.uint8), _ptr(grads, torch.float32),
+      _ptr(weights, torch.float32), _ptr(m1, torch.float32, True),
+      _ptr(m2, torch.float32, True), _ptr(w16, torch.bfloat16, True), int(chunk_begin),
+      int(chunk_end), _ptr(chunk_tensor, torch.int32), _ptr(tensor_l2, torch.float32, True),
+      _ptr(mult, torch.float32), _ptr(tensor_wd_mask, torch.float32, True), int(bool(zero_grads)),
+      _ptr(partial_w, torch.float32, True))
+
+
+def fill_zero_chunks(buf, chunk_tensor, tensor_skip, tensor_chunk_begin, tensor_numel):
+  nt = tensor_chunk_begin.numel() - 1
+  assert buf.numel() == chunk_tensor.numel() * opt_chunk_elems() and buf.is_contiguous()
+  assert nt >= 1 and tensor_skip.numel() == nt and tensor_numel.numel() == nt
+  _lib.C.os2s_fill_zero_chunks(_stream(), _ptr(buf, torch.float32), chunk_tensor.numel(),
+                               _ptr(chunk_tensor, torch.int32), _ptr(tensor_skip, torch.uint8),
+                               _ptr(tensor_chunk_begin, torch.int32), _ptr(tensor_numel, torch.int64))
 
 
 def cast_f32_to_bf16(src, dst):
diff --git a/openseq2seq_amd/csrc/conv1d_wgrad.hip b/openseq2seq_amd/csrc/conv1d_wgrad.hip
--- a/openseq2seq_amd/csrc/conv1d_wgrad.hip
+++ b/openseq2seq_amd/csrc/conv1d_wgrad.hip
@@ -1027,6 +1027,32 @@
   return OS2S_OK;
 }
 
+enum { kWgradOther = 0, kWgradPingPong = 1, kWgradOneWave = 3 };
+static int wgrad_tap_quad_choice(os2s::WgradArgs a, long long x_row_stride, bool grouped, int* units, size_t* smem_out) {
+  using namespace os2s;
+  const int B = a.B, Tin = a.Tin, Tout = a.Tout, Cin = a.Cin, Cout = a.Cout, K = a.K, stride = a.stride, dil = a.dil;
+  const bool pp_shape = stride == 1 && K >= 2 && B <= 64 && Cout >= 128 && Cin >= 64 &&
+                        Tin < 65536 && Tout <= 255 * 64 && 63 + 3 * dil + 1 <= 96 &&
+                        (long long)Tin * x_row_stride * 2 < (1ll << 30) &&
+                        (long long)Tin * x_row_stride * 2 < (1ll << 31) &&
+                        (long long)Tout * Cout * 2 < (1ll << 31);
+  const int pp_units = ceil_div(Cout, 128) * ceil_div(Cin, 128) * ceil_div(K, kWppTaps);
+  const bool sw_shape = pp_shape && 63 + 3 * dil + 1 <= kSwXInstr * 16 &&
+                        Cout % 128 == 0 && Cin % 128 == 0;
+  *units = pp_units;
+  if (sw_shape && g_wgrad_variant == 3 && !grouped) {
+    wgrad_tap_quad_geometry(a, kSwXBuf);
+    *smem_out = (size_t)kSwRing * (kSwYBuf + kSwXBuf) + a.steptab_bytes;
+    if (*smem_out <= 160 * 1024) return kWgradOneWave;
+  }
+  if (pp_shape && g_wgrad_variant != 0 && (grouped || g_wgrad_variant == 1 || pp_units >= g_wgrad_pp_min_units)) {
+    wgrad_tap_quad_geometry(a, 24 * 1024);
+    *smem_out = (size_t)2 * 64 * 256 + (size_t)3 * a.xbuf_bytes + a.steptab_bytes + (a.dbg ? 2 * 48 * 10 * 8 : 0);
+    if (*smem_out <= 160 * 1024) return kWgradPingPong;
+  }
+  return kWgradOther;
+}
+
 static int conv1d_wgrad_impl_g(os2s_stream_t stream, const uint16_t* x, long long x_row_stride,
                                const uint16_t* dy, float* dw, const int32_t* in_len, int B,
                                int Tin, int Cin, int Cout, int K, int stride, int dil,
@@ -1046,44 +1072,37 @@
     for (int i = 0; i < ngroups; ++i) { a.gx[i] = groups[i].x; a.gdy[i] = groups[i].dy; a.gdw[i] = groups[i].dw; }
   }
 
-  const bool pp_shape = stride == 1 && K >= 2 && B <= 64 && Cout >= 128 && Cin >= 64 &&
-                        Tin < 65536 && Tout <= 255 * 64 && 63 + 3 * dil + 1 <= 96 &&
-                        (long long)Tin * x_row_stride * 2 < (1ll << 30) &&
-                        (long long)Tin * x_row_stride * 2 < (1ll << 31) &&
-                        (long long)Tout * Cout * 2 < (1ll << 31);
-  const int pp_units = ceil_div(Cout, 128) * ceil_div(Cin, 128) * ceil_div(K, kWppTaps);
-  const bool sw_shape = pp_shape && 63 + 3 * dil + 1 <= kSwXInstr * 16 &&
-                        Cout % 128 == 0 && Cin % 128 == 0;
-  if (sw_shape && g_wgrad_variant == 3 && !groups) {
+  int pp_units = 0;
+  size_t tq_smem = 0;
+  const int choice = wgrad_tap_quad_choice(a, x_row_stride, groups != nullptr, &pp_units, &tq_smem);
+  if (choice == kWgradOneWave) {
     wgrad_tap_quad_geometry(a, kSwXBuf);
-    const size_t smem = (size_t)kSwRing * (kSwYBuf + kSwXBuf) + a.steptab_bytes;
-    if (smem <= 160 * 1024) {
+    {
       const int grid = wgrad_split_grid(a, pp_units, workspace, workspace_bytes);
 #ifdef OS2S_SW_ABLATE
       switch (g_wgrad_sw_ablate) {
-        case 1: OS2S_LAUNCH_LDS(conv1d_wgrad_sw_kernel<1>, dim3(grid), dim3(256), smem, (hipStream_t)stream, a); return OS2S_OK;
-        case 2: OS2S_LAUNCH_LDS(conv1d_wgrad_sw_kernel<2>, dim3(grid), dim3(256), smem, (hipStream_t)stream, a); return OS2S_OK;
-        case 3: OS2S_LAUNCH_LDS(conv1d_wgrad_sw_kernel<3>, dim3(grid), dim3(256), smem, (hipStream_t)stream, a); return OS2S_OK;
-        case 4: OS2S_LAUNCH_LDS(conv1d_wgrad_sw_kernel<4>, dim3(grid), dim3(256), smem, (hipStream_t)stream, a); return OS2S_OK;
-        case 5: OS2S_LAUNCH_LDS(conv1d_wgrad_sw_kernel<5>, dim3(grid), dim3(256), smem, (hipStream_t)stream, a); return OS2S_OK;
-        case 8: OS2S_LAUNCH_LDS(conv1d_wgrad_sw_kernel<8>, dim3(grid), dim3(256), smem, (hipStream_t)stream, a); return OS2S_OK;
+        case 1: OS2S_LAUNCH_LDS(conv1d_wgrad_sw_kernel<1>, dim3(grid), dim3(256), tq_smem, (hipStream_t)stream, a); return OS2S_OK;
+        case 2: OS2S_LAUNCH_LDS(conv1d_wgrad_sw_kernel<2>, dim3(grid), dim3(256), tq_smem, (hipStream_t)stream, a); return OS2S_OK;
+        case 3: OS2S_LAUNCH_LDS(conv1d_wgrad_sw_kernel<3>, dim3(grid), dim3(256), tq_smem, (hipStream_t)stream, a); return OS2S_OK;
+        case 4: OS2S_LAUNCH_LDS(conv1d_wgrad_sw_kernel<4>, dim3(grid), dim3(256), tq_smem, (hipStream_t)stream, a); return OS2S_OK;
+        case 5: OS2S_LAUNCH_LDS(conv1d_wgrad_sw_kernel<5>, dim3(grid), dim3(256), tq_smem, (hipStream_t)stream, a); return OS2S_OK;
+        case 8: OS2S_LAUNCH_LDS(conv1d_wgrad_sw_kernel<8>, dim3(grid), dim3(256), tq_smem, (hipStream_t)stream, a); return OS2S_OK;
         default: break;
       }
 #endif
-      OS2S_LAUNCH_LDS(conv1d_wgrad_sw_kernel<0>, dim3(grid), dim3(256), smem, (hipStream_t)stream, a);
+      OS2S_LAUNCH_LDS(conv1d_wgrad_sw_kernel<0>, dim3(grid), dim3(256), tq_smem, (hipStream_t)stream, a);
       return OS2S_OK;
     }
   }
 
-  if (pp_shape && g_wgrad_variant != 0 && (groups || g_wgrad_variant == 1 || pp_units >= g_wgrad_pp_min_units)) {
+  if (choice == kWgradPingPong) {
     wgrad_tap_quad_geometry(a, 24 * 1024);
-    const size_t smem = (size_t)2 * 64 * 256 + (size_t)3 * a.xbuf_bytes + a.steptab_bytes + (a.dbg ? 2 * 48 * 10 * 8 : 0);
-    if (smem <= 160 * 1024) {
+    {
       const int grid = wgrad_split_grid(a, a.NG * pp_units, workspace, workspace_bytes);
       if (a.dbg) {
-        OS2S_LAUNCH_LDS(conv1d_wgrad_pp_kernel<true>, dim3(grid), dim3(512), smem, (hipStream_t)stream, a);
+        OS2S_LAUNCH_LDS(conv1d_wgrad_pp_kernel<true>, dim3(grid), dim3(512), tq_smem, (hipStream_t)stream, a);
       } else {
-        OS2S_LAUNCH_LDS(conv1d_wgrad_pp_kernel<false>, dim3(grid), dim3(512), smem, (hipStream_t)stream, a);
+        OS2S_LAUNCH_LDS(conv1d_wgrad_pp_kernel<false>, dim3(grid), dim3(512), tq_smem, (hipStream_t)stream, a);
       }
       return OS2S_OK;
     }
@@ -1157,6 +1176,17 @@
   return OS2S_OK;
 }
 
+extern "C" int os2s_conv1d_wgrad_single_owner(int B, int Tin, int Cin, int Cout, int K, int stride, int dil, int Tout,
+                                              long long x_row_stride) {
+  if (B < 1 || Tin < 1 || Tout < 1 || Cin < 8 || Cout < 8 || K < 1 || stride < 1 || dil < 1) return 0;
+  os2s::WgradArgs a = wgrad_args(nullptr, x_row_stride, nullptr, nullptr, nullptr, B, Tin, Cin, Cout, 0);
+  a.Tout = Tout; a.K = K; a.stride = stride; a.dil = dil;
+  a.dbg = g_wgrad_dbg;
+  int units = 0;
+  size_t smem = 0;
+  return wgrad_tap_quad_choice(a, x_row_stride, false, &units, &smem) != kWgradOther ? 1 : 0;
+}
+
 extern "C" int os2s_conv1d_wgrad_ws(os2s_stream_t stream, const uint16_t* x, long long x_row_stride,
                                     const uint16_t* dy, float* dw, const int32_t* in_len, int B,
                                     int Tin, int Cin, int Cout, int K, int stride, int dil,
diff --git a/openseq2seq_amd/csrc/optimizer.hip b/openseq2seq_amd/csrc/optimizer.hip
--- a/openseq2seq_amd/csrc/optimizer.hip
+++ b/openseq2seq_amd/csrc/optimizer.hip
@@ -75,41 +75,90 @@
   }
 }
 
-template <bool NEED_W>
+__device__ __forceinline__ float thread_sum_squares(const f32x4 (&v)[kChunk / 4 / 256]) {
+  float s = v[0][1] * v[0][1];
+  s = __builtin_fmaf(v[0][0], v[0][0], s);
+  s = __builtin_fmaf(v[0][2], v[0][2], s);
+  s = __builtin_fmaf(v[0][3], v[0][3], s);
+#pragma unroll
+  for (int i = 1; i < kChunk / 4 / 256; ++i) {
+#pragma unroll
+    for (int e = 0; e < 4; ++e) s = __builtin_fmaf(v[i][e], v[i][e], s);
+  }
+  return s;
+}
+
+__device__ __forceinline__ float chunk_sum_squares(const f32x4 (&w)[kChunk / 4 / 256], float* red4) {
+  float s = wave_sum(thread_sum_squares(w));
+  if ((threadIdx.x & 63) == 0) red4[threadIdx.x >> 6] = s;
+  __syncthreads();
+  float b = 0.f;
+  if (threadIdx.x == 0) {
+    for (int k = 0; k < 4; ++k) b += red4[k];
+  }
+  return b;
+}
+
 __global__ __launch_bounds__(256) void mt_grad_stats_kernel(
     const float* __restrict__ grads, const float* __restrict__ weights,
     const int32_t* __restrict__ chunk_tensor, const float* __restrict__ tensor_l2,
-    const OptDeviceState* __restrict__ st, int world_size, float* __restrict__ partial) {
-  __shared__ float red[4][4];
+    OptDeviceState* __restrict__ st, int world_size, float* __restrict__ partial,
+    float* __restrict__ partial_w, const uint8_t* __restrict__ tensor_need_w, int need_default,
+    int* __restrict__ mismatch) {
+  constexpr int N = kChunk / 4 / 256;
+  __shared__ float red[4][3];
+  __shared__ float red_w[4];
   const int c = blockIdx.x;
   const int ti = chunk_tensor[c];
-  const float inv = 1.f / (st->grad_scale_latched * (float)world_size);
+  const float scale = st->loss_scale;
+  if (c == 0 && threadIdx.x == 0) st->grad_scale_latched = scale;
+  const float inv = 1.f / (scale * (float)world_size);
   const float l2 = tensor_l2 ? tensor_l2[ti] : 0.f;
+  const bool need_w = (tensor_need_w ? tensor_need_w[ti] != 0 : need_default != 0) || l2 != 0.f;
+  const bool read_w = need_w || (mismatch != nullptr && partial_w != nullptr);
   const f32x4* g4 = reinterpret_cast<const f32x4*>(grads + (long long)c * kChunk);
   const f32x4* w4 = reinterpret_cast<const f32x4*>(weights + (long long)c * kChunk);
-  float sg = 0.f, sw = 0.f, mx = 0.f, nan = 0.f;
-#pragma unroll
-  for (int i = 0; i < kChunk / 4 / 256; ++i) {
-    const f32x4 g = g4[i * 256 + threadIdx.x];
-    f32x4 w = {0.f, 0.f, 0.f, 0.f};
-    if (NEED_W) w = w4[i * 256 + threadIdx.x];
+  f32x4 g[N], w[N];
+#pragma unroll
+  for (int i = 0; i < N; ++i) g[i] = g4[i * 256 + threadIdx.x];
+  if (read_w) {
+#pragma unroll
+    for (int i = 0; i < N; ++i) w[i] = w4[i * 256 + threadIdx.x];
+  } else {
+#pragma unroll
+    for (int i = 0; i < N; ++i) w[i] = f32x4{0.f, 0.f, 0.f, 0.f};
+  }
+  float mx = 0.f, nan = 0.f;
+#pragma unroll
+  for (int i = 0; i < N; ++i) {
 #pragma unroll
     for (int e = 0; e < 4; ++e) {
-      const float ge = NEED_W ? g[e] * inv + l2 * w[e] : g[e] * inv;
-      sg += ge * ge;
-      sw += w[e] * w[e];
+      const float ge = need_w ? __builtin_fmaf(inv, g[i][e], l2 * w[i][e]) : inv * g[i][e];
+      g[i][e] = ge;
       mx = fmaxf(mx, fabsf(ge));
       nan = (ge != ge) ? 1.f : nan;
     }
   }
-  sg = wave_sum(sg); sw = wave_sum(sw); mx = wave_max(mx); nan = wave_max(nan);
+  float sg = thread_sum_squares(g);
+  float sw = 0.f;
+  if (read_w) sw = chunk_sum_squares(w, red_w);
+  sg = wave_sum(sg); mx = wave_max(mx); nan = wave_max(nan);
   const int lane = threadIdx.x & 63, wid = threadIdx.x >> 6;
-  if (lane == 0) { red[wid][0] = sg; red[wid][1] = sw; red[wid][2] = mx; red[wid][3] = nan; }
+  if (lane == 0) { red[wid][0] = sg; red[wid][1] = mx; red[wid][2] = nan; }
   __syncthreads();
   if (threadIdx.x == 0) {
-    float a = 0.f, b = 0.f, m = 0.f, n = 0.f;
-    for (int w = 0; w < 4; ++w) { a += red[w][0]; b += red[w][1]; m = fmaxf(m, red[w][2]); n = fmaxf(n, red[w][3]); }
-    partial[c * 4 + 0] = a; partial[c * 4 + 1] = b; partial[c * 4 + 2] = m; partial[c * 4 + 3] = n;
+    float a = 0.f, m = 0.f, n = 0.f;
+    for (int k = 0; k < 4; ++k) { a += red[k][0]; m = fmaxf(m, red[k][1]); n = fmaxf(n, red[k][2]); }
+    if (partial_w) {
+      if (need_w) {
+        partial_w[c] = sw;
+      } else {
+        const float cached = partial_w[c];
+        if (read_w && __float_as_uint(cached) != __float_as_uint(sw)) atomicAdd(mismatch, 1);
+        sw = cached;
+      }
+    }
+    partial[c * 4 + 0] = a; partial[c * 4 + 1] = sw; partial[c * 4 + 2] = m; partial[c * 4 + 3] = n;
   }
 }
 
@@ -272,8 +321,9 @@
     float* __restrict__ m2, bf16_t* __restrict__ w16, const int32_t* __restrict__ chunk_tensor,
     const float* __restrict__ tensor_l2, const float* __restrict__ tensor_mult,
     const float* __restrict__ tensor_wd_mask, os2s_opt_config_t cfg,
-    const OptDeviceState* __restrict__ st, int chunk0, int zero_grads) {
+    const OptDeviceState* __restrict__ st, int chunk0, int zero_grads, float* __restrict__ partial_w) {
   constexpr int N = kChunk / 4 / 256;
+  __shared__ float red_w[4];
   const int c = blockIdx.x + chunk0;
   if (st->skip) {
     if (zero_grads) {
@@ -338,9 +388,30 @@
       __builtin_nontemporal_store(o, reinterpret_cast<u32x2*>(w16 + off));
     }
   }
-}
-
-__global__ void opt_latch_scale_kernel(OptDeviceState* st) { st->grad_scale_latched = st->loss_scale; }
+  if (partial_w) {
+    const float sw = chunk_sum_squares(w, red_w);
+    if (threadIdx.x == 0) partial_w[c] = sw;
+  }
+}
+
+__global__ __launch_bounds__(256) void fill_zero_chunks_kernel(float* __restrict__ buf,
+                                                               const int32_t* __restrict__ chunk_tensor,
+                                                               const uint8_t* __restrict__ tensor_skip,
+                                                               const int32_t* __restrict__ tensor_chunk_begin,
+                                                               const long long* __restrict__ tensor_numel) {
+  const int c = blockIdx.x;
+  const int t = chunk_tensor[c];
+  if (tensor_skip[t]) {
+    if (c != tensor_chunk_begin[t + 1] - 1) return;
+    const long long first = tensor_numel[t] - (long long)(c - tensor_chunk_begin[t]) * kChunk;
+    float* p = buf + (long long)c * kChunk;
+    for (long long i = (first < 0 ? 0 : first) + threadIdx.x; i < kChunk; i += 256) p[i] = 0.f;
+    return;
+  }
+  f32x4* p = reinterpret_cast<f32x4*>(buf + (long long)c * kChunk);
+#pragma unroll
+  for (int i = 0; i < kChunk / 4 / 256; ++i) p[i * 256 + threadIdx.x] = f32x4{0.f, 0.f, 0.f, 0.f};
+}
 
 __global__ void opt_init_state_kernel(OptDeviceState* st, float loss_scale) {
   st->global_step = 0; st->scaler_iteration = 0; st->last_overflow_iteration = -1;
@@ -436,37 +507,44 @@
   return OS2S_OK;
 }
 
+extern "C" int os2s_opt_prepare_cached(os2s_stream_t stream_, const os2s_opt_config_t* cfg, void* state,
+                                       const float* grads, const float* weights, int nchunks, int ntensors,
+                                       const int32_t* chunk_tensor, const int32_t* tensor_chunk_begin,
+                                       const float* tensor_l2, float* partial, float* tensor_gnorm2,
+                                       float* tensor_wnorm2, float* tensor_amax, float* tensor_mult, float* tensor_v,
+                                       float* partial_w, const uint8_t* tensor_need_w, int* mismatch) {
+  OS2S_REQUIRE(cfg && state && grads && weights && chunk_tensor && tensor_chunk_begin);
+  OS2S_REQUIRE(partial && tensor_gnorm2 && tensor_wnorm2 && tensor_amax && tensor_mult);
+  OS2S_REQUIRE(nchunks >= 1 && ntensors >= 1 && cfg->world_size >= 1);
+  OS2S_REQUIRE(partial_w || (!tensor_need_w && !mismatch));
+  if (cfg->optimizer == 2) OS2S_REQUIRE(tensor_v);
+  hipStream_t stream = (hipStream_t)stream_;
+  OptDeviceState* st = (OptDeviceState*)state;
+  const int need_default = (tensor_l2 != nullptr || cfg->use_larc) ? 1 : 0;
+  OS2S_LAUNCH(mt_grad_stats_kernel, dim3(nchunks), dim3(256), 0, stream, grads, weights, chunk_tensor, tensor_l2, st,
+              cfg->world_size, partial, partial_w, tensor_need_w, need_default, mismatch);
+  OS2S_LAUNCH(mt_tensor_reduce_kernel, dim3(ntensors), dim3(256), 0, stream, partial,
+              tensor_chunk_begin, tensor_gnorm2, tensor_wnorm2, tensor_amax, tensor_mult);
+  OS2S_LAUNCH(mt_finalize_kernel, dim3(1), dim3(256), 0, stream, ntensors, *cfg, st,
+              tensor_gnorm2, tensor_wnorm2, tensor_amax, tensor_mult, tensor_v);
+  return OS2S_OK;
+}
+
 extern "C" int os2s_opt_prepare(os2s_stream_t stream_, const os2s_opt_config_t* cfg, void* state,
                                 const float* grads, const float* weights, int nchunks, int ntensors,
                                 const int32_t* chunk_tensor, const int32_t* tensor_chunk_begin,
                                 const float* tensor_l2, float* partial, float* tensor_gnorm2, float* tensor_wnorm2,
                                 float* tensor_amax, float* tensor_mult, float* tensor_v) {
-  OS2S_REQUIRE(cfg && state && grads && weights && chunk_tensor && tensor_chunk_begin);
-  OS2S_REQUIRE(partial && tensor_gnorm2 && tensor_wnorm2 && tensor_amax && tensor_mult);
-  OS2S_REQUIRE(nchunks >= 1 && ntensors >= 1 && cfg->world_size >= 1);
-  if (cfg->optimizer == 2) OS2S_REQUIRE(tensor_v);
-  hipStream_t stream = (hipStream_t)stream_;
-  OptDeviceState* st = (OptDeviceState*)state;
-  OS2S_LAUNCH(opt_latch_scale_kernel, dim3(1), dim3(1), 0, stream, st);
-  if (tensor_l2 != nullptr || cfg->use_larc) {
-    OS2S_LAUNCH(mt_grad_stats_kernel<true>, dim3(nchunks), dim3(256), 0, stream, grads, weights,
-                chunk_tensor, tensor_l2, st, cfg->world_size, partial);
-  } else {
-    OS2S_LAUNCH(mt_grad_stats_kernel<false>, dim3(nchunks), dim3(256), 0, stream, grads, weights,
-                chunk_tensor, tensor_l2, st, cfg->world_size, partial);
-  }
-  OS2S_LAUNCH(mt_tensor_reduce_kernel, dim3(ntensors), dim3(256), 0, stream, partial,
-              tensor_chunk_begin, tensor_gnorm2, tensor_wnorm2, tensor_amax, tensor_mult);
-  OS2S_LAUNCH(mt_finalize_kernel, dim3(1), dim3(256), 0, stream, ntensors, *cfg, st,
-              tensor_gnorm2, tensor_wnorm2, tensor_amax, tensor_mult, tensor_v);
-  return OS2S_OK;
-}
-
-extern "C" int os2s_opt_apply_range(os2s_stream_t stream_, const os2s_opt_config_t* cfg, const void* state,
-                                    float* grads, float* weights, float* m1, float* m2, uint16_t* w16,
-                                    int chunk_begin, int chunk_end, const int32_t* chunk_tensor,
-                                    const float* tensor_l2, const float* tensor_mult,
-                                    const float* tensor_wd_mask, int zero_grads) {
+  return os2s_opt_prepare_cached(stream_, cfg, state, grads, weights, nchunks, ntensors, chunk_tensor,
+                                 tensor_chunk_begin, tensor_l2, partial, tensor_gnorm2, tensor_wnorm2, tensor_amax,
+                                 tensor_mult, tensor_v, nullptr, nullptr, nullptr);
+}
+
+extern "C" int os2s_opt_apply_range_cached(os2s_stream_t stream_, const os2s_opt_config_t* cfg, const void* state,
+                                           float* grads, float* weights, float* m1, float* m2, uint16_t* w16,
+                                           int chunk_begin, int chunk_end, const int32_t* chunk_tensor,
+                                           const float* tensor_l2, const float* tensor_mult,
+                                           const float* tensor_wd_mask, int zero_grads, float* partial_w) {
   OS2S_REQUIRE(cfg && state && grads && weights && chunk_tensor && tensor_mult);
   OS2S_REQUIRE(chunk_begin >= 0 && chunk_end >= chunk_begin);
   if (cfg->optimizer != 0) OS2S_REQUIRE(m1);
@@ -477,7 +555,7 @@
   const int n = chunk_end - chunk_begin;
 #define OS2S_APPLY(OPT)                                                                    \
   OS2S_LAUNCH(mt_apply_kernel<OPT>, dim3(n), dim3(256), 0, stream, grads, weights, m1, m2, \
-              w16, chunk_tensor, tensor_l2, tensor_mult, tensor_wd_mask, *cfg, st, chunk_begin, zero_grads ? 1 : 0)
+              w16, chunk_tensor, tensor_l2, tensor_mult, tensor_wd_mask, *cfg, st, chunk_begin, zero_grads ? 1 : 0, partial_w)
   switch (cfg->optimizer) {
     case 0: OS2S_APPLY(0); break;
     case 1: OS2S_APPLY(1); break;
@@ -485,6 +563,24 @@
     default: OS2S_APPLY(3); break;
   }
 #undef OS2S_APPLY
+  return OS2S_OK;
+}
+
+extern "C" int os2s_opt_apply_range(os2s_stream_t stream_, const os2s_opt_config_t* cfg, const void* state,
+                                    float* grads, float* weights, float* m1, float* m2, uint16_t* w16,
+                                    int chunk_begin, int chunk_end, const int32_t* chunk_tensor,
+                                    const float* tensor_l2, const float* tensor_mult,
+                                    const float* tensor_wd_mask, int zero_grads) {
+  return os2s_opt_apply_range_cached(stream_, cfg, state, grads, weights, m1, m2, w16, chunk_begin, chunk_end,
+                                     chunk_tensor, tensor_l2, tensor_mult, tensor_wd_mask, zero_grads, nullptr);
+}
+
+extern "C" int os2s_fill_zero_chunks(os2s_stream_t stream, float* buf, int nchunks, const int32_t* chunk_tensor,
+                                     const uint8_t* tensor_skip, const int32_t* tensor_chunk_begin,
+                                     const long long* tensor_numel) {
+  OS2S_REQUIRE(buf && chunk_tensor && tensor_skip && tensor_chunk_begin && tensor_numel && nchunks >= 1);
+  OS2S_LAUNCH(fill_zero_chunks_kernel, dim3(nchunks), dim3(256), 0, (hipStream_t)stream, buf, chunk_tensor,
+              tensor_skip, tensor_chunk_begin, tensor_numel);
   return OS2S_OK;
 }
 
diff --git a/openseq2seq_amd/models/model.py b/openseq2seq_amd/models/model.py
--- a/openseq2seq_amd/models/model.py
+++ b/openseq2seq_amd/models/model.py
@@ -225,10 +225,8 @@
       iter_size = p.get('iter_size', 1)
       micro = self._step_count % iter_size
       if micro == 0:
-        if self._store.grads_zeroed:
-          self._store.grads_zeroed = False
-        else:
-          self._store.zero_grads()
+        self._store.begin_grad_epoch(already_zeroed=self._store.grads_zeroed)
+        self._store.grads_zeroed = False
       last_micro = (micro == iter_size - 1)
       overlap = self._reducer is not None and last_micro
       snap = None
@@ -240,7 +238,7 @@
       if getattr(self, "_halves_enabled", None) is not None and self._halves_enabled():
         loss = self._forward_backward_halves(batch)
       else:
-        tape = Tape(on_done=self._reducer.mark_done if overlap else None)
+        tape = Tape(on_done=self._grads_final if overlap else None)
         tape.defer_free = DEFER_TAPE_FREE
         loss = self._forward_backward(batch, tape)
         tape.backward()
@@ -253,6 +251,7 @@
         loss = self._recover_gru_abort(batch, loss, snap, micro, overlap, ran_persistent)
       self._step_count += 1
       if last_micro:
+        self._store.finish_grad_epoch()
         if self._reducer is not None:
           self._reducer.finish()
         if p.get('os2s_async_optimizer', ASYNC_OPTIMIZER):
@@ -264,6 +263,10 @@
     finally:
       set_side_stream_enabled(prev)
     return loss
+
+  def _grads_final(self, offset):
+    self._store.finish_grad_epoch(offset)
+    self._reducer.mark_done(offset)
 
   def _has_gru_layers(self):
     for part in (getattr(self, "_encoder", None), getattr(self, "_decoder", None)):
@@ -306,7 +309,7 @@
       self._store.grads.copy_(snap[1])
     else:
       raise RuntimeError("persistent GRU abort inside an accumulation window before a snapshot existed")
-    tape = Tape(on_done=self._reducer.mark_done if overlap else None)
+    tape = Tape(on_done=self._grads_final if overlap else None)
     loss = self._forward_backward(batch, tape)
     tape.backward()
     torch.cuda.current_stream().synchronize()
diff --git a/openseq2seq_amd/optimizers/flat_params.py b/openseq2seq_amd/optimizers/flat_params.py
--- a/openseq2seq_amd/optimizers/flat_params.py
+++ b/openseq2seq_amd/optimizers/flat_params.py
@@ -7,12 +7,32 @@
 
 from .. import capi
 
-
-def _guarded(slot, wt=False):
+CACHED_WNORM = None
+CHECK_WNORM = None
+GRAD_OVERWRITE = None
+
+
+def cached_wnorm():
+  return os.environ.get("OS2S_OPT_CACHED_WNORM", "1") != "0" if CACHED_WNORM is None else bool(CACHED_WNORM)
+
+
+def check_wnorm():
+  return os.environ.get("OS2S_OPT_CHECK_WNORM", "0") == "1" if CHECK_WNORM is None else bool(CHECK_WNORM)
+
+
+def grad_overwrite():
+  return os.environ.get("OS2S_GRAD_OVERWRITE", "1") != "0" if GRAD_OVERWRITE is None else bool(GRAD_OVERWRITE)
+
+
+def _guarded(slot, wt=False, marks_w=False, is_grad=False):
   def get(self):
     st = self.store
     if st is not None and (st._pending or st._wt_event is not None):
       st._ready(self, wt)
+    if marks_w:
+      self.need_w = True
+    elif is_grad and self.overwrite_first and st is not None and self.grad_epoch != st.grad_epoch:
+      st.prepare_grad(self, can_overwrite=False, keep=True)
     return getattr(self, slot)
 
   def put(self, value):
@@ -22,9 +42,10 @@
 
 class Param(object):
   __slots__ = ("name", "shape", "index", "offset", "numel", "l2", "kind", "store",
-               "_master", "_grad", "_w16", "_wt16", "wt_offset", "trainable_mask", "logical_out", "logical_in")
-  master = _guarded("_master")
-  grad = _guarded("_grad")
+               "_master", "_grad", "_w16", "_wt16", "wt_offset", "trainable_mask", "logical_out", "logical_in",
+               "need_w", "overwrite_first", "grad_epoch")
+  master = _guarded("_master", marks_w=True)
+  grad = _guarded("_grad", is_grad=True)
   w16 = _guarded("_w16")
   wt16 = _guarded("_wt16", wt=True)
 
@@ -35,12 +56,17 @@
     self.logical_in = None
     self.store = None
     self._master = self._grad = self._w16 = self._wt16 = None
-
-
-def _whole(slot):
+    self.need_w = True
+    self.overwrite_first = False
+    self.grad_epoch = -1
+
+
+def _whole(slot, marks_w=False):
   def get(self):
     if self._pending or self._wt_event is not None:
       self.wait_all()
+    if marks_w:
+      self.invalidate_wnorm()
     return getattr(self, slot)
 
   def put(self, value):
@@ -50,7 +76,7 @@
 
 class FlatParams(object):
 
-  master = _whole("_master")
+  master = _whole("_master", marks_w=True)
   grads = _whole("_grads")
   m1 = _whole("_m1")
   m2 = _whole("_m2")
@@ -63,6 +89,7 @@
     self._pending, self._wt_event, self._main_stream, self._opt_stream = [], None, None, None
     self._done_upto = 0
     self.grads_zeroed = False
+    self.grad_epoch = 0
     self._master = self._grads = self._m1 = self._m2 = self._w16 = self._wt16 = self._t_v = None
     self.params = []
     self.state = {}
@@ -117,6 +144,13 @@
     self.tensor_l2 = torch.tensor([p.l2 for p in self.params], dtype=torch.float32, device=dev)
     self.l2_active = any(float(p.l2) != 0.0 for p in self.params)
     self.partial = torch.zeros(off // ch * 4, dtype=torch.float32, device=dev)
+    self.partial_w = torch.zeros(off // ch, dtype=torch.float32, device=dev)
+    self._need_w_dev = torch.ones(max(nt, 1), dtype=torch.uint8, device=dev)
+    self._need_w_sent = b"\x01" * nt
+    self._wnorm_mismatch = torch.zeros(1, dtype=torch.int32, device=dev)
+    self._skip_fill_dev = torch.zeros(max(nt, 1), dtype=torch.uint8, device=dev)
+    self._skip_fill_sent = b"\x00" * nt
+    self.tensor_numel = torch.tensor([p.numel for p in self.params], dtype=torch.int64, device=dev)
     self.t_gnorm2 = torch.zeros(nt, dtype=torch.float32, device=dev)
     self.t_wnorm2 = torch.zeros(nt, dtype=torch.float32, device=dev)
     self.t_amax = torch.zeros(nt, dtype=torch.float32, device=dev)
@@ -159,7 +193,75 @@
                                   self._wt_tiles)
 
   def zero_grads(self):
+    self.grad_epoch += 1
     self.grads.zero_()
+
+  def invalidate_wnorm(self):
+    for p in self.params:
+      p.need_w = True
+
+  def _mask(self, flags, dev_tensor, sent):
+    cur = bytes(bytearray(flags))
+    if cur != sent:
+      host = torch.frombuffer(bytearray(cur), dtype=torch.uint8)
+      if dev_tensor.is_cuda:
+        host = host.pin_memory()
+      dev_tensor.copy_(host, non_blocking=True)
+    return dev_tensor, cur
+
+  def need_w_mask(self):
+    m, self._need_w_sent = self._mask([p.need_w for p in self.params], self._need_w_dev, self._need_w_sent)
+    return m
+
+  def weights_updated(self):
+    for p in self.params:
+      p.need_w = False
+
+  def wnorm_check_buffer(self):
+    return self._wnorm_mismatch if check_wnorm() else None
+
+  def wnorm_mismatches(self):
+    self.wait_all()
+    return int(self._wnorm_mismatch.item())
+
+  def begin_grad_epoch(self, already_zeroed=False):
+    self.grad_epoch += 1
+    on = grad_overwrite()
+    self._unfinished = [p for p in self.params if p.overwrite_first] if on else []
+    if already_zeroed:
+      return
+    skip = [on and p.overwrite_first for p in self.params]
+    if not any(skip):
+      self.zero_grads()
+      return
+    m, self._skip_fill_sent = self._mask(skip, self._skip_fill_dev, self._skip_fill_sent)
+    capi.fill_zero_chunks(self.grads, self.chunk_tensor, m, self.tensor_chunk_begin, self.tensor_numel)
+
+  def prepare_grad(self, p, can_overwrite=True, keep=False):
+    if not self.overwrites(p):
+      return True
+    p.grad_epoch = self.grad_epoch
+    if can_overwrite:
+      return False
+    if not keep:
+      p.overwrite_first = False
+    if self._pending:
+      self._ready(p)
+    p._grad.zero_()
+    return True
+
+  def overwrites(self, p):
+    return p.overwrite_first and p.grad_epoch != self.grad_epoch and grad_overwrite()
+
+  def finish_grad_epoch(self, offset=0):
+    todo = getattr(self, "_unfinished", None)
+    if todo is None:
+      todo = self._unfinished = [p for p in self.params if p.overwrite_first] if grad_overwrite() else []
+    while todo and todo[-1].offset >= offset:
+      p = todo.pop()
+      if p.overwrite_first and p.grad_epoch != self.grad_epoch:
+        p._grad.zero_()
+        p.grad_epoch = self.grad_epoch
 
   def _streams(self):
     cur = torch.cuda.current_stream()
diff --git a/openseq2seq_amd/optimizers/optimizers.py b/openseq2seq_amd/optimizers/optimizers.py
--- a/openseq2seq_amd/optimizers/optimizers.py
+++ b/openseq2seq_amd/optimizers/optimizers.py
@@ -4,6 +4,7 @@
 
 from .. import capi
 from ..utils.utils import check_params
+from . import flat_params
 from . import lr_policies
 from .automatic_loss_scaler import AutomaticLossScaler
 from .novograd import NovoGrad
@@ -98,11 +99,28 @@
     self.loss_scale_view = self.state[32:36].view(torch.float32)
     self.lr_view = self.state[36:40].view(torch.float32)
 
+  def _wnorm_cache(self):
+    s = self.store
+    if not (self.cfg.use_larc and flat_params.cached_wnorm()):
+      return {}, {}
+    return (dict(partial_w=s.partial_w, need_w=s.need_w_mask(), mismatch=s.wnorm_check_buffer()),
+            dict(partial_w=s.partial_w))
+
+  def _updated(self, cached):
+    s = self.store
+    if cached:
+      s.weights_updated()
+    else:
+      s.invalidate_wnorm()
+
   def run(self):
     s = self.store
-    capi.opt_step(self.cfg, self.state, s.grads, s.master, s.m1, s.m2, s.w16,
+    s.wait_all()
+    prep, _ = self._wnorm_cache()
+    capi.opt_step(self.cfg, self.state, s._grads, s._master, s._m1, s._m2, s._w16,
                   s.chunk_tensor, s.tensor_chunk_begin, s.tensor_l2 if s.l2_active else None, None, s.partial,
-                  s.t_gnorm2, s.t_wnorm2, s.t_amax, s.t_mult, s.t_v)
+                  s.t_gnorm2, s.t_wnorm2, s.t_amax, s.t_mult, s._t_v, **prep)
+    self._updated(bool(prep))
     s.refresh_dgrad_copies()
 
   def run_async(self, nranges=8):
@@ -116,15 +134,18 @@
     bounds = [(nchunks * i) // nranges for i in range(nranges + 1)]
     pending = []
     with torch.cuda.stream(side):
+      prep, apply = self._wnorm_cache()
       capi.opt_prepare(self.cfg, self.state, s._grads, s._master, s.chunk_tensor, s.tensor_chunk_begin,
                        s.tensor_l2 if s.l2_active else None, s.partial, s.t_gnorm2, s.t_wnorm2, s.t_amax,
-                       s.t_mult, s._t_v)
+                       s.t_mult, s._t_v, **prep)
       for c0, c1 in zip(bounds[:-1], bounds[1:]):
         capi.opt_apply_range(self.cfg, self.state, s._grads, s._master, s._m1, s._m2, s._w16, c0, c1,
-                             s.chunk_tensor, s.tensor_l2 if s.l2_active else None, s.t_mult, zero_grads=True)
+                             s.chunk_tensor, s.tensor_l2 if s.l2_active else None, s.t_mult, zero_grads=True,
+                             **apply)
         ev = torch.cuda.Event()
         ev.record(side)
         pending.append((c1 * s.chunk, ev))
+      self._updated(bool(prep))
       s.version = getattr(s, "version", 0) + 1
       s._refresh_dgrad_copies_raw()
       evw = torch.cuda.Event()
diff --git a/openseq2seq_amd/parts/cnns/conv_blocks.py b/openseq2seq_amd/parts/cnns/conv_blocks.py
--- a/openseq2seq_amd/parts/cnns/conv_blocks.py
+++ b/openseq2seq_amd/parts/cnns/conv_blocks.py
@@ -45,6 +45,7 @@
     self._set_geometry(name, cin, cout, k, stride, dilation, padding)
     self.momentum, self.eps = bn_momentum, bn_epsilon
     self.kernel = store.add(name + "/kernel", (k, cout, cin), initializer, kind="conv", l2=l2)
+    self.kernel.overwrite_first = True
     self._add_bn(store, bn_name, cout, l2)
 
   def _set_geometry(self, name, cin, cout, k, stride, dilation, padding):
@@ -102,15 +103,20 @@
        dy.is_contiguous() and x.stride(2) == 1 and x.stride(0) == x.shape[1] * x.stride(1):
       key = (tuple(x.shape), tuple(dy.shape), x.stride(1), self.k, self.dil, f["pad_left"],
              None if inp.lens is None else inp.lens.data_ptr())
+      self.kernel.store.prepare_grad(self.kernel, can_overwrite=False)
       tape.defer_conv_wgrad(self.kernel, key, dict(x=x, dy=dy, dw=self.kernel.grad), units,
                             dict(K=self.k, stride=1, dil=self.dil, pad_left=f["pad_left"], in_len=inp.lens))
       return
     global _WGRAD_RR
     _WGRAD_RR += 1
     with on_side_stream(dy.device, inp.data, dy, which=0 if WGRAD_STREAMS < 2 else (0, 2)[_WGRAD_RR & 1]):
+      store = self.kernel.store
+      owner = store.overwrites(self.kernel) and x.dim() == 3 and \
+          capi.conv1d_wgrad_single_owner(x, dy, self.k, stride=self.stride, dil=self.dil)
+      accumulate = store.prepare_grad(self.kernel, can_overwrite=owner)
       capi.conv1d_wgrad(inp.data, dy, self.k, stride=self.stride, dil=self.dil,
                         pad_left=f["pad_left"], in_len=inp.lens, out=self.kernel.grad,
-                        accumulate=True)
+                        accumulate=accumulate)
 
   def backward_branch(self, inp, dy, f, final=False):
     self.backward_weights(inp, dy, f)
@@ -387,6 +393,8 @@
         br.backward_branch(inp, dy, f)
     if wgrouped:
       with on_side_stream(dz.device, *([w[1].data for w in wgrouped] + [w[2] for w in wgrouped])):
+        for br, _, _ in wgrouped:
+          br.kernel.store.prepare_grad(br.kernel, can_overwrite=False)
         for i0 in range(0, len(wgrouped), 16):
           capi.conv1x1_wgrad_grouped([dict(x=inp.data, dy=dy, dw=br.kernel.grad)
                                       for br, inp, dy in wgrouped[i0:i0 + 16]], in_len=wgrouped[0][1].lens,
diff --git a/openseq2seq_amd/parts/cnns/dense_residual.py b/openseq2seq_amd/parts/cnns/dense_residual.py
--- a/openseq2seq_amd/parts/cnns/dense_residual.py
+++ b/openseq2seq_amd/parts/cnns/dense_residual.py
@@ -171,6 +171,7 @@
     if self.dzcat is None:
       self.dzcat = torch.empty((self.B, self.T, plan.dtot), dtype=torch.bfloat16, device=dz.device)
     for br in E.branches:
+      br.kernel.store.prepare_grad(br.kernel, can_overwrite=False)
       br.kernel.grad, br.gamma.grad, br.beta.grad
     capi.dres_copy_cols(dz, self.dzcat[:, :, E.doff:E.doff + E.cout], dz_lens)
     E.P.zero_()
```

Measured after the change: 962,600 frames/sec (median of 6 runs). 1.02x the previous value.
